# anihcsam/OpenGaussian

Measured on AMD Instinct MI355X. Metric: fwd+bwd Mpix/s at 1080p, 1M Gaussians (RGB+6-D ins_feat); k-means it/s, higher is better.
Workload: dtype f32; 1 GPU; S1M-1080p RGB(SH3)+depth+alpha (all grads) + 6-ch ins_feat (grad to ins_feat) fwd+bwd, ONE fused 9-channel pass; gaussians=1000000, width=1920, height=1080, views_cycled=8, parallelism=single

## Files before the change

include/ogs_raster.h:

```cpp
#ifndef OGS_RASTER_H
#define OGS_RASTER_H

#include <stddef.h>
#include <stdint.h>

#ifdef __cplusplus
extern "C" {
#endif

#define OGS_OK 0
#define OGS_ERR_INVALID_ARG (-1)
#define OGS_ERR_HIP (-2)
#define OGS_ERR_UNSUPPORTED (-3)
#define OGS_ERR_SCRATCH_TOO_SMALL (-4)
#define OGS_ERR_DEVICE (-5)

#define OGS_TILE 16
#define OGS_MAX_CHANNELS 12

typedef struct OgsRasterFwdArgs {
    int32_t P;
    int32_t W, H;
    int32_t C;
    int32_t sh_degree;
    int32_t sh_coeffs;
    float tanfovx, tanfovy;
    float scale_modifier;
    int32_t prefiltered;
    int32_t debug;
    const float* bg;
    const float* means3D;
    const float* colors_precomp;
    const float* shs;
    const float* opacities;
    const float* scales;
    const float* rotations;
    const float* cov3D_precomp;
    const float* viewmatrix;
    const float* projmatrix;
    const float* campos;
    float* out_color;
    float* out_depth;
    float* out_alpha;
    int32_t* radii;
    void* geom_buffer;
    void* geom_tmp;
    void* image_buffer;
    uint32_t* point_list;
    void* binning_tmp;
    void* sorted_rec;
    void* quad_list;
    const int32_t* group_ids;
    int32_t num_groups;
    int32_t full_binning;
} OgsRasterFwdArgs;

typedef struct OgsRasterBwdArgs {
    int32_t P, W, H, C, sh_degree, sh_coeffs;
    float tanfovx, tanfovy, scale_modifier;
    int32_t debug;
    int32_t num_rendered;
    int32_t geom_channels;
    const float* bg;
    const float* means3D;
    const float* colors_precomp;
    const float* shs;
    const float* opacities;
    const float* scales;
    const float* rotations;
    const float* cov3D_precomp;
    const float* viewmatrix;
    const float* projmatrix;
    const float* campos;
    const int32_t* radii;
    const float* out_alpha;
    const float* dL_dcolor;
    const float* dL_ddepth;
    const float* dL_dalpha;
    const void* geom_buffer;
    const void* image_buffer;
    const uint32_t* point_list;
    const void* sorted_rec;
    const void* quad_list;
    void* bwd_tmp;
    float* dL_dmeans2D;
    float* dL_dcolors;
    float* dL_dopacity;
    float* dL_dmeans3D;
    float* dL_dcov3D;
    float* dL_dsh;
    float* dL_dscales;
    float* dL_drotations;
    int32_t num_groups;
    float* dL_dsh_rgb;
} OgsRasterBwdArgs;

int ogs_version(void);
const char* ogs_last_error(void);

int ogs_check_async_status(void);

size_t ogs_raster_geom_bytes(int32_t P, int32_t C);
size_t ogs_raster_geom_tmp_bytes(int32_t P);
size_t ogs_raster_image_bytes(int32_t W, int32_t H);
size_t ogs_raster_image_bytes_grouped(int32_t W, int32_t H, int32_t num_groups);
size_t ogs_raster_binning_tmp_bytes(int64_t num_rendered, int32_t W, int32_t H);
size_t ogs_raster_backward_tmp_bytes(int32_t P);
size_t ogs_raster_sorted_bytes(int64_t num_rendered, int32_t C);
size_t ogs_raster_quad_list_bytes(int64_t num_rendered);

int ogs_raster_forward_geometry(const OgsRasterFwdArgs* args, void* stream, int64_t* num_rendered_host);

int ogs_raster_forward_render(const OgsRasterFwdArgs* args, int64_t num_rendered, void* stream);

int ogs_raster_read_num_rendered_async(const OgsRasterFwdArgs* args, void* stream, uint32_t* host_pinned);
int ogs_raster_forward_render_deferred(const OgsRasterFwdArgs* args, int64_t capacity, void* stream);

size_t ogs_raster_tiny_max_points(void);
int ogs_raster_forward_tiny(const OgsRasterFwdArgs* args, void* stream);

int ogs_raster_forward_reblend(const OgsRasterFwdArgs* args, void* stream);

int ogs_raster_compact_kept(int32_t W, int32_t H, int32_t C, const void* image_buffer, const void* sorted_rec,
                            const void* quad_list, void* new_image_buffer, void* new_sorted_rec, void* new_quad_list,
                            void* stream);

typedef struct OgsGroupStatsArgs {
    const int32_t* labels;
    int32_t num_labels;
    float alpha_threshold;
    float* max_alpha;
    int64_t* count;
    float* feat_sum;
    void* stats_tmp;
} OgsGroupStatsArgs;

size_t ogs_raster_stats_image_bytes(int32_t W, int32_t H, int32_t num_groups);
size_t ogs_raster_stats_tmp_bytes(int32_t num_groups, int32_t num_labels, int32_t C);
int ogs_raster_forward_group_stats(const OgsRasterFwdArgs* args, const OgsGroupStatsArgs* stats, int64_t num_rendered,
                                   void* stream);

int ogs_raster_backward(const OgsRasterBwdArgs* args, void* stream);

int ogs_mark_visible(int32_t P, const float* means3D, const float* viewmatrix, const float* projmatrix,
                     uint8_t* present, void* stream);

int ogs_sh_grad_from_views(int32_t P, int32_t V, int32_t sh_degree, int32_t sh_coeffs, const float* means3D,
                           const float* campos, const float* dL_drgb, float* dL_dsh, void* stream);

int ogs_raster_export_binning(const OgsRasterFwdArgs* args, int64_t num_rendered, uint64_t* keys_out,
                              uint32_t* ranges_out, uint32_t* n_contrib_out, void* stream);

int ogs_prof_enable(int on);
int ogs_prof_filter(const char* prefix);
int ogs_prof_collect(char* buf, size_t n);

int ogs_selftest_wave_fold16(const float* in, float* out, void* stream);
int ogs_selftest_tile_order(const uint32_t* ranges, int64_t vtiles, uint32_t* order, void* stream);
size_t ogs_selftest_radix_tmp_bytes(int64_t n);
int ogs_selftest_radix_sort(uint32_t* keys0, uint32_t* vals0, uint32_t* keys1, uint32_t* vals1, int64_t n, int32_t key_bits,
                            int32_t variant, int32_t items, const uint32_t* n_dev, void* tmp, int32_t* result_buffer,
                            void* stream);

#ifdef __cplusplus
}
#endif
#endif
```

opengaussian_amd/_lib.py:

```python
from __future__ import annotations

import ctypes as C
import os

_HERE = os.path.dirname(os.path.abspath(__file__))
LIB_PATH = os.environ.get("OGS_LIB_PATH") or os.path.join(_HERE, "lib", "libogs_hip.so")

_f32p = C.POINTER(C.c_float)
_vp = C.c_void_p


class OgsRasterFwdArgs(C.Structure):
    _fields_ = [
        ("P", C.c_int32), ("W", C.c_int32), ("H", C.c_int32), ("C", C.c_int32),
        ("sh_degree", C.c_int32), ("sh_coeffs", C.c_int32),
        ("tanfovx", C.c_float), ("tanfovy", C.c_float), ("scale_modifier", C.c_float),
        ("prefiltered", C.c_int32), ("debug", C.c_int32),
        ("bg", _vp), ("means3D", _vp), ("colors_precomp", _vp), ("shs", _vp), ("opacities", _vp),
        ("scales", _vp), ("rotations", _vp), ("cov3D_precomp", _vp),
        ("viewmatrix", _vp), ("projmatrix", _vp), ("campos", _vp),
        ("out_color", _vp), ("out_depth", _vp), ("out_alpha", _vp), ("radii", _vp),
        ("geom_buffer", _vp), ("geom_tmp", _vp), ("image_buffer", _vp), ("point_list", _vp),
        ("binning_tmp", _vp), ("sorted_rec", _vp), ("quad_list", _vp), ("group_ids", _vp), ("num_groups", C.c_int32),
        ("full_binning", C.c_int32),
    ]


class OgsRasterBwdArgs(C.Structure):
    _fields_ = [
        ("P", C.c_int32), ("W", C.c_int32), ("H", C.c_int32), ("C", C.c_int32),
        ("sh_degree", C.c_int32), ("sh_coeffs", C.c_int32),
        ("tanfovx", C.c_float), ("tanfovy", C.c_float), ("scale_modifier", C.c_float),
        ("debug", C.c_int32), ("num_rendered", C.c_int32), ("geom_channels", C.c_int32),
        ("bg", _vp), ("means3D", _vp), ("colors_precomp", _vp), ("shs", _vp), ("opacities", _vp),
        ("scales", _vp), ("rotations", _vp), ("cov3D_precomp", _vp),
        ("viewmatrix", _vp), ("projmatrix", _vp), ("campos", _vp),
        ("radii", _vp), ("out_alpha", _vp), ("dL_dcolor", _vp), ("dL_ddepth", _vp), ("dL_dalpha", _vp),
        ("geom_buffer", _vp), ("image_buffer", _vp), ("point_list", _vp), ("sorted_rec", _vp), ("quad_list", _vp), ("bwd_tmp", _vp),
        ("dL_dmeans2D", _vp), ("dL_dcolors", _vp), ("dL_dopacity", _vp), ("dL_dmeans3D", _vp),
        ("dL_dcov3D", _vp), ("dL_dsh", _vp), ("dL_dscales", _vp), ("dL_drotations", _vp), ("num_groups", C.c_int32), ("dL_dsh_rgb", _vp),
    ]


class OgsAdamTensor(C.Structure):
    _fields_ = [("param", _vp), ("grad", _vp), ("exp_avg", _vp), ("exp_avg_sq", _vp), ("numel", C.c_int64),
                ("lr", C.c_double), ("step", C.c_int64)]


class OgsRowTensor(C.Structure):
    _fields_ = [("src", _vp), ("dst", _vp), ("width", C.c_int32), ("zero_new", C.c_int32)]


class OgsDensifyArgs(C.Structure):
    _fields_ = [("N", C.c_int32), ("grad_accum", _vp), ("denom", _vp), ("scaling", _vp), ("opacity", _vp),
                ("max_grad", C.c_float), ("min_opacity", C.c_float), ("extent", C.c_float), ("percent_dense", C.c_float),
                ("prune_world_size", C.c_int32)]


class OgsGroupStatsArgs(C.Structure):
    _fields_ = [("labels", _vp), ("num_labels", C.c_int32), ("alpha_threshold", C.c_float), ("max_alpha", _vp),
                ("count", _vp), ("feat_sum", _vp), ("stats_tmp", _vp)]


SIGNATURES = {
    "ogs_version": (C.c_int, []),
    "ogs_last_error": (C.c_char_p, []),
    "ogs_raster_geom_bytes": (C.c_size_t, [C.c_int32, C.c_int32]),
    "ogs_raster_geom_tmp_bytes": (C.c_size_t, [C.c_int32]),
    "ogs_raster_image_bytes": (C.c_size_t, [C.c_int32, C.c_int32]),
    "ogs_raster_image_bytes_grouped": (C.c_size_t, [C.c_int32, C.c_int32, C.c_int32]),
    "ogs_raster_binning_tmp_bytes": (C.c_size_t, [C.c_int64, C.c_int32, C.c_int32]),
    "ogs_raster_backward_tmp_bytes": (C.c_size_t, [C.c_int32]),
    "ogs_raster_sorted_bytes": (C.c_size_t, [C.c_int64, C.c_int32]),
    "ogs_raster_quad_list_bytes": (C.c_size_t, [C.c_int64]),
    "ogs_raster_forward_geometry": (C.c_int, [C.POINTER(OgsRasterFwdArgs), _vp, C.POINTER(C.c_int64)]),
    "ogs_raster_forward_render": (C.c_int, [C.POINTER(OgsRasterFwdArgs), C.c_int64, _vp]),
    "ogs_raster_read_num_rendered_async": (C.c_int, [C.POINTER(OgsRasterFwdArgs), _vp, _vp]),
    "ogs_raster_forward_render_deferred": (C.c_int, [C.POINTER(OgsRasterFwdArgs), C.c_int64, _vp]),
    "ogs_raster_stats_image_bytes": (C.c_size_t, [C.c_int32, C.c_int32, C.c_int32]),
    "ogs_raster_stats_tmp_bytes": (C.c_size_t, [C.c_int32, C.c_int32, C.c_int32]),
    "ogs_raster_forward_group_stats": (C.c_int, [C.POINTER(OgsRasterFwdArgs), C.POINTER(OgsGroupStatsArgs), C.c_int64, _vp]),
    "ogs_raster_backward": (C.c_int, [C.POINTER(OgsRasterBwdArgs), _vp]),
    "ogs_raster_tiny_max_points": (C.c_size_t, []),
    "ogs_raster_forward_tiny": (C.c_int, [C.POINTER(OgsRasterFwdArgs), _vp]),
    "ogs_raster_forward_reblend": (C.c_int, [C.POINTER(OgsRasterFwdArgs), _vp]),
    "ogs_raster_compact_kept": (C.c_int, [C.c_int32, C.c_int32, C.c_int32, _vp, _vp, _vp, _vp, _vp, _vp, _vp]),
    "ogs_mark_visible": (C.c_int, [C.c_int32, _vp, _vp, _vp, _vp, _vp]),
    "ogs_sh_grad_from_views": (C.c_int, [C.c_int32, C.c_int32, C.c_int32, C.c_int32, _vp, _vp, _vp, _vp, _vp]),
    "ogs_raster_export_binning": (C.c_int, [C.POINTER(OgsRasterFwdArgs), C.c_int64, _vp, _vp, _vp, _vp]),
    "ogs_selftest_wave_fold16": (C.c_int, [_vp, _vp, _vp]),
    "ogs_selftest_tile_order": (C.c_int, [_vp, C.c_int64, _vp, _vp]),
    "ogs_selftest_radix_tmp_bytes": (C.c_size_t, [C.c_int64]),
    "ogs_selftest_radix_sort": (C.c_int, [_vp, _vp, _vp, _vp, C.c_int64, C.c_int32, C.c_int32, C.c_int32, _vp, _vp, _vp, _vp]),
    "ogs_check_async_status": (C.c_int, []),
    "ogs_prof_enable": (C.c_int, [C.c_int]),
    "ogs_prof_filter": (C.c_int, [C.c_char_p]),
    "ogs_prof_collect": (C.c_int, [C.c_char_p, C.c_size_t]),
    "ogs_kmeans_tmp_bytes": (C.c_size_t, [C.c_int64, C.c_int32, C.c_int32]),
    "ogs_kmeans_lloyd": (C.c_int, [_vp, C.c_int64, C.c_int32, _vp, C.c_int32, C.c_int32, C.c_int32, C.c_int32,
                                   _vp, C.c_int64, _vp, _vp]),
    "ogs_kmeans_assign": (C.c_int, [_vp, C.c_int64, C.c_int32, _vp, C.c_int32, _vp, C.c_int64, _vp]),
    "ogs_mask_feature_sums": (C.c_int, [_vp, _vp, _vp, C.c_int32, C.c_int32, C.c_int64, C.c_int32, _vp, _vp]),
    "ogs_mask_feature_sums_backward": (C.c_int, [_vp, _vp, _vp, _vp, _vp, C.c_int32, C.c_int32, C.c_int64, _vp, _vp, _vp]),
    "ogs_mask_cohesion": (C.c_int, [_vp, _vp, _vp, C.c_int32, C.c_int32, C.c_int64, _vp, _vp]),
    "ogs_mask_cohesion_backward": (C.c_int, [_vp, _vp, _vp, _vp, C.c_int32, C.c_int32, C.c_int64, _vp, _vp, _vp]),
    "ogs_separation_loss": (C.c_int, [_vp, C.c_int32, C.c_int32, C.c_int32, _vp, _vp, _vp, _vp]),
    "ogs_adam_step": (C.c_int, [C.POINTER(OgsAdamTensor), C.c_int32, C.c_double, C.c_double, C.c_double, _vp]),
    "ogs_rows_gather": (C.c_int, [C.POINTER(OgsRowTensor), C.c_int32, _vp, _vp, C.c_int64, _vp]),
    "ogs_densify_tmp_bytes": (C.c_size_t, [C.c_int32]),
    "ogs_densify_plan": (C.c_int, [C.POINTER(OgsDensifyArgs), _vp, C.POINTER(C.c_uint32), _vp]),
    "ogs_densify_map": (C.c_int, [C.c_int32, _vp, _vp, _vp, _vp, _vp]),
    "ogs_densify_split_children": (C.c_int, [C.c_int64, _vp, _vp, _vp, _vp, _vp, _vp, _vp, _vp, _vp, _vp]),
    "ogs_densify_stats": (C.c_int, [C.c_int32, _vp, C.c_int32, _vp, _vp, _vp, _vp, _vp, _vp]),
    "ogs_kmeans_accumulate": (C.c_int, [_vp, C.c_int64, C.c_int32, _vp, C.c_int32, C.c_int32, _vp, _vp, _vp]),
    "ogs_kmeans_update": (C.c_int, [_vp, C.c_int32, C.c_int32, C.c_int32, _vp, _vp, _vp]),
    "ogs_kmeans_gather": (C.c_int, [_vp, _vp, C.c_int64, C.c_int32, C.c_int32, _vp, _vp]),
}

_lib = None


class OgsError(RuntimeError):
    pass


def lib() -> C.CDLL:
    global _lib
    if _lib is None:
        if not os.path.exists(LIB_PATH):
            raise OgsError(f"{LIB_PATH} not found -- build it with `python -m opengaussian_amd.build` "
                           "(the product path has no CPU fallback)")
        l = C.CDLL(LIB_PATH)
        for name, (res, args) in SIGNATURES.items():
            fn = getattr(l, name)
            fn.restype = res
            fn.argtypes = args
        _lib = l
    return _lib


def check(rc: int, what: str):
    if rc != 0:
        raise OgsError(f"{what} failed (code {rc}): {lib().ogs_last_error().decode()}")


def prof_filter(prefix: str):
    check(lib().ogs_prof_filter(prefix.encode()), "ogs_prof_filter")


def prof_enable(mode):
    check(lib().ogs_prof_enable(int(mode)), "ogs_prof_enable")


def prof_collect() -> dict:
    import json
    buf = C.create_string_buffer(1 << 16)
    check(lib().ogs_prof_collect(buf, len(buf)), "ogs_prof_collect")
    return json.loads(buf.value.decode())


def ptr(t):
    return None if t is None else t.data_ptr()
```

opengaussian_amd/csrc/binning.hip:

```cpp
#include <stdlib.h>
#include <string.h>

#include "ogs_common.h"

namespace ogs {

namespace {

constexpr size_t kSweepHeaderWords = 4 * 256 + 4 + 60;
constexpr int kScanItems = 8;
constexpr int kScanTile = kBlock * kScanItems;

__device__ __forceinline__ uint32_t wave_inclusive_scan(uint32_t v) {
#pragma unroll
    for (int d = 1; d < kWave; d <<= 1) {
        uint32_t t = __shfl_up(v, d, kWave);
        if (lane_id() >= d) v += t;
    }
    return v;
}

__device__ __forceinline__ uint32_t block_exclusive_scan(uint32_t v, uint32_t& total, uint32_t* wave_sums ) {
    const int wave = threadIdx.x >> 6;
    const uint32_t inc = wave_inclusive_scan(v);
    if (lane_id() == kWave - 1) wave_sums[wave] = inc;
    __syncthreads();
    uint32_t base = 0, tot = 0;
#pragma unroll
    for (int w = 0; w < kBlock / kWave; ++w) {
        const uint32_t s = wave_sums[w];
        if (w < wave) base += s;
        tot += s;
    }
    total = tot;
    __syncthreads();
    return base + inc - v;
}

__device__ __forceinline__ void load_items(const uint32_t* __restrict__ in, const uint32_t* __restrict__ gather,
                                           int64_t base, int64_t n, uint32_t item[kScanItems]) {
#pragma unroll
    for (int i = 0; i < kScanItems; ++i) {
        const int64_t idx = base + i;
        uint32_t v = 0;
        if (idx < n) v = gather ? in[gather[idx]] : in[idx];
        item[i] = v;
    }
}

__global__ __launch_bounds__(kBlock) void scan_reduce_kernel(const uint32_t* __restrict__ in,
                                                             const uint32_t* __restrict__ gather, int64_t n,
                                                             uint32_t* __restrict__ partials, const uint32_t* __restrict__ n_dev) {
    __shared__ uint32_t wave_sums[4];
    if (n_dev) n = min(n, (int64_t)*n_dev);
    const int64_t base = (int64_t)blockIdx.x * kScanTile + (int64_t)threadIdx.x * kScanItems;
    uint32_t item[kScanItems];
    load_items(in, gather, base, n, item);
    uint32_t s = 0;
#pragma unroll
    for (int i = 0; i < kScanItems; ++i) s += item[i];
    uint32_t total;
    block_exclusive_scan(s, total, wave_sums);
    if (threadIdx.x == 0) partials[blockIdx.x] = total;
}

template <bool SUM_PARTIALS>
__global__ __launch_bounds__(kBlock) void scan_apply_kernel(const uint32_t* __restrict__ in,
                                                            const uint32_t* __restrict__ gather,
                                                            uint32_t* __restrict__ out, int64_t n,
                                                            const uint32_t* __restrict__ partial_offsets,
                                                            uint32_t* __restrict__ total_out, const uint32_t* __restrict__ n_dev) {
    __shared__ uint32_t wave_sums[4];
    if (n_dev) n = min(n, (int64_t)*n_dev);
    const int64_t base = (int64_t)blockIdx.x * kScanTile + (int64_t)threadIdx.x * kScanItems;
    uint32_t item[kScanItems];
    load_items(in, gather, base, n, item);
    uint32_t s = 0;
#pragma unroll
    for (int i = 0; i < kScanItems; ++i) s += item[i];
    uint32_t block_base = 0;
    if (SUM_PARTIALS) {
        uint32_t acc = 0;
        for (uint32_t j = threadIdx.x; j < blockIdx.x; j += kBlock) acc += partial_offsets[j];
        uint32_t tot;
        block_exclusive_scan(acc, tot, wave_sums);
        block_base = tot;
    } else if (partial_offsets) {
        block_base = partial_offsets[blockIdx.x];
    }
    uint32_t total;
    uint32_t run = block_exclusive_scan(s, total, wave_sums) + block_base;
#pragma unroll
    for (int i = 0; i < kScanItems; ++i) {
        const int64_t idx = base + i;
        if (idx < n) out[idx] = run;
        run += item[i];
    }
    if (total_out && threadIdx.x == 0) {
        if (SUM_PARTIALS) { if (blockIdx.x == gridDim.x - 1) *total_out = block_base + total; }
        else if (partial_offsets == nullptr) *total_out = total;
    }
}

__global__ void scan_total_kernel(const uint32_t* __restrict__ in, const uint32_t* __restrict__ gather,
                                  const uint32_t* __restrict__ out, int64_t n, uint32_t* __restrict__ total_out,
                                  const uint32_t* __restrict__ n_dev) {
    if (threadIdx.x == 0 && blockIdx.x == 0) {
        if (n_dev) n = min(n, (int64_t)*n_dev);
        if (n <= 0) { *total_out = 0u; return; }
        const uint32_t last = gather ? in[gather[n - 1]] : in[n - 1];
        *total_out = out[n - 1] + last;
    }
}

inline int scan_blocks(int64_t n) { return (int)((n + kScanTile - 1) / kScanTile); }
constexpr int kFlatScanBlocks = 16384;

template <int ITEMS>
__global__ __launch_bounds__(kBlock) void radix_hist_kernel(const uint32_t* __restrict__ keys, int64_t n_cap,
                                                            const uint32_t* __restrict__ n_dev, int shift,
                                                            int bits, uint32_t* __restrict__ hist, int nblocks, bool drop) {
    __shared__ uint32_t h[256];
    const int64_t n = n_dev ? min((int64_t)*n_dev, n_cap) : n_cap;
    const int ndig = 1 << bits;
    const uint32_t mask = ndig - 1;
    h[threadIdx.x] = 0;
    __syncthreads();
    const int64_t base = (int64_t)blockIdx.x * (kBlock * ITEMS);
#pragma unroll
    for (int i = 0; i < ITEMS; ++i) {
        const int64_t idx = base + i * kBlock + threadIdx.x;
        if (idx < n) {
            const uint32_t k = keys[idx];
            if (!(drop && k == kDropKey)) atomicAdd(&h[(k >> shift) & mask], 1u);
        }
    }
    __syncthreads();
    if ((int)threadIdx.x < ndig) hist[(size_t)threadIdx.x * nblocks + blockIdx.x] = h[threadIdx.x];
}

__global__ __launch_bounds__(kBlock) void radix_rowscan_kernel(uint32_t* __restrict__ hist, int nblocks,
                                                               uint32_t* __restrict__ row_total) {
    __shared__ uint32_t wave_sums[4];
    uint32_t* row = hist + (size_t)blockIdx.x * nblocks;
    uint32_t carry = 0;
    for (int base = 0; base < nblocks; base += kScanTile) {
        uint32_t item[kScanItems];
        const int b0 = base + (int)threadIdx.x * kScanItems;
        uint32_t sum = 0;
#pragma unroll
        for (int i = 0; i < kScanItems; ++i) {
            item[i] = (b0 + i < nblocks) ? row[b0 + i] : 0u;
            sum += item[i];
        }
        uint32_t total;
        uint32_t run = carry + block_exclusive_scan(sum, total, wave_sums);
#pragma unroll
        for (int i = 0; i < kScanItems; ++i) {
            if (b0 + i < nblocks) row[b0 + i] = run;
            run += item[i];
        }
        carry += total;
    }
    if (threadIdx.x == 0) row_total[blockIdx.x] = carry;
}

template <int ITEMS>
__global__ __launch_bounds__(kBlock) void radix_scatter_kernel(const uint32_t* __restrict__ keys_in,
                                                               const uint32_t* __restrict__ vals_in,
                                                               uint32_t* __restrict__ keys_out,
                                                               uint32_t* __restrict__ vals_out, int64_t n_cap,
                                                               const uint32_t* __restrict__ n_dev, int shift,
                                                               int bits, const uint32_t* __restrict__ offsets,
                                                               const uint32_t* __restrict__ row_total,
                                                               int nblocks, bool drop, uint32_t* __restrict__ kept_out) {
    __shared__ uint32_t wave_hist_s[kBlock / kWave][256];
    __shared__ uint32_t scan_sums[4];
    __shared__ uint32_t dig_start[256], glob_base[256];
    __shared__ uint32_t stage_k[kBlock * ITEMS], stage_v[kBlock * ITEMS];
    volatile uint32_t(*wave_hist)[256] = wave_hist_s;
    const int64_t n = n_dev ? min((int64_t)*n_dev, n_cap) : n_cap;
    const int ndig = 1 << bits;
    const uint32_t mask = ndig - 1;
    const int tid = threadIdx.x, lane = tid & 63, wave = tid >> 6;
#pragma unroll
    for (int w = 0; w < kBlock / kWave; ++w) wave_hist_s[w][tid] = 0;
    __syncthreads();

    const int64_t base = (int64_t)blockIdx.x * (kBlock * ITEMS) + (int64_t)wave * (ITEMS * kWave);
    uint32_t key[ITEMS], val[ITEMS], rank[ITEMS];
#pragma unroll
    for (int i = 0; i < ITEMS; ++i) {
        const int64_t idx = base + i * kWave + lane;
        const bool valid = idx < n;
        key[i] = valid ? keys_in[idx] : 0xFFFFFFFFu;
        val[i] = valid ? vals_in[idx] : 0u;
    }
    const uint64_t lt_mask = (1ull << lane) - 1ull;
#pragma unroll
    for (int i = 0; i < ITEMS; ++i) {
        const int64_t idx = base + i * kWave + lane;
        const bool valid = drop ? key[i] != kDropKey : idx < n;
        const uint32_t d = (key[i] >> shift) & mask;
        uint64_t peers = __ballot(valid);
        for (int b = 0; b < bits; ++b) {
            const bool bit = (d >> b) & 1u;
            const uint64_t m = __ballot(bit);
            peers &= bit ? m : ~m;
        }
        const uint32_t r = __popcll(peers & lt_mask);
        const uint32_t cnt = __popcll(peers);
        uint32_t pre = 0;
        if (valid) pre = wave_hist[wave][d];
        __builtin_amdgcn_wave_barrier();
        if (valid && r == 0) wave_hist[wave][d] = pre + cnt;
        __builtin_amdgcn_wave_barrier();
        rank[i] = pre + r;
    }
    __syncthreads();
    uint32_t run_len = 0;
    if (tid < ndig) {
#pragma unroll
        for (int w = 0; w < kBlock / kWave; ++w) {
            const uint32_t t = wave_hist_s[w][tid];
            wave_hist_s[w][tid] = run_len;
            run_len += t;
        }
    }
    uint32_t n_valid;
    const uint32_t local_start = block_exclusive_scan(run_len, n_valid, scan_sums);
    uint32_t dummy_total;
    const uint32_t digit_base = block_exclusive_scan(tid < ndig ? row_total[tid] : 0u, dummy_total, scan_sums);
    if (kept_out != nullptr && blockIdx.x == 0 && tid == 0) *kept_out = dummy_total;
    if (tid < ndig) {
        dig_start[tid] = local_start;
        glob_base[tid] = digit_base + offsets[(size_t)tid * nblocks + blockIdx.x] - local_start;
    }
    __syncthreads();
#pragma unroll
    for (int i = 0; i < ITEMS; ++i) {
        const int64_t idx = base + i * kWave + lane;
        if (drop ? key[i] != kDropKey : idx < n) {
            const uint32_t d = (key[i] >> shift) & mask;
            const uint32_t lp = dig_start[d] + wave_hist_s[wave][d] + rank[i];
            stage_k[lp] = key[i];
            stage_v[lp] = val[i];
        }
    }
    __syncthreads();
    for (uint32_t j = tid; j < n_valid; j += kBlock) {
        const uint32_t k = stage_k[j];
        const uint32_t pos = glob_base[(k >> shift) & mask] + j;
        keys_out[pos] = k;
        vals_out[pos] = stage_v[j];
    }
}

constexpr uint32_t kStatAgg = 1u << 30, kStatInc = 2u << 30, kStatMask = (1u << 30) - 1u;
constexpr int kSpinLimit = 1 << 22;
constexpr int kLookBack = 8;
constexpr int kHistAllBlocks = 256;

struct RadixPlanDev { int npass; int shift[4]; int bits[4]; };

__global__ __launch_bounds__(kBlock) void radix_hist_all_kernel(const uint32_t* __restrict__ keys, int64_t n_cap,
                                                                const uint32_t* __restrict__ n_dev, RadixPlanDev plan,
                                                                uint32_t* __restrict__ ghist , bool drop) {
    __shared__ uint32_t h[4][256];
    const int64_t n = n_dev ? min((int64_t)*n_dev, n_cap) : n_cap;
#pragma unroll
    for (int p = 0; p < 4; ++p) h[p][threadIdx.x] = 0;
    __syncthreads();
    for (int64_t idx = (int64_t)blockIdx.x * kBlock + threadIdx.x; idx < n; idx += (int64_t)gridDim.x * kBlock) {
        const uint32_t k = keys[idx];
        if (drop && k == kDropKey) continue;
#pragma unroll
        for (int p = 0; p < 4; ++p)
            if (p < plan.npass) atomicAdd(&h[p][(k >> plan.shift[p]) & ((1u << plan.bits[p]) - 1u)], 1u);
    }
    __syncthreads();
#pragma unroll
    for (int p = 0; p < 4; ++p)
        if (p < plan.npass && h[p][threadIdx.x] != 0) atomicAdd(&ghist[p * 256 + threadIdx.x], h[p][threadIdx.x]);
}

template <int ITEMS>
__global__ __launch_bounds__(kBlock) void radix_onesweep_kernel(const uint32_t* __restrict__ keys_in,
                                                                const uint32_t* __restrict__ vals_in,
                                                                uint32_t* __restrict__ keys_out,
                                                                uint32_t* __restrict__ vals_out, int64_t n_cap,
                                                                const uint32_t* __restrict__ n_dev, int shift, int bits,
                                                                const uint32_t* __restrict__ ghist ,
                                                                uint32_t* __restrict__ status ,
                                                                uint32_t* __restrict__ ticket ,
                                                                uint32_t* __restrict__ status_word ,
                                                                int spin_limit, bool drop,
                                                                uint32_t* __restrict__ kept_out) {
    __shared__ uint32_t wave_hist_s[kBlock / kWave][256];
    __shared__ uint32_t scan_sums[4];
    __shared__ uint32_t dig_start[256], glob_base[256];
    __shared__ uint32_t stage_k[kBlock * ITEMS], stage_v[kBlock * ITEMS];
    __shared__ uint32_t s_ticket;
    volatile uint32_t(*wave_hist)[256] = wave_hist_s;
    const int64_t n = n_dev ? min((int64_t)*n_dev, n_cap) : n_cap;
    const int ndig = 1 << bits;
    const uint32_t mask = ndig - 1;
    const int tid = threadIdx.x, lane = tid & 63, wave = tid >> 6;
    if (tid == 0) s_ticket = atomicAdd(ticket, 1u);
#pragma unroll
    for (int w = 0; w < kBlock / kWave; ++w) wave_hist_s[w][tid] = 0;
    __syncthreads();
    const uint32_t tile = s_ticket;
    if ((int64_t)tile * (kBlock * ITEMS) >= n) {
        if (kept_out != nullptr && tile == 0 && tid == 0) *kept_out = 0u;
        return;
    }

    const int64_t base = (int64_t)tile * (kBlock * ITEMS) + (int64_t)wave * (ITEMS * kWave);
    uint32_t key[ITEMS], val[ITEMS], rank[ITEMS];
#pragma unroll
    for (int i = 0; i < ITEMS; ++i) {
        const int64_t idx = base + i * kWave + lane;
        const bool valid = idx < n;
        key[i] = valid ? keys_in[idx] : 0xFFFFFFFFu;
        val[i] = valid ? vals_in[idx] : 0u;
    }
    const uint64_t lt_mask = (1ull << lane) - 1ull;
#pragma unroll
    for (int i = 0; i < ITEMS; ++i) {
        const int64_t idx = base + i * kWave + lane;
        const bool valid = drop ? key[i] != kDropKey : idx < n;
        const uint32_t d = (key[i] >> shift) & mask;
        uint64_t peers = __ballot(valid);
        for (int b = 0; b < bits; ++b) {
            const bool bit = (d >> b) & 1u;
            const uint64_t m = __ballot(bit);
            peers &= bit ? m : ~m;
        }
        const uint32_t r = __popcll(peers & lt_mask);
        const uint32_t cnt = __popcll(peers);
        uint32_t pre = 0;
        if (valid) pre = wave_hist[wave][d];
        __builtin_amdgcn_wave_barrier();
        if (valid && r == 0) wave_hist[wave][d] = pre + cnt;
        __builtin_amdgcn_wave_barrier();
        rank[i] = pre + r;
    }
    __syncthreads();
    uint32_t run_len = 0;
    if (tid < ndig) {
#pragma unroll
        for (int w = 0; w < kBlock / kWave; ++w) {
            const uint32_t t = wave_hist_s[w][tid];
            wave_hist_s[w][tid] = run_len;
            run_len += t;
        }
        __hip_atomic_store(&status[(size_t)tile * 256 + tid], (tile == 0 ? kStatInc : kStatAgg) | run_len,
                           __ATOMIC_RELAXED, __HIP_MEMORY_SCOPE_AGENT);
    }
    uint32_t n_valid;
    const uint32_t local_start = block_exclusive_scan(run_len, n_valid, scan_sums);
    uint32_t dummy_total;
    const uint32_t digit_base = block_exclusive_scan(tid < ndig ? ghist[tid] : 0u, dummy_total, scan_sums);
    if (kept_out != nullptr && tile == 0 && tid == 0) *kept_out = dummy_total;
    uint32_t before = 0;
    if (tid < ndig && tile > 0) {
        int64_t pb = (int64_t)tile - 1;
        int spins = 0;
        bool done = false;
        while (!done) {
            uint32_t sw[kLookBack];
#pragma unroll
            for (int k = 0; k < kLookBack; ++k)
                sw[k] = pb - k >= 0 ? __hip_atomic_load(&status[(size_t)(pb - k) * 256 + tid], __ATOMIC_RELAXED, __HIP_MEMORY_SCOPE_AGENT)
                                    : kStatInc;
            int used = 0;
#pragma unroll
            for (int k = 0; k < kLookBack; ++k) {
                if (done || used != k) continue;
                const uint32_t flag = sw[k] & ~kStatMask;
                if (flag == 0u) continue;
                before += sw[k] & kStatMask;
                used = k + 1;
                done = flag == kStatInc;
            }
            pb -= used;
            if (!done && used < kLookBack) {
                if (++spins > spin_limit) {
                    __hip_atomic_fetch_or(status_word, kAsyncRadixSpin, __ATOMIC_RELAXED, __HIP_MEMORY_SCOPE_SYSTEM);
                    break;
                }
                __builtin_amdgcn_s_sleep(1);
            }
        }
        __hip_atomic_store(&status[(size_t)tile * 256 + tid], kStatInc | ((before + run_len) & kStatMask),
                           __ATOMIC_RELAXED, __HIP_MEMORY_SCOPE_AGENT);
    }
    if (tid < ndig) {
        dig_start[tid] = local_start;
        glob_base[tid] = digit_base + before - local_start;
    }
    __syncthreads();
#pragma unroll
    for (int i = 0; i < ITEMS; ++i) {
        const int64_t idx = base + i * kWave + lane;
        if (drop ? key[i] != kDropKey : idx < n) {
            const uint32_t d = (key[i] >> shift) & mask;
            const uint32_t lp = dig_start[d] + wave_hist_s[wave][d] + rank[i];
            stage_k[lp] = key[i];
            stage_v[lp] = val[i];
        }
    }
    __syncthreads();
    for (uint32_t j = tid; j < n_valid; j += kBlock) {
        const uint32_t k = stage_k[j];
        const uint32_t pos = glob_base[(k >> shift) & mask] + j;
        if ((int64_t)pos < n) {
            keys_out[pos] = k;
            vals_out[pos] = stage_v[j];
        }
    }
}

constexpr int kRangeItems = 4;
__global__ __launch_bounds__(kBlock) void tile_ranges_kernel(const uint32_t* __restrict__ tile_keys, int64_t D_cap,
                                                             const uint32_t* __restrict__ n_dev,
                                                             uint2* __restrict__ ranges) {
    const int64_t D = n_dev ? min((int64_t)*n_dev, D_cap) : D_cap;
    const int64_t i0 = ((int64_t)blockIdx.x * kBlock + threadIdx.x) * kRangeItems;
    if (i0 >= D) return;
    uint32_t k[kRangeItems];
    if (i0 + kRangeItems <= D) {
        const uint4 v = *reinterpret_cast<const uint4*>(tile_keys + i0);
        k[0] = v.x; k[1] = v.y; k[2] = v.z; k[3] = v.w;
    } else {
#pragma unroll
        for (int j = 0; j < kRangeItems; ++j) k[j] = i0 + j < D ? tile_keys[i0 + j] : 0u;
    }
    uint32_t prev = i0 > 0 ? tile_keys[i0 - 1] : 0u;
#pragma unroll
    for (int j = 0; j < kRangeItems; ++j) {
        const int64_t i = i0 + j;
        if (i < D) {
            const uint32_t cur = k[j];
            if (i == 0) {
                ranges[cur].x = 0;
            } else if (prev != cur) {
                ranges[prev].y = (uint32_t)i;
                ranges[cur].x = (uint32_t)i;
            }
            if (i == D - 1) ranges[cur].y = (uint32_t)D;
            prev = cur;
        }
    }
}

__global__ __launch_bounds__(kBlock) void export_keys_kernel(const uint2* __restrict__ ranges,
                                                             const uint32_t* __restrict__ point_list,
                                                             const float4* __restrict__ rec, int recv4,
                                                             uint64_t* __restrict__ keys_out) {
    const uint32_t tile = blockIdx.x;
    const uint2 r = ranges[tile];
    for (uint32_t i = r.x + threadIdx.x; i < r.y; i += kBlock) {
        const uint32_t gid = point_list[i] & kGidMask;
        const uint32_t bits = __float_as_uint(rec[(size_t)gid * recv4].z);
        keys_out[i] = ((uint64_t)tile << 32) | bits;
    }
}

}

size_t scan_tmp_bytes(int64_t n) {
    size_t total = 0;
    int64_t m = n;
    while (true) {
        const int nb = scan_blocks(m);
        if (nb <= 1) break;
        total += align_up((size_t)nb * sizeof(uint32_t));
        m = nb;
    }
    return total + kAlign;
}

size_t sort_tmp_bytes(int64_t n) {
    const int64_t hist = (int64_t)256 * sort_blocks_for(n > 0 ? n : 1);
    const size_t legacy = align_up((size_t)hist * sizeof(uint32_t)) + align_up(256 * sizeof(uint32_t)) + scan_tmp_bytes(hist);
    const int64_t tiles4 = ((n > 0 ? n : 1) + kBlock * 4 - 1) / (kBlock * 4);
    const size_t sweep = align_up(kSweepHeaderWords * sizeof(uint32_t)) + 4 * align_up((size_t)256 * tiles4 * sizeof(uint32_t));
    return legacy > sweep ? legacy : sweep;
}

static int sweep_items_for(int64_t n, int forced) {
    if (forced == 4 || forced == 16) return forced;
    return n <= (int64_t)(256 << 10) ? 4 : 16;
}

bool radix_onesweep_enabled(int64_t n) {
    static const int forced = [] {
        const char* e = getenv("OGS_RADIX");
        return !e ? 0 : strcmp(e, "legacy") == 0 ? 1 : strcmp(e, "sweep") == 0 ? 2 : 0;
    }();
    if (forced == 1 || n >= (int64_t)kStatMask) return false;
    return forced == 2 || n <= (int64_t)(256 << 10);
}

namespace {
struct SweepTmp {
    uint32_t* ghist;
    uint32_t* ticket;
    uint32_t* status[4];
    size_t zero_bytes;
    static SweepTmp carve(void* tmp, int64_t n, int npass, int items_forced) {
        SweepTmp t;
        char* p = static_cast<char*>(tmp);
        t.ghist = reinterpret_cast<uint32_t*>(p);
        t.ticket = t.ghist + 4 * 256;
        const int items = sweep_items_for(n, items_forced);
        const int64_t tiles = ((n > 0 ? n : 1) + (int64_t)kBlock * items - 1) / ((int64_t)kBlock * items);
        const size_t table = align_up((size_t)256 * tiles * sizeof(uint32_t));
        char* q = p + align_up(kSweepHeaderWords * sizeof(uint32_t));
        for (int i = 0; i < 4; ++i) t.status[i] = reinterpret_cast<uint32_t*>(q + (size_t)i * table);
        t.zero_bytes = align_up(kSweepHeaderWords * sizeof(uint32_t)) + (size_t)npass * table;
        return t;
    }
};
}

int radix_sort_begin(const uint32_t* keys, int64_t n, const uint32_t* n_dev, int npass, const int* shifts, const int* bits,
                     void* tmp, hipStream_t stream, int debug, bool drop, int items) {
    if (n <= 0) return OGS_OK;
    if (npass < 1 || npass > 4) { set_error("radix_sort_begin: npass=%d out of range", npass); return OGS_ERR_INVALID_ARG; }
    const SweepTmp t = SweepTmp::carve(tmp, n, npass, items);
    OGS_HIP_CHECK(hipMemsetAsync(tmp, 0, t.zero_bytes, stream));
    RadixPlanDev plan{};
    plan.npass = npass;
    for (int i = 0; i < npass; ++i) {
        if (bits[i] < 1 || bits[i] > 8) { set_error("radix_sort_begin: bits=%d out of range", bits[i]); return OGS_ERR_INVALID_ARG; }
        plan.shift[i] = shifts[i];
        plan.bits[i] = bits[i];
    }
    const int64_t want = (n + kBlock * 16 - 1) / (kBlock * 16);
    const int grid = (int)(want < 1 ? 1 : (want > kHistAllBlocks ? kHistAllBlocks : want));
    OGS_LAUNCH(radix_hist_all_kernel, dim3(grid), dim3(kBlock), 0, stream, keys, n, n_dev, plan, t.ghist, drop);
    OGS_LAUNCH_CHECK(debug, stream);
    return OGS_OK;
}

int radix_sort_pass(int pass, int npass, const uint32_t* keys_in, const uint32_t* vals_in, uint32_t* keys_out, uint32_t* vals_out,
                    int64_t n, int shift, int bits, void* tmp, hipStream_t stream, int debug, const uint32_t* n_dev, bool drop,
                    uint32_t* kept_out, int items_forced, int spin_limit) {
    if (n <= 0) return OGS_OK;
    const SweepTmp t = SweepTmp::carve(tmp, n, npass, items_forced);
    const int items = sweep_items_for(n, items_forced);
    const int nb = (int)((n + (int64_t)kBlock * items - 1) / ((int64_t)kBlock * items));
    uint32_t* status_word = async_status_word();
    if (!status_word) return OGS_ERR_HIP;
    if (spin_limit < 0) spin_limit = kSpinLimit;
    if (items == 4) {
        OGS_LAUNCH(radix_onesweep_kernel<4>, dim3(nb), dim3(kBlock), 0, stream, keys_in, vals_in, keys_out, vals_out, n, n_dev,
                   shift, bits, (const uint32_t*)(t.ghist + pass * 256), t.status[pass], t.ticket + pass, status_word, spin_limit,
                   drop, kept_out);
    } else {
        OGS_LAUNCH(radix_onesweep_kernel<16>, dim3(nb), dim3(kBlock), 0, stream, keys_in, vals_in, keys_out, vals_out, n, n_dev,
                   shift, bits, (const uint32_t*)(t.ghist + pass * 256), t.status[pass], t.ticket + pass, status_word, spin_limit,
                   drop, kept_out);
    }
    OGS_LAUNCH_CHECK(debug, stream);
    return OGS_OK;
}

int exclusive_scan_u32(const uint32_t* in, const uint32_t* gather, uint32_t* out, int64_t n, uint32_t* total,
                       void* tmp, hipStream_t stream, int debug, const uint32_t* n_dev) {
    if (n <= 0) {
        if (total) OGS_HIP_CHECK(hipMemsetAsync(total, 0, sizeof(uint32_t), stream));
        return OGS_OK;
    }
    const int nb = scan_blocks(n);
    if (nb == 1) {
        OGS_LAUNCH(scan_apply_kernel<false>, dim3(1), dim3(kBlock), 0, stream, in, gather, out, n,
                           (const uint32_t*)nullptr, total, n_dev);
        OGS_LAUNCH_CHECK(debug, stream);
        return OGS_OK;
    }
    uint32_t* partials = static_cast<uint32_t*>(tmp);
    void* next_tmp = static_cast<char*>(tmp) + align_up((size_t)nb * sizeof(uint32_t));
    OGS_LAUNCH(scan_reduce_kernel, dim3(nb), dim3(kBlock), 0, stream, in, gather, n, partials, n_dev);
    OGS_LAUNCH_CHECK(debug, stream);
    if (nb <= kFlatScanBlocks) {
        OGS_LAUNCH(scan_apply_kernel<true>, dim3(nb), dim3(kBlock), 0, stream, in, gather, out, n,
                           (const uint32_t*)partials, total, n_dev);
        OGS_LAUNCH_CHECK(debug, stream);
        return OGS_OK;
    }
    int rc = exclusive_scan_u32(partials, nullptr, partials, nb, nullptr, next_tmp, stream, debug, nullptr);
    if (rc != OGS_OK) return rc;
    OGS_LAUNCH(scan_apply_kernel<false>, dim3(nb), dim3(kBlock), 0, stream, in, gather, out, n,
                       (const uint32_t*)partials, (uint32_t*)nullptr, n_dev);
    OGS_LAUNCH_CHECK(debug, stream);
    if (total) {
        if (in == out) { set_error("exclusive_scan_u32: total with in-place scan unsupported"); return OGS_ERR_INVALID_ARG; }
        OGS_LAUNCH(scan_total_kernel, dim3(1), dim3(64), 0, stream, in, gather, (const uint32_t*)out, n, total, n_dev);
        OGS_LAUNCH_CHECK(debug, stream);
    }
    return OGS_OK;
}

int radix_pass(const uint32_t* keys_in, const uint32_t* vals_in, uint32_t* keys_out, uint32_t* vals_out, int64_t n,
               int shift, int bits, void* tmp, hipStream_t stream, int debug, const uint32_t* n_dev, bool drop,
               uint32_t* kept_out) {
    if (n <= 0) return OGS_OK;
    if (bits < 1 || bits > 8) { set_error("radix_pass: bits=%d out of range", bits); return OGS_ERR_INVALID_ARG; }
    const int items = sort_items_for(n);
    const int nb = sort_blocks_for(n);
    const int ndig = 1 << bits;
    uint32_t* hist = static_cast<uint32_t*>(tmp);
    uint32_t* row_total = reinterpret_cast<uint32_t*>(static_cast<char*>(tmp) + align_up((size_t)256 * nb * sizeof(uint32_t)));
    if (items == 4) {
        OGS_LAUNCH(radix_hist_kernel<4>, dim3(nb), dim3(kBlock), 0, stream, keys_in, n, n_dev, shift, bits, hist, nb, drop);
    } else {
        OGS_LAUNCH(radix_hist_kernel<8>, dim3(nb), dim3(kBlock), 0, stream, keys_in, n, n_dev, shift, bits, hist, nb, drop);
    }
    OGS_LAUNCH_CHECK(debug, stream);
    OGS_LAUNCH(radix_rowscan_kernel, dim3(ndig), dim3(kBlock), 0, stream, hist, nb, row_total);
    OGS_LAUNCH_CHECK(debug, stream);
    if (items == 4) {
        OGS_LAUNCH(radix_scatter_kernel<4>, dim3(nb), dim3(kBlock), 0, stream, keys_in, vals_in, keys_out, vals_out, n, n_dev,
                   shift, bits, (const uint32_t*)hist, (const uint32_t*)row_total, nb, drop, kept_out);
    } else {
        OGS_LAUNCH(radix_scatter_kernel<8>, dim3(nb), dim3(kBlock), 0, stream, keys_in, vals_in, keys_out, vals_out, n, n_dev,
                   shift, bits, (const uint32_t*)hist, (const uint32_t*)row_total, nb, drop, kept_out);
    }
    OGS_LAUNCH_CHECK(debug, stream);
    return OGS_OK;
}

int launch_tile_ranges(const uint32_t* tile_keys_sorted, int64_t D, uint2* ranges, int64_t tiles, hipStream_t s,
                       int debug, const uint32_t* n_dev, bool already_zeroed) {
    if (!already_zeroed) OGS_HIP_CHECK(hipMemsetAsync(ranges, 0, (size_t)tiles * sizeof(uint2), s));
    if (D <= 0) return OGS_OK;
    const int grid = (int)((D + (int64_t)kBlock * kRangeItems - 1) / ((int64_t)kBlock * kRangeItems));
    OGS_LAUNCH(tile_ranges_kernel, dim3(grid), dim3(kBlock), 0, s, tile_keys_sorted, D, n_dev, ranges);
    OGS_LAUNCH_CHECK(debug, s);
    return OGS_OK;
}

int launch_export_keys(const uint2* ranges, int tiles, const uint32_t* point_list, const float4* rec, int recv4,
                       uint64_t* keys_out, hipStream_t s) {
    OGS_LAUNCH(export_keys_kernel, dim3(tiles), dim3(kBlock), 0, s, ranges, point_list, rec, recv4, keys_out);
    OGS_LAUNCH_CHECK(0, s);
    return OGS_OK;
}

}
```

opengaussian_amd/csrc/blend_fwd.hip:

```cpp
#include "ogs_common.h"

namespace ogs {

namespace {

constexpr float kAlphaMin = 1.0f / 255.0f;
typedef float v2f __attribute__((ext_vector_type(2)));

__device__ __forceinline__ uint64_t shfl_up_u64(uint64_t v, int d) {
    const uint32_t lo = __shfl_up((uint32_t)v, d, kWave), hi = __shfl_up((uint32_t)(v >> 32), d, kWave);
    return ((uint64_t)hi << 32) | lo;
}


template <int C>
struct RowRec {
    static constexpr int NV4 = stream_vec4(C);
    float4 v[NV4];
    __device__ __forceinline__ void load_lds(const float4* __restrict__ p) {
#pragma unroll
        for (int k = 0; k < NV4; ++k) v[k] = p[k];
    }
    __device__ __forceinline__ float at(int i) const {
        const float4 q = v[i >> 2];
        return (i & 3) == 0 ? q.x : (i & 3) == 1 ? q.y : (i & 3) == 2 ? q.z : q.w;
    }
    __device__ __forceinline__ float feat(int c) const { return at(8 + c); }
};

constexpr int kRowSlots = 65;
constexpr int kRowListLen = 72;
template <int C>
struct RowsLds {
    float4 s_rec[kBlock / kWave][kRowSlots * stream_vec4(C)];
    uint32_t s_list[kBlock / kWave][4][kRowListLen];
};

template <int C, int RF = -1>
__device__ __forceinline__ void blend_rows_tile(
    const uint2 range, int n, int n_kept, const float* __restrict__ stream,
    const uint32_t* __restrict__ quad_list, int W, int H, int gx, int img, int timg, const float* __restrict__ bg, float* __restrict__ out_color,
    float* __restrict__ out_depth, float* __restrict__ out_alpha, uint32_t* __restrict__ n_contrib,
    float* __restrict__ final_T, int pf_lines, RowsLds<C>& lds, const float* __restrict__ feats = nullptr) {
    constexpr int NV4 = stream_vec4(C);
    constexpr int RS = NV4 * 4;
    constexpr int kListLen = kRowListLen;
    auto& s_rec = lds.s_rec;
    auto& s_list = lds.s_list;
    const int tx = timg % gx, ty = timg / gx;
    const int tid = threadIdx.x, lane = tid & 63, wave = __builtin_amdgcn_readfirstlane(tid >> 6);
    const int row = lane >> 4, l16 = lane & 15;
    const int qx0 = tx * kTile + (wave & 1) * 8, qy0 = ty * kTile + (wave >> 1) * 8;
    const int px = qx0 + 4 * (row & 1) + (l16 & 3);
    const int py = qy0 + 4 * (row >> 1) + (l16 >> 2);
    const bool inside = px < W && py < H;
    const float fy = (float)py;

    const int n_tile = (int)(range.y - range.x);
    const float* __restrict__ tb = stream + (size_t)range.x * RS;
    const uint32_t* __restrict__ qi = quad_list + ((size_t)range.x * 5 + (size_t)wave * n_tile);
    const uint32_t lim = n_kept > 0 ? (uint32_t)n_kept - 1u : 0u;
    RecordPrefetch pf;
    pf.issue(tb, n_kept, RS, tid, pf_lines);

    float4* __restrict__ recs = s_rec[wave];
    uint32_t* __restrict__ mylist = s_list[wave][row];
    if (lane == 0) {
#pragma unroll
        for (int k = 0; k < NV4; ++k) recs[64 * NV4 + k] = float4{0.f, 0.f, 0.f, 0.f};
        recs[64 * NV4 + 1] = float4{0.f, -1.f, 0.f, 0.f};
    }
    float fxe = inside ? (float)px : kFar;
    float T = 1.0f;
    constexpr int NPF = (C + 2) / 2;
    v2f accp[NPF];
#pragma unroll
    for (int k = 0; k < NPF; ++k) accp[k] = (v2f){0.f, 0.f};
    float wacc = 0.f;
    uint32_t last = 0;
    bool all_done = false;

    constexpr uint32_t kNoEntry = 0xFFFFFFFFu;
    uint32_t last_e = kNoEntry;
    auto consume = [&](const RowRec<C>& rec, uint32_t entry) {
        const v2f d = (v2f){rec.at(0), rec.at(1)} - (v2f){fxe, fy};
        const v2f m = (v2f){rec.at(2), rec.at(3)} * d;
        const float u = fmaf(rec.at(4), d.y, m.x);
        const float power = fmaf(m.y, d.y, u * d.x);
        const float h = rec.at(5);
        const bool cand = fabsf(power + h) <= h;
        if (__ballot(cand) != 0ull) {
            const float araw = fminf(0.99f, rec.at(6) * __expf(power));
            const bool act = cand && araw >= kAlphaMin;
            const float alpha = act ? araw : 0.f;
            const float test_T = T * (1.0f - alpha);
            const bool stop = test_T < 0.0001f;
            const float w = stop ? 0.f : alpha * T;
            const v2f w2 = {w, w};
#pragma unroll
            for (int k = 0; k < NPF; ++k)
                accp[k] = __builtin_elementwise_fma((v2f){rec.feat(2 * k), rec.feat(2 * k + 1)}, w2, accp[k]);
            wacc += w;
            T = stop ? T : test_T;
            last_e = (act && !stop) ? entry : last_e;
            fxe = stop ? kFar : fxe;
            if (__ballot(stop) != 0ull) all_done = __ballot(fxe < kFarTest) == 0ull;
        }
    };

    const float bx0 = (float)(qx0 + 4 * 0), by0 = (float)qy0;
    for (int c0 = 0; c0 < n && !all_done; c0 += kWave) {
        const int cnt = min(kWave, n - c0);
        const bool have = lane < cnt;
        const uint32_t ridx = have ? min(qi[c0 + lane], lim) : 0u;
        const float4* __restrict__ rp = reinterpret_cast<const float4*>(tb + (size_t)ridx * RS);
        float4 r[NV4];
#pragma unroll
        for (int k = 0; k < NV4; ++k) r[k] = rp[k];
        if constexpr (RF >= 0) {
            constexpr int E = C - RF;
            const float* __restrict__ fp = feats + (size_t)__float_as_uint(r[1].w) * E;
            float fv[E];
#pragma unroll
            for (int k = 0; k < E; ++k) fv[k] = fp[k];
            float* rf = reinterpret_cast<float*>(r);
#pragma unroll
            for (int k = 0; k < E; ++k) rf[8 + RF + k] = fv[k];
        }
#pragma unroll
        for (int k = 0; k < NV4; ++k) recs[lane * NV4 + k] = r[k];
        bool reach[4];
        {
            const float gxp = r[0].x, gyp = r[0].y;
            const float A = -2.f * r[0].z, B = -r[1].x, Cc = -2.f * r[0].w, thr = -2.f * r[1].y;
            const float nbA = -B / A, nbC = -B / Cc;
#pragma unroll
            for (int b = 0; b < 4; ++b) {
                const float ox = bx0 + 4.f * (float)(b & 1), oy = by0 + 4.f * (float)(b >> 1);
                const float m = max_power_in_box(A, B, Cc, nbA, nbC, gxp - ox - 3.f, gxp - ox, gyp - oy - 3.f, gyp - oy);
                reach[b] = have && m >= thr;
            }
        }
        constexpr uint32_t kDummy = (64u << 16) | (64u * NV4 * 16u);
#pragma unroll
        for (int b = 0; b < 4; ++b) s_list[wave][b][lane] = kDummy;
        if (lane < kListLen - kWave) {
#pragma unroll
            for (int b = 0; b < 4; ++b) s_list[wave][b][kWave + lane] = kDummy;
        }
        int maxlen = 0;
#pragma unroll
        for (int b = 0; b < 4; ++b) {
            const uint64_t mask = __ballot(reach[b]);
            const int pos = (int)__builtin_amdgcn_mbcnt_hi((uint32_t)(mask >> 32), __builtin_amdgcn_mbcnt_lo((uint32_t)mask, 0u));
            if (reach[b]) s_list[wave][b][pos] = ((uint32_t)lane << 16) | ((uint32_t)lane * NV4 * 16u);
            maxlen = max(maxlen, (int)__popcll(mask));
        }
        __builtin_amdgcn_fence(__ATOMIC_RELEASE, "wavefront");
        __builtin_amdgcn_wave_barrier();
        RowRec<C> ra, rb;
        auto rec_of = [&](uint32_t e) {
            return reinterpret_cast<const float4*>(reinterpret_cast<const char*>(recs) + (e & 0xFFFFu));
        };
        uint32_t e0 = mylist[0], e1 = mylist[1];
        ra.load_lds(rec_of(e0));
        for (int t = 0; t < maxlen && !all_done; t += 2) {
            const uint32_t e2 = mylist[t + 2], e3 = mylist[t + 3];
            rb.load_lds(rec_of(e1));
            consume(ra, e0);
            ra.load_lds(rec_of(e2));
            if (t + 1 < maxlen) consume(rb, e1);
            e0 = e2; e1 = e3;
        }
        if (last_e != kNoEntry) last = (uint32_t)c0 + (last_e >> 16) + 1u;
        last_e = kNoEntry;
        __builtin_amdgcn_wave_barrier();
    }

    if (inside) {
        const size_t plane = (size_t)W * H;
        const size_t pix = (size_t)img * plane + (size_t)py * W + px;
        float* oc = out_color + (size_t)img * (C - 1) * plane;
#pragma unroll
        for (int c = 0; c < C; ++c) oc[c * plane + pix] = ((c & 1) ? accp[c / 2].y : accp[c / 2].x) + T * bg[c];
        out_depth[pix] = (C & 1) ? accp[C / 2].y : accp[C / 2].x;
        out_alpha[pix] = wacc;
        n_contrib[pix] = last;
        final_T[pix] = T;
    }
    pf.retire(n_contrib, W);
}

template <int C, int RF = -1>
__global__ __launch_bounds__(kBlock) void blend_forward_rows_kernel(
    const uint2* __restrict__ ranges, const uint32_t* __restrict__ qcount, const float* __restrict__ stream,
    const uint32_t* __restrict__ quad_list, int W, int H, int gx, int tiles, const float* __restrict__ bg, float* __restrict__ out_color,
    float* __restrict__ out_depth, float* __restrict__ out_alpha, uint32_t* __restrict__ n_contrib,
    float* __restrict__ final_T, int pf_lines, const uint32_t* __restrict__ tile_order, const float* __restrict__ feats) {
    __shared__ RowsLds<C> lds;
    const int tile = tile_order ? (int)tile_order[blockIdx.x] : (int)blockIdx.x;
    const int img = tile / tiles, timg = tile - img * tiles;
    const int wave = __builtin_amdgcn_readfirstlane((int)threadIdx.x >> 6);
    blend_rows_tile<C, RF>(ranges[tile], (int)qcount[tile * 5 + wave], (int)qcount[tile * 5 + 4], stream, quad_list, W, H, gx, img, timg,
                           bg, out_color, out_depth, out_alpha, n_contrib, final_T, pf_lines, lds, feats);
}

template <int C>
struct ChunkLds {
    static constexpr int SV = stream_vec4(C);
    uint64_t wave_tot[kBlock / kWave];
    uint32_t done[kBlock / kWave];
    float4 s_rec[(kBlock + 1) * SV];
    uint32_t s_list[kBlock / kWave][4][kRowListLen];
    uint8_t s_qnew[4][kBlock];
};

struct GroupStatsOut {
    const int32_t* labels;
    int32_t L;
    float thr;
    uint32_t* max_alpha;
    unsigned long long* count;
    unsigned long long* fsum;
};

constexpr float kFixedScale = 4294967296.0f;

__device__ __forceinline__ unsigned long long shfl_xor_u64(unsigned long long v, int m) {
    const uint32_t lo = __shfl_xor((uint32_t)v, m, kWave), hi = __shfl_xor((uint32_t)(v >> 32), m, kWave);
    return ((unsigned long long)hi << 32) | lo;
}

template <int C>
__device__ __forceinline__ void group_stats_epilogue(const GroupStatsOut& st, float* __restrict__ s_buf, int img, int W, int pix,
                                                     float alpha, const float (&colour)[C]) {
    float* s_val = s_buf;
    float* s_alpha = s_buf + C * kBlock;
    int* s_key = reinterpret_cast<int*>(s_buf + (C + 1) * kBlock);
    const int tid = threadIdx.x, lane = tid & 63;
    int key = -1;
    if (pix >= 0 && alpha > st.thr) {
        const int l = st.labels[pix];
        key = (l >= 0 && l < st.L) ? l : st.L;
    }
    s_key[tid] = key;
    s_alpha[tid] = pix >= 0 ? alpha : 0.f;
#pragma unroll
    for (int c = 0; c < C; ++c) s_val[c * kBlock + tid] = colour[c];
    lds_barrier();
    if (tid >= kWave) return;
    int k[kBlock / kWave];
    float m = 0.f;
#pragma unroll
    for (int j = 0; j < kBlock / kWave; ++j) {
        k[j] = s_key[lane + kWave * j];
        m = fmaxf(m, s_alpha[lane + kWave * j]);
    }
#pragma unroll
    for (int off = kWave / 2; off > 0; off >>= 1) m = fmaxf(m, __shfl_xor(m, off, kWave));
    if (lane == 0 && m > 0.f) atomicMax(st.max_alpha + img, __float_as_uint(m));
    const size_t row0 = (size_t)img * (size_t)(st.L + 1);
    for (;;) {
        int cand = -1;
#pragma unroll
        for (int j = kBlock / kWave - 1; j >= 0; --j) cand = k[j] >= 0 ? k[j] : cand;
        const uint64_t pending = __ballot(cand >= 0);
        if (pending == 0ull) break;
        const int K = __shfl(cand, __ffsll((unsigned long long)pending) - 1, kWave);
        unsigned long long cnt = 0, sum[C];
#pragma unroll
        for (int c = 0; c < C; ++c) sum[c] = 0ull;
#pragma unroll
        for (int j = 0; j < kBlock / kWave; ++j) {
            if (k[j] == K) {
                ++cnt;
#pragma unroll
                for (int c = 0; c < C; ++c) sum[c] += (unsigned long long)__float2ll_rn(s_val[c * kBlock + lane + kWave * j] * kFixedScale);
                k[j] = -1;
            }
        }
#pragma unroll
        for (int off = kWave / 2; off > 0; off >>= 1) {
            cnt += (unsigned long long)__shfl_xor((uint32_t)cnt, off, kWave);
#pragma unroll
            for (int c = 0; c < C; ++c) sum[c] += shfl_xor_u64(sum[c], off);
        }
        if (lane == 0) {
            const size_t r = row0 + (size_t)K;
            atomicAdd(st.count + r, cnt);
#pragma unroll
            for (int c = 0; c < C; ++c) atomicAdd(st.fsum + r * C + c, sum[c]);
        }
    }
}

__global__ __launch_bounds__(256) void group_stats_finish_kernel(const long long* __restrict__ fsum, float* __restrict__ out, size_t n) {
    const size_t i = (size_t)blockIdx.x * 256 + threadIdx.x;
    if (i < n) out[i] = (float)((double)fsum[i] * (1.0 / 4294967296.0));
}

template <int C, bool STATS = false>
__global__ __launch_bounds__(kBlock) __attribute__((amdgpu_waves_per_eu(6, 8)))
void pack_blend_chunked_kernel(
    const uint2* __restrict__ ranges, const uint32_t* __restrict__ point_list, const float4* __restrict__ rec,
    float4* __restrict__ stream, uint32_t* __restrict__ quad_list, uint32_t* __restrict__ qcount, int W, int H, int gx, int tiles,
    const float* __restrict__ bg, float* __restrict__ out_color, float* __restrict__ out_depth, float* __restrict__ out_alpha,
    uint32_t* __restrict__ n_contrib, float* __restrict__ final_T, const uint32_t* __restrict__ tile_order,
    GroupStatsOut st = GroupStatsOut{}) {
    constexpr int NV = rec_vec4(C);
    constexpr int SV = stream_vec4(C);
    constexpr int kListLen = kRowListLen;
    __shared__ ChunkLds<C> lds;
    const int tile = tile_order ? (int)tile_order[blockIdx.x] : (int)blockIdx.x;
    const int img = tile / tiles, timg = tile - img * tiles;
    const uint2 range = ranges[tile];
    const int n = (int)(range.y - range.x);
    const int tx = timg % gx, ty = timg / gx;
    const int tid = threadIdx.x, lane = tid & 63, wave = __builtin_amdgcn_readfirstlane(tid >> 6);
    const float X0 = (float)(tx * kTile), Y0 = (float)(ty * kTile);
    const int row = lane >> 4, l16 = lane & 15;
    const int qx0 = tx * kTile + (wave & 1) * 8, qy0 = ty * kTile + (wave >> 1) * 8;
    const int px = qx0 + 4 * (row & 1) + (l16 & 3);
    const int py = qy0 + 4 * (row >> 1) + (l16 >> 2);
    const bool inside = px < W && py < H;
    const float fy = (float)py;
    float fxe = inside ? (float)px : kFar;
    float T = 1.0f;
    constexpr int NPF = (C + 2) / 2;
    v2f accp[NPF];
#pragma unroll
    for (int k = 0; k < NPF; ++k) accp[k] = (v2f){0.f, 0.f};
    float wacc = 0.f;
    uint32_t last = 0;
    uint64_t alive = __ballot(inside);

    const float4* __restrict__ recs = lds.s_rec;
    uint32_t* __restrict__ mylist = lds.s_list[wave][row];
    if (tid == 0) {
#pragma unroll
        for (int k = 0; k < SV; ++k) lds.s_rec[kBlock * SV + k] = float4{0.f, 0.f, 0.f, 0.f};
        lds.s_rec[kBlock * SV + 1] = float4{0.f, -1.f, 0.f, 0.f};
    }

    constexpr uint32_t kNoEntry = 0xFFFFFFFFu;
    uint32_t last_e = kNoEntry;
    auto consume = [&](const RowRec<C>& r, uint32_t entry) {
        const v2f d = (v2f){r.at(0), r.at(1)} - (v2f){fxe, fy};
        const v2f m = (v2f){r.at(2), r.at(3)} * d;
        const float u = fmaf(r.at(4), d.y, m.x);
        const float power = fmaf(m.y, d.y, u * d.x);
        const float h = r.at(5);
        const bool cand = fabsf(power + h) <= h;
        if (__ballot(cand) != 0ull) {
            const float araw = fminf(0.99f, r.at(6) * __expf(power));
            const bool act = cand && araw >= kAlphaMin;
            const float alpha = act ? araw : 0.f;
            const float test_T = T * (1.0f - alpha);
            const bool stop = test_T < 0.0001f;
            float w = alpha * T;
            bool contributes = act;
            if (__ballot(stop) != 0ull) {
                w = stop ? 0.f : w;
                T = stop ? T : test_T;
                fxe = stop ? kFar : fxe;
                alive = __ballot(fxe < kFarTest);
                contributes = act && !stop;
            } else {
                T = test_T;
            }
            const v2f w2 = {w, w};
#pragma unroll
            for (int k = 0; k < NPF; ++k)
                accp[k] = __builtin_elementwise_fma((v2f){r.feat(2 * k), r.feat(2 * k + 1)}, w2, accp[k]);
            wacc += w;
            last_e = contributes ? entry : last_e;
        }
    };

    uint32_t running[5];
#pragma unroll
    for (int q = 0; q < 5; ++q) running[q] = 0u;
    const float bx0 = (float)qx0, by0 = (float)qy0;

    for (int base = 0; base < n; base += kBlock) {
        const int i = base + tid;
        uint32_t mask = 0;
        float4 a = make_float4(0, 0, 0, 0), b = a;
        float h = 0.f;
        uint32_t gid_of_thread = 0;
        const uint32_t sv = i < n ? point_list[range.x + i] : 0u;
        if (sv >> kReachBit) {
            const uint32_t gid = sv & kGidMask;
            gid_of_thread = gid;
            const float4* src = rec + (size_t)gid * NV;
            a = src[0]; b = src[1];
            h = 0.5f * (__logf(255.0f * b.w) + kThrMargin);
            const float thr = -2.0f * h;
            const float nbA = -b.y / b.x, nbC = -b.y / b.z;
#pragma unroll
            for (int q = 0; q < 4; ++q) {
                const float qx = X0 + (float)((q & 1) * 8), qy = Y0 + (float)((q >> 1) * 8);
                const float m = max_power_in_box(b.x, b.y, b.z, nbA, nbC, a.x - qx - 7.f, a.x - qx, a.y - qy - 7.f, a.y - qy);
                if (m >= thr) mask |= 1u << q;
            }
        }
        const uint64_t mine = (uint64_t)(mask & 1u) | ((uint64_t)((mask >> 1) & 1u) << 12) |
                              ((uint64_t)((mask >> 2) & 1u) << 24) | ((uint64_t)((mask >> 3) & 1u) << 36) |
                              ((uint64_t)(mask != 0u ? 1u : 0u) << 48);
        uint64_t inc = mine;
#pragma unroll
        for (int d = 1; d < kWave; d <<= 1) {
            const uint64_t t = shfl_up_u64(inc, d);
            if (lane >= d) inc += t;
        }
        if (lane == kWave - 1) lds.wave_tot[wave] = inc;
        lds_barrier();
        uint64_t before = 0, total = 0;
#pragma unroll
        for (int w = 0; w < kBlock / kWave; ++w) {
            const uint64_t t = lds.wave_tot[w];
            if (w < wave) before += t;
            total += t;
        }
        const uint64_t pos = before + inc - mine;
        if (mask) {
            const uint32_t c_loc = (uint32_t)(pos >> 48) & 0xFFFu;
            const uint32_t c_idx = running[4] + c_loc;
            float4* dst = lds.s_rec + c_loc * SV;
            dst[0] = make_float4(a.x, a.y, -0.5f * b.x, -0.5f * b.z);
            dst[1] = make_float4(-b.y, h, b.w, __uint_as_float(gid_of_thread));
            const float4* src = rec + (size_t)gid_of_thread * NV;
            float f[(SV - 2) * 4];
#pragma unroll
            for (int k = 0; k < (SV - 2) * 4; ++k) f[k] = 0.f;
#pragma unroll
            for (int v = 0; v < NV - 2; ++v) {
                const float4 t = src[2 + v];
                f[4 * v] = t.x; f[4 * v + 1] = t.y; f[4 * v + 2] = t.z; f[4 * v + 3] = t.w;
            }
            f[C] = a.z;
#pragma unroll
            for (int v = 0; v < SV - 2; ++v) dst[2 + v] = make_float4(f[4 * v], f[4 * v + 1], f[4 * v + 2], f[4 * v + 3]);
#pragma unroll
            for (int q = 0; q < 4; ++q) {
                if (mask & (1u << q)) {
                    const uint32_t pq = (uint32_t)(pos >> (12 * q)) & 0xFFFu;
                    if constexpr (!STATS) quad_list[(size_t)range.x * 5 + (size_t)q * n + running[q] + pq] = c_idx;
                    lds.s_qnew[q][pq] = (uint8_t)c_loc;
                }
            }
            if constexpr (!STATS) quad_list[(size_t)range.x * 5 + (size_t)4 * n + c_idx] = (uint32_t)i;
        }
        lds_barrier();
        if constexpr (!STATS) {
            const int kept4 = (int)((uint32_t)(total >> 48) & 0xFFFu) * SV;
            float4* __restrict__ out = stream + ((size_t)range.x + (size_t)running[4]) * SV;
            for (int e = tid; e < kept4; e += kBlock) out[e] = lds.s_rec[e];
        }
        const int cnt_q = (int)((uint32_t)(total >> (12 * wave)) & 0xFFFu);
        const uint32_t j0 = wave == 0 ? running[0] : wave == 1 ? running[1] : wave == 2 ? running[2] : running[3];
        for (int c0 = 0; c0 < cnt_q && alive != 0ull; c0 += kWave) {
            const int cnt = min(kWave, cnt_q - c0);
            const bool have = lane < cnt;
            const uint32_t cl = have ? (uint32_t)lds.s_qnew[wave][c0 + lane] : (uint32_t)kBlock;
            const float4 r0 = recs[cl * SV], r1 = recs[cl * SV + 1];
            bool reach[4];
            {
                const float gxp = r0.x, gyp = r0.y;
                const float A = -2.f * r0.z, B = -r1.x, Cc = -2.f * r0.w, thr = -2.f * r1.y;
                const float nbA = -B / A, nbC = -B / Cc;
#pragma unroll
                for (int bb = 0; bb < 4; ++bb) {
                    const float ox = bx0 + 4.f * (float)(bb & 1), oy = by0 + 4.f * (float)(bb >> 1);
                    const float m = max_power_in_box(A, B, Cc, nbA, nbC, gxp - ox - 3.f, gxp - ox, gyp - oy - 3.f, gyp - oy);
                    reach[bb] = have && m >= thr;
                }
            }
            constexpr uint32_t kDummy = (64u << 16) | ((uint32_t)kBlock * SV * 16u);
#pragma unroll
            for (int bb = 0; bb < 4; ++bb) lds.s_list[wave][bb][lane] = kDummy;
            if (lane < kListLen - kWave) {
#pragma unroll
                for (int bb = 0; bb < 4; ++bb) lds.s_list[wave][bb][kWave + lane] = kDummy;
            }
            int maxlen = 0;
#pragma unroll
            for (int bb = 0; bb < 4; ++bb) {
                const uint64_t m64 = __ballot(reach[bb]);
                const int p = (int)__builtin_amdgcn_mbcnt_hi((uint32_t)(m64 >> 32), __builtin_amdgcn_mbcnt_lo((uint32_t)m64, 0u));
                if (reach[bb]) lds.s_list[wave][bb][p] = ((uint32_t)lane << 16) | (cl * SV * 16u);
                maxlen = max(maxlen, (int)__popcll(m64));
            }
            __builtin_amdgcn_fence(__ATOMIC_RELEASE, "wavefront");
            __builtin_amdgcn_wave_barrier();
            RowRec<C> ra, rb;
            auto rec_of = [&](uint32_t e) {
                return reinterpret_cast<const float4*>(reinterpret_cast<const char*>(recs) + (e & 0xFFFFu));
            };
            uint32_t e0 = mylist[0], e1 = mylist[1];
            ra.load_lds(rec_of(e0));
            const uint32_t jbase = j0 + (uint32_t)c0 + 1u;
            for (int t = 0; t < maxlen && alive != 0ull; t += 2) {
                const uint32_t e2 = mylist[t + 2], e3 = mylist[t + 3];
                rb.load_lds(rec_of(e1));
                consume(ra, e0);
                ra.load_lds(rec_of(e2));
                if (t + 1 < maxlen) consume(rb, e1);
                e0 = e2; e1 = e3;
            }
            if (last_e != kNoEntry) last = jbase + (last_e >> 16);
            last_e = kNoEntry;
            __builtin_amdgcn_wave_barrier();
        }
#pragma unroll
        for (int q = 0; q < 5; ++q) running[q] += (uint32_t)(total >> (12 * q)) & 0xFFFu;
        if (lane == 0) lds.done[wave] = alive == 0ull ? 1u : 0u;
        lds_barrier();
        if ((lds.done[0] & lds.done[1] & lds.done[2] & lds.done[3]) != 0u) break;
    }
    if constexpr (STATS) {
        float colour[C];
#pragma unroll
        for (int c = 0; c < C; ++c) colour[c] = ((c & 1) ? accp[c / 2].y : accp[c / 2].x) + T * bg[c];
        group_stats_epilogue<C>(st, reinterpret_cast<float*>(lds.s_rec), img, W, inside ? py * W + px : -1, wacc, colour);
    } else {
        if (tid == 0) {
#pragma unroll
            for (int q = 0; q < 5; ++q) qcount[tile * 5 + q] = running[q];
        }
        if (inside) {
            const size_t plane = (size_t)W * H;
            const size_t pix = (size_t)img * plane + (size_t)py * W + px;
            float* oc = out_color + (size_t)img * (C - 1) * plane;
#pragma unroll
            for (int c = 0; c < C; ++c) oc[c * plane + pix] = ((c & 1) ? accp[c / 2].y : accp[c / 2].x) + T * bg[c];
            out_depth[pix] = (C & 1) ? accp[C / 2].y : accp[C / 2].x;
            out_alpha[pix] = wacc;
            n_contrib[pix] = last;
            final_T[pix] = T;
        }
    }
}

template <int C>
__global__ __launch_bounds__(kBlock) void export_n_contrib_kernel(const uint2* __restrict__ ranges,
                                                                  const uint32_t* __restrict__ point_list,
                                                                  const uint32_t* __restrict__ quad_list, int W, int H,
                                                                  int gx, int tiles, const uint32_t* __restrict__ n_contrib,
                                                                  uint32_t* __restrict__ out) {
    const int tile = blockIdx.x;
    const int img = tile / tiles, timg = tile - img * tiles;
    const int tx = timg % gx, ty = timg / gx;
    const int tid = threadIdx.x, lane = tid & 63, wave = tid >> 6;
    const int px = tx * kTile + (wave & 1) * 8 + (lane & 7);
    const int py = ty * kTile + (wave >> 1) * 8 + (lane >> 3);
    if (px >= W || py >= H) return;
    const uint2 range = ranges[tile];
    const int n_tile = (int)(range.y - range.x);
    n_contrib += (size_t)img * W * H;
    out += (size_t)img * W * H;
    const uint32_t last = n_contrib[(size_t)py * W + px];
    uint32_t res = 0;
    if (last > 0) {
        const uint32_t c_idx = quad_list[(size_t)range.x * 5 + (size_t)wave * n_tile + (last - 1)];
        res = quad_list[(size_t)range.x * 5 + (size_t)4 * n_tile + c_idx] + 1u;
    }
    out[(size_t)py * W + px] = res;
}

template <int C>
__global__ __launch_bounds__(kBlock) void tiny_blend_kernel(int P, const uint32_t* __restrict__ order,
                                                            const float4* __restrict__ rec, int W, int H, int gx,
                                                            const float* __restrict__ bg, float* __restrict__ out_color,
                                                            float* __restrict__ out_depth, float* __restrict__ out_alpha) {
    constexpr int NV = rec_vec4(C);
    constexpr int RS = 8 + (C + 1 + 3) / 4 * 4;
    static_assert(kTinyMaxP == kBlock, "one staging round");
    __shared__ float s_rec[kTinyMaxP * RS];
    __shared__ uint32_t s_wave_cnt[kBlock / kWave];
    const int tile = blockIdx.x;
    const int tx = tile % gx, ty = tile / gx;
    const int tid = threadIdx.x, lane = tid & 63, wave = tid >> 6;
    const int gy = (H + kTile - 1) / kTile;

    bool keep = false;
    float4 a = make_float4(0, 0, 0, 0), b = a;
    uint32_t gid = 0;
    if (tid < P) {
        gid = order[tid];
        const float4* src = rec + (size_t)gid * NV;
        a = src[0]; b = src[1];
        const int radius = __float_as_int(a.w);
        if (radius > 0) {
            const float rf = (float)radius;
            auto tr = [](float v) -> int {
                if (!(fabsf(v) < 3.0e38f)) v = 0.f;
                v = fminf(fmaxf(v, -2.0e9f), 2.0e9f);
                return (int)v;
            };
            const int rminx = min(gx, max(0, tr((a.x - rf) / (float)kTile)));
            const int rminy = min(gy, max(0, tr((a.y - rf) / (float)kTile)));
            const int rmaxx = min(gx, max(0, tr((a.x + rf + (float)kTile - 1.0f) / (float)kTile)));
            const int rmaxy = min(gy, max(0, tr((a.y + rf + (float)kTile - 1.0f) / (float)kTile)));
            keep = tx >= rminx && tx < rmaxx && ty >= rminy && ty < rmaxy;
        }
    }
    const uint64_t bal = __ballot(keep);
    if (lane == 0) s_wave_cnt[wave] = (uint32_t)__popcll(bal);
    __syncthreads();
    uint32_t before = 0, n = 0;
#pragma unroll
    for (int w = 0; w < kBlock / kWave; ++w) {
        const uint32_t c = s_wave_cnt[w];
        if (w < wave) before += c;
        n += c;
    }
    if (keep) {
        const uint32_t pos = before + (uint32_t)__popcll(bal & ((1ull << lane) - 1ull));
        float* dst = s_rec + pos * RS;
        dst[0] = a.x; dst[1] = a.y; dst[2] = -0.5f * b.x; dst[3] = -b.y; dst[4] = -0.5f * b.z;
        dst[5] = 0.5f * (__logf(255.0f * b.w) + kThrMargin);
        dst[6] = b.w; dst[7] = __uint_as_float(gid);
        const float4* src = rec + (size_t)gid * NV;
        float f[(NV - 2) * 4 + 4];
#pragma unroll
        for (int v = 0; v < NV - 2; ++v) {
            const float4 t = src[2 + v];
            f[4 * v] = t.x; f[4 * v + 1] = t.y; f[4 * v + 2] = t.z; f[4 * v + 3] = t.w;
        }
#pragma unroll
        for (int c = 0; c < C; ++c) dst[8 + c] = f[c];
        dst[8 + C] = a.z;
    }
    __syncthreads();

    const int px = tx * kTile + (wave & 1) * 8 + (lane & 7);
    const int py = ty * kTile + (wave >> 1) * 8 + (lane >> 3);
    const bool inside = px < W && py < H;
    const float fx = (float)px, fy = (float)py;
    float T = 1.0f, wacc = 0.f;
    float acc[C + 1];
#pragma unroll
    for (int c = 0; c <= C; ++c) acc[c] = 0.f;
    bool done = !inside;
    for (uint32_t j = 0; j < n; ++j) {
        if (__ballot(!done) == 0ull) break;
        const float* r = s_rec + j * RS;
        const float dx = r[0] - fx, dy = r[1] - fy;
        const float power = blend_power(r[2], r[3], r[4], dx, dy);
        const bool cand = !done && fabsf(power + r[5]) <= r[5];
        if (cand) {
            float alpha = fminf(0.99f, r[6] * __expf(power));
            alpha = alpha >= kAlphaMin ? alpha : 0.f;
            const float test_T = T * (1.0f - alpha);
            const bool stop = test_T < 0.0001f;
            const float w = stop ? 0.f : alpha * T;
#pragma unroll
            for (int c = 0; c <= C; ++c) acc[c] = fmaf(r[8 + c], w, acc[c]);
            wacc += w;
            T = stop ? T : test_T;
            done = stop;
        }
    }
    if (inside) {
        const size_t plane = (size_t)W * H;
        const size_t pix = (size_t)py * W + px;
#pragma unroll
        for (int c = 0; c < C; ++c) out_color[c * plane + pix] = acc[c] + T * bg[c];
        out_depth[pix] = acc[C];
        out_alpha[pix] = wacc;
    }
}

template <int C>
int tiny_c(const OgsRasterFwdArgs& a, const GeomState& gs, const uint32_t* order, hipStream_t s) {
    const int gx = (a.W + kTile - 1) / kTile, gy = (a.H + kTile - 1) / kTile;
    OGS_LAUNCH(tiny_blend_kernel<C>, dim3((unsigned)(gx * gy)), dim3(kBlock), 0, s, a.P, order, (const float4*)gs.rec, a.W, a.H,
               gx, a.bg, a.out_color, a.out_depth, a.out_alpha);
    OGS_LAUNCH_CHECK(a.debug, s);
    return OGS_OK;
}


constexpr int kOrderThreads = 1024;
constexpr int64_t kOrderMaxTiles = 1 << 16;
__device__ __forceinline__ uint32_t work_class(uint32_t n) {
    if (n < 8u) return 255u - n;
    const uint32_t e = 31u - (uint32_t)__builtin_clz(n);
    const uint32_t v = e * 8u + ((n >> (e - 3u)) & 7u);
    return 255u - min(v, 255u);
}
__device__ __forceinline__ uint32_t class_counter_add(uint32_t* bins, uint32_t cls, bool valid, int lane) {
    uint32_t pos = 0u;
    uint64_t todo = __ballot(valid);
    while (todo != 0ull) {
        const int leader = __ffsll((unsigned long long)todo) - 1;
        const uint32_t c0 = (uint32_t)__shfl((int)cls, leader, kWave);
        const uint64_t same = __ballot(valid && cls == c0) & todo;
        uint32_t base = 0u;
        if (lane == leader) base = atomicAdd(&bins[c0], (uint32_t)__popcll(same));
        base = (uint32_t)__shfl((int)base, leader, kWave);
        if ((same >> lane) & 1ull) pos = base + (uint32_t)__popcll(same & ((1ull << lane) - 1ull));
        todo &= ~same;
    }
    return pos;
}
__global__ __launch_bounds__(kOrderThreads) void tile_order_kernel(const uint2* __restrict__ ranges, uint32_t vtiles,
                                                                   uint32_t* __restrict__ order) {
    __shared__ uint32_t bins[256];
    __shared__ uint32_t wave_max[kOrderThreads / kWave], wave_sum[kOrderThreads / kWave];
    const uint32_t tid = threadIdx.x;
    uint32_t my_max = 0u, my_sum = 0u;
    for (uint32_t t0 = 0; t0 < vtiles; t0 += 8u * kOrderThreads) {
        uint2 r[8];
#pragma unroll
        for (int k = 0; k < 8; ++k) {
            const uint32_t t = t0 + (uint32_t)k * kOrderThreads + tid;
            r[k] = t < vtiles ? ranges[t] : make_uint2(0u, 0u);
        }
#pragma unroll
        for (int k = 0; k < 8; ++k) { my_max = max(my_max, r[k].y - r[k].x); my_sum += r[k].y - r[k].x; }
    }
#pragma unroll
    for (int d = 32; d >= 1; d >>= 1) {
        my_max = max(my_max, (uint32_t)__shfl_xor((int)my_max, d, kWave));
        my_sum += (uint32_t)__shfl_xor((int)my_sum, d, kWave);
    }
    if ((tid & 63u) == 0u) { wave_max[tid >> 6] = my_max; wave_sum[tid >> 6] = my_sum; }
    if (tid < 256u) bins[tid] = 0u;
    __syncthreads();
    uint32_t longest = 0u;
    unsigned long long total = 0ull;
#pragma unroll
    for (int w = 0; w < kOrderThreads / kWave; ++w) { longest = max(longest, wave_max[w]); total += wave_sum[w]; }
    if ((unsigned long long)longest * vtiles <= 2ull * total) {
        for (uint32_t t = tid; t < vtiles; t += kOrderThreads) order[t] = t;
        return;
    }
    for (uint32_t t0 = 0; t0 < vtiles; t0 += kOrderThreads) {
        const uint32_t t = t0 + tid;
        const bool valid = t < vtiles;
        const uint2 r = valid ? ranges[t] : make_uint2(0u, 0u);
        (void)class_counter_add(bins, work_class(r.y - r.x), valid, (int)(tid & 63u));
    }
    __syncthreads();
    if (tid < 64u) {
        uint32_t c[4], sum = 0u;
#pragma unroll
        for (int k = 0; k < 4; ++k) { c[k] = bins[tid * 4u + k]; sum += c[k]; }
        uint32_t incl = sum;
#pragma unroll
        for (int d = 1; d < 64; d <<= 1) {
            const uint32_t o = __shfl_up(incl, d, kWave);
            if ((int)tid >= d) incl += o;
        }
        uint32_t base = incl - sum;
#pragma unroll
        for (int k = 0; k < 4; ++k) { bins[tid * 4u + k] = base; base += c[k]; }
    }
    __syncthreads();
    for (uint32_t t0 = 0; t0 < vtiles; t0 += kOrderThreads) {
        const uint32_t t = t0 + tid;
        const bool valid = t < vtiles;
        const uint2 r = valid ? ranges[t] : make_uint2(0u, 0u);
        const uint32_t pos = class_counter_add(bins, work_class(r.y - r.x), valid, (int)(tid & 63u));
        if (valid) order[pos] = t;
    }
}

template <int C>
int launch_c(const OgsRasterFwdArgs& a, const GeomState& gs, const ImageState& is, int64_t D, hipStream_t s) {
    const int gx = (a.W + kTile - 1) / kTile, gy = (a.H + kTile - 1) / kTile;
    const int tiles = gx * gy;
    const unsigned vtiles = (unsigned)tiles * (unsigned)num_groups_of(a.num_groups);
    if (D > 0) {
        const uint32_t* order = launch_tile_order(is, vtiles, a.P, s, a.debug);
        static constexpr const char* const kChunked[4] = {"pack_blend_chunked_kernel<3>", "pack_blend_chunked_kernel<6>",
                                                          "pack_blend_chunked_kernel<9>", "pack_blend_chunked_kernel<12>"};
        OGS_LAUNCH_NAMED(chan_name<C>(kChunked), pack_blend_chunked_kernel<C>, dim3(vtiles), dim3(kBlock), 0, s,
                         (const uint2*)is.ranges, (const uint32_t*)a.point_list, (const float4*)gs.rec, stream_base<C>(a.sorted_rec),
                         quad_base(a.quad_list), is.qcount, a.W, a.H, gx, tiles, a.bg, a.out_color, a.out_depth, a.out_alpha,
                         is.n_contrib, is.final_T, order);
        OGS_LAUNCH_CHECK(a.debug, s);
        return OGS_OK;
    }
    OGS_HIP_CHECK(hipMemsetAsync(is.qcount, 0, (size_t)vtiles * 5 * sizeof(uint32_t), s));
    static constexpr const char* const kRows[4] = {"blend_forward_rows_kernel<3>", "blend_forward_rows_kernel<6>",
                                                   "blend_forward_rows_kernel<9>", "blend_forward_rows_kernel<12>"};
    OGS_LAUNCH_NAMED(chan_name<C>(kRows), blend_forward_rows_kernel<C>, dim3(vtiles), dim3(kBlock), 0, s,
                     (const uint2*)is.ranges, (const uint32_t*)is.qcount, (const float*)stream_base<C>(a.sorted_rec),
                     (const uint32_t*)quad_base(a.quad_list), a.W, a.H, gx, tiles, a.bg, a.out_color, a.out_depth,
                     a.out_alpha, is.n_contrib, is.final_T, blend_prefetch_lines(), (const uint32_t*)nullptr, (const float*)nullptr);
    OGS_LAUNCH_CHECK(a.debug, s);
    return OGS_OK;
}

template <int C>
int stats_c(const OgsRasterFwdArgs& a, const OgsGroupStatsArgs& sa, const GeomState& gs, const ImageState& is, hipStream_t s) {
    const int gx = (a.W + kTile - 1) / kTile, gy = (a.H + kTile - 1) / kTile;
    const int tiles = gx * gy;
    const int G = num_groups_of(a.num_groups);
    const unsigned vtiles = (unsigned)tiles * (unsigned)G;
    const size_t rows = (size_t)G * (size_t)(sa.num_labels + 1);
    long long* fixed = static_cast<long long*>(sa.stats_tmp);
    OGS_HIP_CHECK(hipMemsetAsync(sa.max_alpha, 0, (size_t)G * sizeof(float), s));
    OGS_HIP_CHECK(hipMemsetAsync(sa.count, 0, rows * sizeof(int64_t), s));
    OGS_HIP_CHECK(hipMemsetAsync(fixed, 0, rows * C * sizeof(long long), s));
    const uint32_t* order = launch_tile_order(is, vtiles, a.P, s, a.debug);
    GroupStatsOut st;
    st.labels = sa.labels;
    st.L = sa.num_labels;
    st.thr = sa.alpha_threshold;
    st.max_alpha = reinterpret_cast<uint32_t*>(sa.max_alpha);
    st.count = reinterpret_cast<unsigned long long*>(sa.count);
    st.fsum = reinterpret_cast<unsigned long long*>(fixed);
    static constexpr const char* const kStats[4] = {"pack_blend_chunked_kernel<3, stats>", "pack_blend_chunked_kernel<6, stats>",
                                                    "pack_blend_chunked_kernel<9, stats>", "pack_blend_chunked_kernel<12, stats>"};
    OGS_LAUNCH_NAMED(chan_name<C>(kStats), (pack_blend_chunked_kernel<C, true>), dim3(vtiles), dim3(kBlock), 0, s,
                     (const uint2*)is.ranges, (const uint32_t*)a.point_list, (const float4*)gs.rec, (float4*)nullptr,
                     (uint32_t*)nullptr, (uint32_t*)nullptr, a.W, a.H, gx, tiles, a.bg, (float*)nullptr, (float*)nullptr,
                     (float*)nullptr, (uint32_t*)nullptr, (float*)nullptr, order, st);
    OGS_LAUNCH_CHECK(a.debug, s);
    const size_t n = rows * C;
    OGS_LAUNCH(group_stats_finish_kernel, dim3((unsigned)((n + 255) / 256)), dim3(256), 0, s, (const long long*)fixed,
               sa.feat_sum, n);
    OGS_LAUNCH_CHECK(a.debug, s);
    return OGS_OK;
}

template <int C>
int reblend_c(const OgsRasterFwdArgs& a, const ImageState& is, hipStream_t s) {
    const int gx = (a.W + kTile - 1) / kTile, gy = (a.H + kTile - 1) / kTile;
    const int tiles = gx * gy;
    const unsigned vtiles = (unsigned)tiles;
    const uint32_t* order = tile_order_of(is, vtiles, a.P);
    static constexpr const char* const kRows[4] = {"blend_forward_rows_kernel<3, refresh>", "blend_forward_rows_kernel<6, refresh>",
                                                   "blend_forward_rows_kernel<9, refresh>", "blend_forward_rows_kernel<12, refresh>"};
    const float* stream = reinterpret_cast<const float*>(stream_base<C>(a.sorted_rec));
#define OGS_REBLEND(RFV)                                                                                                    \
    OGS_LAUNCH_NAMED(chan_name<C>(kRows), (blend_forward_rows_kernel<C, RFV>), dim3(vtiles), dim3(kBlock), 0, s,           \
                     (const uint2*)is.ranges, (const uint32_t*)is.qcount, stream, (const uint32_t*)quad_base(a.quad_list), a.W,  \
                     a.H, gx, tiles, a.bg, a.out_color, a.out_depth, a.out_alpha, is.n_contrib, is.final_T,                  \
                     blend_prefetch_lines(), order, a.colors_precomp)
    if (a.sh_coeffs != 0) {
        if constexpr (C > 3) {
            OGS_REBLEND(3);
        } else {
            set_error("forward_reblend: a 3-channel SH pass has no channel to replace");
            return OGS_ERR_INVALID_ARG;
        }
    } else {
        OGS_REBLEND(0);
    }
#undef OGS_REBLEND
    OGS_LAUNCH_CHECK(a.debug, s);
    return OGS_OK;
}

template <int C>
__global__ __launch_bounds__(kBlock) void compact_kept_kernel(const uint2* __restrict__ old_ranges, const uint2* __restrict__ new_ranges,
                                                              const uint32_t* __restrict__ qcount, const float4* __restrict__ old_rec,
                                                              const uint32_t* __restrict__ old_quad, float4* __restrict__ new_rec,
                                                              uint32_t* __restrict__ new_quad) {
    constexpr int SV = stream_vec4(C);
    const int tile = blockIdx.x;
    const uint2 ro = old_ranges[tile], rn = new_ranges[tile];
    const uint32_t n_old = ro.y - ro.x, k = qcount[tile * 5 + 4];
    const float4* __restrict__ src = old_rec + (size_t)ro.x * SV;
    float4* __restrict__ dst = new_rec + (size_t)rn.x * SV;
    for (uint32_t e = threadIdx.x; e < k * SV; e += kBlock) dst[e] = src[e];
#pragma unroll
    for (int q = 0; q < 4; ++q) {
        const uint32_t nq = qcount[tile * 5 + q];
        const uint32_t* __restrict__ qs = old_quad + ((size_t)ro.x * 5 + (size_t)q * n_old);
        uint32_t* __restrict__ qd = new_quad + ((size_t)rn.x * 5 + (size_t)q * k);
        for (uint32_t e = threadIdx.x; e < nq; e += kBlock) qd[e] = qs[e];
    }
}

template <int C>
int compact_c(int W, int H, const ImageState& is_old, const ImageState& is_new, const void* old_rec, const void* old_quad,
              void* new_rec, void* new_quad, hipStream_t s) {
    const int gx = (W + kTile - 1) / kTile, gy = (H + kTile - 1) / kTile;
    OGS_LAUNCH(compact_kept_kernel<C>, dim3((unsigned)(gx * gy)), dim3(kBlock), 0, s, (const uint2*)is_old.ranges,
               (const uint2*)is_new.ranges, (const uint32_t*)is_old.qcount, (const float4*)stream_base<C>(const_cast<void*>(old_rec)),
               (const uint32_t*)quad_base(const_cast<void*>(old_quad)), stream_base<C>(new_rec), quad_base(new_quad));
    OGS_LAUNCH_CHECK(0, s);
    return OGS_OK;
}

template <int C>
int export_c(const OgsRasterFwdArgs& a, const ImageState& is, uint32_t* out, hipStream_t s) {
    const int gx = (a.W + kTile - 1) / kTile, gy = (a.H + kTile - 1) / kTile;
    OGS_LAUNCH(export_n_contrib_kernel<C>, dim3((unsigned)(gx * gy) * (unsigned)num_groups_of(a.num_groups)), dim3(kBlock), 0,
               s, (const uint2*)is.ranges, (const uint32_t*)a.point_list, (const uint32_t*)quad_base(a.quad_list), a.W,
               a.H, gx, gx * gy, (const uint32_t*)is.n_contrib, out);
    OGS_LAUNCH_CHECK(0, s);
    return OGS_OK;
}

}

static bool tile_order_enabled() {
    static const bool v = [] { const char* e = getenv("OGS_TILE_ORDER"); return !(e && atoi(e) == 0); }();
    return v;
}
const uint32_t* tile_order_of(const ImageState& is, int64_t vtiles, int P) {
    return (tile_order_enabled() && vtiles > 1 && vtiles <= kOrderMaxTiles && (int64_t)P >= 4 * vtiles) ? is.tile_order : nullptr;
}
const uint32_t* launch_tile_order(const ImageState& is, int64_t vtiles, int P, hipStream_t s, int debug) {
    const uint32_t* order = tile_order_of(is, vtiles, P);
    if (!order) return nullptr;
    OGS_LAUNCH(tile_order_kernel, dim3(1), dim3(kOrderThreads), 0, s, (const uint2*)is.ranges, (uint32_t)vtiles, is.tile_order);
    if (debug) (void)hipStreamSynchronize(s);
    return order;
}

int launch_tile_order_test(const uint32_t* ranges, int64_t vtiles, uint32_t* order, hipStream_t s) {
    if (vtiles > kOrderMaxTiles) { set_error("selftest: more than %lld tiles", (long long)kOrderMaxTiles); return OGS_ERR_UNSUPPORTED; }
    OGS_LAUNCH(tile_order_kernel, dim3(1), dim3(kOrderThreads), 0, s, (const uint2*)ranges, (uint32_t)vtiles, order);
    OGS_LAUNCH_CHECK(1, s);
    return OGS_OK;
}

int launch_blend_forward(const OgsRasterFwdArgs& a, const GeomState& gs, const ImageState& is, int64_t D,
                         hipStream_t s) {
    switch (a.C) {
        case 3: return launch_c<3>(a, gs, is, D, s);
        case 6: return launch_c<6>(a, gs, is, D, s);
        case 9: return launch_c<9>(a, gs, is, D, s);
        case 12: return launch_c<12>(a, gs, is, D, s);
        default: set_error("unsupported channel count C=%d", a.C); return OGS_ERR_UNSUPPORTED;
    }
}

int launch_group_stats(const OgsRasterFwdArgs& a, const OgsGroupStatsArgs& st, const GeomState& gs, const ImageState& is,
                       hipStream_t s) {
    switch (a.C) {
        case 3: return stats_c<3>(a, st, gs, is, s);
        case 6: return stats_c<6>(a, st, gs, is, s);
        case 9: return stats_c<9>(a, st, gs, is, s);
        case 12: return stats_c<12>(a, st, gs, is, s);
        default: set_error("unsupported channel count C=%d", a.C); return OGS_ERR_UNSUPPORTED;
    }
}

int launch_compact_kept(int W, int H, int C, const ImageState& is_old, const ImageState& is_new, const void* old_rec,
                        const void* old_quad, void* new_rec, void* new_quad, hipStream_t s) {
    switch (C) {
        case 3: return compact_c<3>(W, H, is_old, is_new, old_rec, old_quad, new_rec, new_quad, s);
        case 6: return compact_c<6>(W, H, is_old, is_new, old_rec, old_quad, new_rec, new_quad, s);
        case 9: return compact_c<9>(W, H, is_old, is_new, old_rec, old_quad, new_rec, new_quad, s);
        case 12: return compact_c<12>(W, H, is_old, is_new, old_rec, old_quad, new_rec, new_quad, s);
        default: set_error("unsupported channel count C=%d", C); return OGS_ERR_UNSUPPORTED;
    }
}

int launch_reblend(const OgsRasterFwdArgs& a, const ImageState& is, hipStream_t s) {
    switch (a.C) {
        case 3: return reblend_c<3>(a, is, s);
        case 6: return reblend_c<6>(a, is, s);
        case 9: return reblend_c<9>(a, is, s);
        case 12: return reblend_c<12>(a, is, s);
        default: set_error("unsupported channel count C=%d", a.C); return OGS_ERR_UNSUPPORTED;
    }
}

int launch_tiny_blend(const OgsRasterFwdArgs& a, const GeomState& gs, const uint32_t* order, hipStream_t s) {
    switch (a.C) {
        case 3: return tiny_c<3>(a, gs, order, s);
        case 6: return tiny_c<6>(a, gs, order, s);
        case 9: return tiny_c<9>(a, gs, order, s);
        case 12: return tiny_c<12>(a, gs, order, s);
        default: set_error("unsupported channel count C=%d", a.C); return OGS_ERR_UNSUPPORTED;
    }
}

int launch_export_n_contrib(const OgsRasterFwdArgs& a, const ImageState& is, uint32_t* out, hipStream_t s) {
    switch (a.C) {
        case 3: return export_c<3>(a, is, out, s);
        case 6: return export_c<6>(a, is, out, s);
        case 9: return export_c<9>(a, is, out, s);
        case 12: return export_c<12>(a, is, out, s);
        default: set_error("unsupported channel count C=%d", a.C); return OGS_ERR_UNSUPPORTED;
    }
}

}
```

opengaussian_amd/csrc/capi.hip:

```cpp
#include <stdarg.h>
#include <stdlib.h>
#include <string.h>

#include <map>
#include <mutex>
#include <string>
#include <vector>

#include "ogs_common.h"

namespace ogs {

static thread_local char g_err[512] = "";

void set_error(const char* fmt, ...) {
    va_list ap;
    va_start(ap, fmt);
    vsnprintf(g_err, sizeof(g_err), fmt, ap);
    va_end(ap);
}

namespace {
struct ProfRec { const char* name; hipEvent_t start, stop; };
int g_prof_mode = 0;
char g_prof_prefix[64] = "blend_";
std::vector<ProfRec> g_prof;
std::vector<hipEvent_t> g_event_pool;
std::mutex g_prof_mu;
hipEvent_t take_event() {
    if (!g_event_pool.empty()) { hipEvent_t e = g_event_pool.back(); g_event_pool.pop_back(); return e; }
    hipEvent_t e = nullptr;
    (void)hipEventCreate(&e);
    return e;
}
}

ProfScope::ProfScope(const char* n, hipStream_t s) : name(n), stream(s), slot(-1) {
    if (g_prof_mode == 0) return;
    if (g_prof_mode == 2 && strncmp(n, g_prof_prefix, strlen(g_prof_prefix)) != 0) return;
    std::lock_guard<std::mutex> lk(g_prof_mu);
    ProfRec r{n, take_event(), take_event()};
    (void)hipEventRecord(r.start, s);
    g_prof.push_back(r);
    slot = (int)g_prof.size() - 1;
}
ProfScope::~ProfScope() {
    if (slot < 0) return;
    std::lock_guard<std::mutex> lk(g_prof_mu);
    (void)hipEventRecord(g_prof[slot].stop, stream);
}

namespace {
uint32_t* g_async_status = nullptr;
std::mutex g_async_mu;
}
uint32_t* async_status_word() {
    std::lock_guard<std::mutex> lk(g_async_mu);
    if (!g_async_status) {
        void* p = nullptr;
        const hipError_t e = hipHostMalloc(&p, 64, hipHostMallocMapped | hipHostMallocPortable);
        if (e != hipSuccess || !p) {
            set_error("hipHostMalloc of the async status word failed: %s", hipGetErrorString(e));
            return nullptr;
        }
        memset(p, 0, 64);
        g_async_status = static_cast<uint32_t*>(p);
    }
    return g_async_status;
}
int take_async_status() {
    std::lock_guard<std::mutex> lk(g_async_mu);
    if (!g_async_status) return 0;
    return (int)__atomic_exchange_n(g_async_status, 0u, __ATOMIC_ACQ_REL);
}
int check_async_status(const char* where) {
    const int st = take_async_status();
    if (st == 0) return OGS_OK;
    set_error("%s: a kernel of an earlier launch reported status 0x%x%s -- the results of the passes since the last check "
              "are not valid", where, st,
              (st & (int)kAsyncRadixSpin) ? " (one-launch radix pass: a look-back wait exceeded its bound)" : "");
    return OGS_ERR_DEVICE;
}

}
int ogs::blend_prefetch_lines() {
    static const int v = [] {
        const char* e = getenv("OGS_BLEND_PREFETCH");
        const int n = e ? atoi(e) : kPrefetchMax;
        const int lines = (n & 0xFF) > kPrefetchMax ? kPrefetchMax : (n & 0xFF);
#ifdef OGS_EXPERIMENTS
        return n < 0 ? 0 : (lines | (n & 0x300));
#else
        return n < 0 ? 0 : lines;
#endif
    }();
    return v;
}
namespace ogs {

static int bit_length(uint32_t v) {
    int n = 0;
    while (v) { ++n; v >>= 1; }
    return n;
}

static int validate_fwd(const OgsRasterFwdArgs* a, bool images = true) {
    if (!a) { set_error("args == NULL"); return OGS_ERR_INVALID_ARG; }
    if (a->P < 0 || a->W <= 0 || a->H <= 0) { set_error("bad sizes P=%d W=%d H=%d", a->P, a->W, a->H); return OGS_ERR_INVALID_ARG; }
    if (a->C != 3 && a->C != 6 && a->C != 9 && a->C != 12) { set_error("C=%d unsupported (3, 6, 9, 12)", a->C); return OGS_ERR_UNSUPPORTED; }
    if (a->shs == nullptr && a->colors_precomp == nullptr) {
        set_error("provide shs or colors_precomp"); return OGS_ERR_INVALID_ARG;
    }
    if (a->shs != nullptr && (a->colors_precomp != nullptr) != (a->C > 3)) {
        set_error("with shs: C == 3 and no colors_precomp, or C > 3 with colors_precomp holding the C-3 extra channels");
        return OGS_ERR_INVALID_ARG;
    }
    const bool sr = a->scales != nullptr && a->rotations != nullptr;
    if (sr == (a->cov3D_precomp != nullptr) || (a->scales != nullptr) != (a->rotations != nullptr)) {
        set_error("provide exactly one of (scales, rotations) / cov3D_precomp"); return OGS_ERR_INVALID_ARG;
    }
    if (a->shs) {
        if (a->sh_degree < 0 || a->sh_degree > 3 || a->sh_coeffs < (a->sh_degree + 1) * (a->sh_degree + 1)) {
            set_error("sh_degree=%d needs >= %d coefficients, got %d", a->sh_degree, (a->sh_degree + 1) * (a->sh_degree + 1), a->sh_coeffs);
            return OGS_ERR_INVALID_ARG;
        }
    }
    if (!a->bg || !a->viewmatrix || !a->projmatrix || !a->campos || (images && (!a->out_color || !a->out_depth || !a->out_alpha))) {
        set_error("NULL required pointer"); return OGS_ERR_INVALID_ARG;
    }
    if (a->P > 0 && (!a->means3D || !a->opacities || !a->radii || !a->geom_buffer || !a->geom_tmp)) {
        set_error("NULL required per-Gaussian pointer"); return OGS_ERR_INVALID_ARG;
    }
    if (a->num_groups < 0 || (a->num_groups > 1 && a->P > 0 && !a->group_ids)) {
        set_error("num_groups=%d needs group_ids", a->num_groups); return OGS_ERR_INVALID_ARG;
    }
    return OGS_OK;
}

}

using namespace ogs;

extern "C" {

int ogs_version(void) { return 400; }

int ogs_check_async_status(void) { return check_async_status("ogs_check_async_status"); }

int ogs_prof_enable(int on) {
    std::lock_guard<std::mutex> lk(g_prof_mu);
    for (auto& r : g_prof) { g_event_pool.push_back(r.start); g_event_pool.push_back(r.stop); }
    g_prof.clear();
    g_prof_mode = on;
    return OGS_OK;
}

int ogs_prof_filter(const char* prefix) {
    std::lock_guard<std::mutex> lk(g_prof_mu);
    if (!prefix || strlen(prefix) >= sizeof(g_prof_prefix)) { set_error("prof_filter: prefix NULL or longer than %zu", sizeof(g_prof_prefix) - 1); return OGS_ERR_INVALID_ARG; }
    strcpy(g_prof_prefix, prefix);
    return OGS_OK;
}

int ogs_prof_collect(char* buf, size_t n) {
    std::lock_guard<std::mutex> lk(g_prof_mu);
    std::map<std::string, std::pair<long, double>> agg;
    for (auto& r : g_prof) {
        OGS_HIP_CHECK(hipEventSynchronize(r.stop));
        float ms = 0.f;
        OGS_HIP_CHECK(hipEventElapsedTime(&ms, r.start, r.stop));
        auto& a = agg[r.name];
        a.first += 1;
        a.second += ms;
    }
    std::string out = "{";
    bool first = true;
    for (auto& kv : agg) {
        char line[384];
        std::string nm = kv.first;
        for (auto& ch : nm) if (ch == '"') ch = '\'';
        snprintf(line, sizeof(line), "%s\"%s\": {\"calls\": %ld, \"total_ms\": %.6f}", first ? "" : ", ", nm.c_str(),
                 kv.second.first, kv.second.second);
        out += line;
        first = false;
    }
    out += "}";
    if (!buf || out.size() + 1 > n) { set_error("prof_collect: buffer too small (%zu needed)", out.size() + 1); return OGS_ERR_SCRATCH_TOO_SMALL; }
    memcpy(buf, out.c_str(), out.size() + 1);
    return OGS_OK;
}
const char* ogs_last_error(void) { return g_err; }

size_t ogs_raster_geom_bytes(int32_t P, int32_t C) { return GeomState::bytes(P > 0 ? P : 1, C); }
size_t ogs_raster_geom_tmp_bytes(int32_t P) { return GeomTmp::bytes(P > 0 ? P : 1); }
size_t ogs_raster_image_bytes(int32_t W, int32_t H) { return ImageState::bytes(W, H); }
size_t ogs_raster_image_bytes_grouped(int32_t W, int32_t H, int32_t G) { return ImageState::bytes(W, H, num_groups_of(G)); }
size_t ogs_raster_binning_tmp_bytes(int64_t D, int32_t, int32_t) { return BinTmp::bytes(D > 0 ? D : 1); }
size_t ogs_raster_sorted_bytes(int64_t D, int32_t C) {
    return align_up((size_t)(D > 0 ? D : 1) * stream_vec4(C) * sizeof(float4));
}
size_t ogs_raster_quad_list_bytes(int64_t D) {
    return align_up((size_t)(5 * (D > 0 ? D : 1) + 2 * kQuadPad) * sizeof(uint32_t));
}
size_t ogs_raster_backward_tmp_bytes(int32_t P) { return align_up((size_t)(P > 0 ? P : 1) * 16 * sizeof(double)); }

int ogs_raster_forward_geometry(const OgsRasterFwdArgs* a, void* stream_, int64_t* num_rendered_host) {
    int rc = validate_fwd(a, false);
    if (rc != OGS_OK) return rc;
    hipStream_t s = static_cast<hipStream_t>(stream_);
    if (num_rendered_host) *num_rendered_host = 0;
    if (a->P == 0) return OGS_OK;
    rc = check_async_status("forward (entry)");
    if (rc != OGS_OK) return rc;
    const GeomState gs = GeomState::carve(a->geom_buffer, a->P, a->C);
    const GeomTmp gt = GeomTmp::carve(a->geom_tmp, a->P);
    if (a->P <= kSmallMaxP) {
        rc = launch_small_geometry(*a, gs, gt, s);
        if (rc != OGS_OK) return rc;
    } else {
        rc = launch_preprocess(*a, gs, gt, s);
        if (rc != OGS_OK) return rc;
        const bool sweep = radix_onesweep_enabled(a->P);
        if (sweep) {
            const int shifts[4] = {0, 8, 16, 24}, nbits[4] = {8, 8, 8, 8};
            rc = radix_sort_begin(gt.keys[0], a->P, nullptr, 4, shifts, nbits, gt.sort_tmp, s, a->debug, true);
            if (rc != OGS_OK) return rc;
        }
        for (int pass = 0; pass < 4; ++pass) {
            const int in = pass & 1, out = in ^ 1;
            const bool drop = pass == 0;
            const uint32_t* n_pass = drop ? nullptr : gt.visible();
            rc = sweep ? radix_sort_pass(pass, 4, gt.keys[in], gt.order[in], gt.keys[out], gt.order[out], a->P, 8 * pass, 8, gt.sort_tmp, s, a->debug, n_pass, drop, drop ? gt.visible() : nullptr)
                       : radix_pass(gt.keys[in], gt.order[in], gt.keys[out], gt.order[out], a->P, 8 * pass, 8, gt.sort_tmp, s, a->debug, n_pass, drop, drop ? gt.visible() : nullptr);
            if (rc != OGS_OK) return rc;
        }
        rc = exclusive_scan_u32(gt.tiles_touched, gt.order[0], gt.offsets, a->P, gt.num_rendered, gt.sort_tmp, s, a->debug, gt.visible());
        if (rc != OGS_OK) return rc;
    }
    if (num_rendered_host) {
        uint32_t d = 0;
        OGS_HIP_CHECK(hipMemcpyAsync(&d, gt.num_rendered, sizeof(uint32_t), hipMemcpyDeviceToHost, s));
        OGS_HIP_CHECK(hipStreamSynchronize(s));
        *num_rendered_host = (int64_t)d;
        rc = check_async_status("forward geometry phase");
        if (rc != OGS_OK) return rc;
    }
    return OGS_OK;
}

int ogs_raster_read_num_rendered_async(const OgsRasterFwdArgs* a, void* stream_, uint32_t* host_pinned) {
    if (!a || !host_pinned) { set_error("read_num_rendered_async: NULL pointer"); return OGS_ERR_INVALID_ARG; }
    if (a->P == 0) { *host_pinned = 0; return OGS_OK; }
    const GeomTmp gt = GeomTmp::carve(a->geom_tmp, a->P);
    OGS_HIP_CHECK(hipMemcpyAsync(host_pinned, gt.num_rendered, sizeof(uint32_t), hipMemcpyDeviceToHost,
                                 static_cast<hipStream_t>(stream_)));
    return OGS_OK;
}

static int render_impl(const OgsRasterFwdArgs* a, int64_t D, bool deferred, hipStream_t s,
                       const OgsGroupStatsArgs* stats = nullptr) {
    int rc = validate_fwd(a, stats == nullptr);
    if (rc != OGS_OK) return rc;
    if (!a->image_buffer) { set_error("image_buffer == NULL"); return OGS_ERR_INVALID_ARG; }
    const int G = num_groups_of(a->num_groups);
    const ImageState is = stats ? ImageState::carve_stats(a->image_buffer, a->W, a->H, G)
                                : ImageState::carve(a->image_buffer, a->W, a->H, G);
    const int gx = (a->W + kTile - 1) / kTile, gy = (a->H + kTile - 1) / kTile;
    const int64_t tiles = (int64_t)gx * gy * G;
    if (tiles >= (1ll << 31)) { set_error("%d groups x %d tiles exceed 2^31 virtual tiles", G, gx * gy); return OGS_ERR_UNSUPPORTED; }
    const GeomState gs = GeomState::carve(a->geom_buffer, a->P > 0 ? a->P : 1, a->C);
    if (D > 0) {
        if (!a->point_list || !a->binning_tmp) { set_error("point_list / binning_tmp == NULL with num_rendered=%lld", (long long)D); return OGS_ERR_INVALID_ARG; }
        if (D >= (1ll << 31)) { set_error("num_rendered=%lld exceeds 2^31", (long long)D); return OGS_ERR_UNSUPPORTED; }
        const GeomTmp gt = GeomTmp::carve(a->geom_tmp, a->P);
        const BinTmp bt = BinTmp::carve(a->binning_tmp, D);
        const int bits = bit_length((uint32_t)(tiles - 1));
        const int passes = bits == 0 ? 1 : (bits + 7) / 8;
        const int per = bits == 0 ? 1 : (bits + passes - 1) / passes;
        uint32_t* vbuf[2];
        vbuf[passes & 1] = a->point_list;
        vbuf[(passes & 1) ^ 1] = bt.vals;
        const uint32_t* n_dev = deferred ? gt.num_rendered : nullptr;
        const bool cull = a->full_binning == 0;
        const bool zero_in_dup = tiles <= (int64_t)a->P;
        rc = launch_duplicate(*a, gs, gt, bt.tile_keys[0], vbuf[0], (uint32_t)D, cull, s, zero_in_dup ? is.ranges : nullptr,
                              zero_in_dup ? (int)tiles : 0);
        if (rc != OGS_OK) return rc;
        const bool sweep = radix_onesweep_enabled(D);
        int shifts[4], nbits[4];
        for (int p = 0; p < passes; ++p) {
            shifts[p] = p * per;
            nbits[p] = (p == passes - 1) ? (bits == 0 ? 1 : bits - shifts[p]) : per;
        }
        if (passes == 2 && (bits & 1)) {
            nbits[0] = bits / 2; shifts[1] = nbits[0]; nbits[1] = bits - nbits[0];
        }
        if (sweep) {
            rc = radix_sort_begin(bt.tile_keys[0], D, n_dev, passes, shifts, nbits, bt.sort_tmp, s, a->debug, cull);
            if (rc != OGS_OK) return rc;
        }
        for (int p = 0; p < passes; ++p) {
            const int in = p & 1, out = in ^ 1;
            const bool drop = cull && p == 0;
            const uint32_t* n_pass = (cull && p > 0) ? bt.kept : n_dev;
            rc = sweep ? radix_sort_pass(p, passes, bt.tile_keys[in], vbuf[in], bt.tile_keys[out], vbuf[out], D, shifts[p], nbits[p], bt.sort_tmp, s, a->debug, n_pass, drop, drop ? bt.kept : nullptr)
                       : radix_pass(bt.tile_keys[in], vbuf[in], bt.tile_keys[out], vbuf[out], D, shifts[p], nbits[p], bt.sort_tmp, s, a->debug, n_pass, drop, drop ? bt.kept : nullptr);
            if (rc != OGS_OK) return rc;
        }
        rc = launch_tile_ranges(bt.tile_keys[passes & 1], D, is.ranges, tiles, s, a->debug, cull ? bt.kept : n_dev, zero_in_dup);
        if (rc != OGS_OK) return rc;
    } else {
        OGS_HIP_CHECK(hipMemsetAsync(is.ranges, 0, (size_t)tiles * sizeof(uint2), s));
    }
    if (stats) return launch_group_stats(*a, *stats, gs, is, s);
    if (!a->sorted_rec || !a->quad_list) { set_error("sorted_rec / quad_list == NULL"); return OGS_ERR_INVALID_ARG; }
    return launch_blend_forward(*a, gs, is, D, s);
}

int ogs_raster_forward_render(const OgsRasterFwdArgs* a, int64_t D, void* stream_) {
    return render_impl(a, D, false, static_cast<hipStream_t>(stream_));
}

size_t ogs_raster_stats_image_bytes(int32_t W, int32_t H, int32_t G) {
    return ImageState::stats_bytes(W > 0 ? W : 1, H > 0 ? H : 1, num_groups_of(G));
}
size_t ogs_raster_stats_tmp_bytes(int32_t G, int32_t L, int32_t C) {
    return align_up((size_t)num_groups_of(G) * (size_t)((L > 0 ? L : 0) + 1) * (size_t)(C > 0 ? C : 1) * sizeof(int64_t));
}

int ogs_raster_forward_group_stats(const OgsRasterFwdArgs* a, const OgsGroupStatsArgs* st, int64_t D, void* stream_) {
    if (!a || !st) { set_error("forward_group_stats: NULL argument"); return OGS_ERR_INVALID_ARG; }
    if (st->num_labels < 0) { set_error("forward_group_stats: num_labels=%d < 0", st->num_labels); return OGS_ERR_INVALID_ARG; }
    if (!st->labels || !st->max_alpha || !st->count || !st->feat_sum || !st->stats_tmp) {
        set_error("forward_group_stats: NULL labels / output / stats_tmp pointer"); return OGS_ERR_INVALID_ARG;
    }
    if (D < 0) { set_error("forward_group_stats: num_rendered=%lld < 0", (long long)D); return OGS_ERR_INVALID_ARG; }
    if (a->P == 0) D = 0;
    return render_impl(a, D, false, static_cast<hipStream_t>(stream_), st);
}

int ogs_raster_forward_render_deferred(const OgsRasterFwdArgs* a, int64_t capacity, void* stream_) {
    if (capacity <= 0) { set_error("forward_render_deferred: capacity must be > 0"); return OGS_ERR_INVALID_ARG; }
    return render_impl(a, capacity, true, static_cast<hipStream_t>(stream_));
}

int ogs_raster_forward_reblend(const OgsRasterFwdArgs* a, void* stream_) {
    if (!a) { set_error("args == NULL"); return OGS_ERR_INVALID_ARG; }
    if (a->P <= 0 || a->W <= 0 || a->H <= 0) { set_error("forward_reblend: bad sizes P=%d W=%d H=%d", a->P, a->W, a->H); return OGS_ERR_INVALID_ARG; }
    if (a->C != 3 && a->C != 6 && a->C != 9 && a->C != 12) { set_error("C=%d unsupported (3, 6, 9, 12)", a->C); return OGS_ERR_UNSUPPORTED; }
    if (a->num_groups > 1) { set_error("forward_reblend: grouped passes are not kept"); return OGS_ERR_UNSUPPORTED; }
    if (!a->colors_precomp || !a->bg || !a->out_color || !a->out_depth || !a->out_alpha || !a->image_buffer || !a->sorted_rec ||
        !a->quad_list) {
        set_error("forward_reblend: NULL required pointer (colors_precomp, bg, out_*, image_buffer, sorted_rec, quad_list)");
        return OGS_ERR_INVALID_ARG;
    }
    const int rc = check_async_status("forward_reblend (entry)");
    if (rc != OGS_OK) return rc;
    const ImageState is = ImageState::carve(a->image_buffer, a->W, a->H, 1);
    return launch_reblend(*a, is, static_cast<hipStream_t>(stream_));
}

int ogs_raster_compact_kept(int32_t W, int32_t H, int32_t C, const void* image_buffer, const void* sorted_rec, const void* quad_list,
                            void* new_image_buffer, void* new_sorted_rec, void* new_quad_list, void* stream_) {
    if (W <= 0 || H <= 0) { set_error("compact_kept: bad sizes W=%d H=%d", W, H); return OGS_ERR_INVALID_ARG; }
    if (!image_buffer || !sorted_rec || !quad_list || !new_image_buffer || !new_sorted_rec || !new_quad_list) {
        set_error("compact_kept: NULL pointer"); return OGS_ERR_INVALID_ARG;
    }
    const ImageState is_old = ImageState::carve(const_cast<void*>(image_buffer), W, H, 1);
    const ImageState is_new = ImageState::carve(new_image_buffer, W, H, 1);
    return launch_compact_kept(W, H, C, is_old, is_new, sorted_rec, quad_list, new_sorted_rec, new_quad_list,
                               static_cast<hipStream_t>(stream_));
}

size_t ogs_raster_tiny_max_points(void) { return (size_t)kTinyMaxP; }

int ogs_raster_forward_tiny(const OgsRasterFwdArgs* a, void* stream_) {
    int rc = validate_fwd(a);
    if (rc != OGS_OK) return rc;
    if (a->P <= 0 || a->P > kTinyMaxP) { set_error("forward_tiny: P=%d outside [1, %d]", a->P, kTinyMaxP); return OGS_ERR_INVALID_ARG; }
    if (a->num_groups > 1) { set_error("forward_tiny: grouped passes use the streaming path"); return OGS_ERR_UNSUPPORTED; }
    hipStream_t s = static_cast<hipStream_t>(stream_);
    const GeomState gs = GeomState::carve(a->geom_buffer, a->P, a->C);
    uint32_t* order = static_cast<uint32_t*>(a->geom_tmp);
    rc = launch_tiny_geometry(*a, gs, order, s);
    if (rc != OGS_OK) return rc;
    return launch_tiny_blend(*a, gs, order, s);
}

int ogs_raster_backward(const OgsRasterBwdArgs* a, void* stream_) {
    if (!a) { set_error("args == NULL"); return OGS_ERR_INVALID_ARG; }
    if (a->C != 3 && a->C != 6 && a->C != 9) { set_error("backward: C=%d unsupported (3, 6, 9)", a->C); return OGS_ERR_UNSUPPORTED; }
    if (a->P == 0) return OGS_OK;
    const bool feat_only = backward_is_features_only(*a);
    if (!a->dL_dcolor || !a->image_buffer || !a->bwd_tmp || !a->radii) {
        set_error("backward: NULL required pointer"); return OGS_ERR_INVALID_ARG;
    }
    if (!feat_only && (!a->geom_buffer || !a->bg || !a->means3D || !a->viewmatrix || !a->projmatrix || !a->campos)) {
        set_error("backward: NULL required pointer"); return OGS_ERR_INVALID_ARG;
    }
    if (!feat_only && a->num_rendered > 0 && !a->point_list) { set_error("backward: point_list == NULL"); return OGS_ERR_INVALID_ARG; }
    if ((int64_t)a->P * grad_stride(a->C) >= (1ll << 32)) {
        set_error("backward: P=%d exceeds the %lld Gaussians the 32-bit gradient-record offsets address", a->P,
                  (long long)((1ll << 32) / grad_stride(a->C)) - 1);
        return OGS_ERR_UNSUPPORTED;
    }
    {
        const int st = check_async_status("backward (entry)");
        if (st != OGS_OK) return st;
    }
    hipStream_t s = static_cast<hipStream_t>(stream_);
    const GeomState gs = GeomState::carve(const_cast<void*>(a->geom_buffer), a->P, a->C);
    if (a->num_groups < 0) { set_error("backward: num_groups=%d", a->num_groups); return OGS_ERR_INVALID_ARG; }
    const ImageState is = ImageState::carve(const_cast<void*>(a->image_buffer), a->W, a->H, num_groups_of(a->num_groups));
    void* grad_rec = a->bwd_tmp;
    const int rec_doubles = feat_only ? feat_grad_stride(a->C, a->shs ? 3 : 0) : grad_stride(a->C);
    OGS_HIP_CHECK(hipMemsetAsync(grad_rec, 0, (size_t)a->P * rec_doubles * sizeof(double), s));
    if (a->num_rendered > 0 && (!a->sorted_rec || !a->quad_list)) { set_error("backward: sorted_rec / quad_list == NULL"); return OGS_ERR_INVALID_ARG; }
    int rc = launch_blend_backward(*a, is, grad_rec, s);
    if (rc != OGS_OK) return rc;
    return launch_preprocess_backward(*a, gs, grad_rec, s);
}

int ogs_mark_visible(int32_t P, const float* means3D, const float* viewmatrix, const float*, uint8_t* present,
                     void* stream_) {
    if (P == 0) return OGS_OK;
    if (!means3D || !viewmatrix || !present) { set_error("mark_visible: NULL pointer"); return OGS_ERR_INVALID_ARG; }
    return launch_mark_visible(P, means3D, viewmatrix, present, static_cast<hipStream_t>(stream_));
}

int ogs_sh_grad_from_views(int32_t P, int32_t V, int32_t sh_degree, int32_t sh_coeffs, const float* means3D,
                           const float* campos, const float* dL_drgb, float* dL_dsh, void* stream_) {
    if (P == 0) return OGS_OK;
    if (P < 0 || V < 1 || sh_degree < 0 || sh_degree > 3 || sh_coeffs < (sh_degree + 1) * (sh_degree + 1)) {
        set_error("sh_grad_from_views: bad sizes P=%d V=%d degree=%d coeffs=%d", P, V, sh_degree, sh_coeffs);
        return OGS_ERR_INVALID_ARG;
    }
    if (!means3D || !campos || !dL_drgb || !dL_dsh) { set_error("sh_grad_from_views: NULL pointer"); return OGS_ERR_INVALID_ARG; }
    return launch_sh_grad_from_views(P, V, sh_degree, sh_coeffs, means3D, campos, dL_drgb, dL_dsh,
                                     static_cast<hipStream_t>(stream_));
}

int ogs_selftest_wave_fold16(const float* in, float* out, void* stream_) {
    if (!in || !out) { set_error("selftest: NULL pointer"); return OGS_ERR_INVALID_ARG; }
    return launch_wave_fold16_test(in, out, static_cast<hipStream_t>(stream_));
}

int ogs_selftest_tile_order(const uint32_t* ranges, int64_t vtiles, uint32_t* order, void* stream_) {
    if (!ranges || !order || vtiles <= 0) { set_error("selftest: NULL pointer / no tiles"); return OGS_ERR_INVALID_ARG; }
    return launch_tile_order_test(ranges, vtiles, order, static_cast<hipStream_t>(stream_));
}

size_t ogs_selftest_radix_tmp_bytes(int64_t n) { return sort_tmp_bytes(n > 0 ? n : 1); }

int ogs_selftest_radix_sort(uint32_t* keys0, uint32_t* vals0, uint32_t* keys1, uint32_t* vals1, int64_t n, int32_t key_bits,
                            int32_t variant, int32_t items, const uint32_t* n_dev, void* tmp, int32_t* result_buffer,
                            void* stream_) {
    if (!result_buffer) { set_error("selftest_radix_sort: NULL result_buffer"); return OGS_ERR_INVALID_ARG; }
    *result_buffer = 0;
    if (n <= 0) return OGS_OK;
    if (items != 0 && items != 4 && items != 16) { set_error("selftest_radix_sort: items=%d (0, 4 or 16)", items); return OGS_ERR_INVALID_ARG; }
    if (!keys0 || !vals0 || !keys1 || !vals1 || !tmp || key_bits < 1 || key_bits > 32) {
        set_error("selftest_radix_sort: bad arguments"); return OGS_ERR_INVALID_ARG;
    }
    hipStream_t s = static_cast<hipStream_t>(stream_);
    uint32_t* k[2] = {keys0, keys1};
    uint32_t* v[2] = {vals0, vals1};
    const int passes = (key_bits + 7) / 8, per = (key_bits + passes - 1) / passes;
    int shifts[4], nbits[4];
    for (int p = 0; p < passes; ++p) { shifts[p] = p * per; nbits[p] = p == passes - 1 ? key_bits - shifts[p] : per; }
    const bool sweep = (variant & 1) != 0, drop = (variant & 2) != 0;
    const int spin_limit = (variant & 4) ? 0 : -1;
    (void)take_async_status();
    uint32_t* kept = nullptr;
    if (drop) {
        OGS_HIP_CHECK(hipMalloc(&kept, sizeof(uint32_t)));
        OGS_HIP_CHECK(hipMemsetAsync(kept, 0xA5, sizeof(uint32_t), s));
    }
    int rc = OGS_OK;
    if (sweep) rc = radix_sort_begin(k[0], n, n_dev, passes, shifts, nbits, tmp, s, 0, drop, items);
    for (int p = 0; p < passes && rc == OGS_OK; ++p) {
        const int in = p & 1, out = in ^ 1;
        const bool d0 = drop && p == 0;
        const uint32_t* n_pass = (drop && p > 0) ? kept : n_dev;
        rc = sweep ? radix_sort_pass(p, passes, k[in], v[in], k[out], v[out], n, shifts[p], nbits[p], tmp, s, 0, n_pass, d0, d0 ? kept : nullptr, items, spin_limit)
                   : radix_pass(k[in], v[in], k[out], v[out], n, shifts[p], nbits[p], tmp, s, 0, n_pass, d0, d0 ? kept : nullptr);
    }
    uint32_t kept_host = 0;
    if (drop) {
        if (rc == OGS_OK && hipMemcpyAsync(&kept_host, kept, sizeof(uint32_t), hipMemcpyDeviceToHost, s) != hipSuccess) rc = OGS_ERR_HIP;
        (void)hipStreamSynchronize(s);
        (void)hipFree(kept);
    } else {
        (void)hipStreamSynchronize(s);
    }
    if (rc != OGS_OK) return rc;
    *result_buffer = (passes & 1) | (drop ? (int32_t)(kept_host << 1) : 0);
    return check_async_status("selftest_radix_sort");
}

int ogs_raster_export_binning(const OgsRasterFwdArgs* a, int64_t D, uint64_t* keys_out, uint32_t* ranges_out,
                              uint32_t* n_contrib_out, void* stream_) {
    if (!a) { set_error("args == NULL"); return OGS_ERR_INVALID_ARG; }
    hipStream_t s = static_cast<hipStream_t>(stream_);
    const int G = num_groups_of(a->num_groups);
    const ImageState is = ImageState::carve(a->image_buffer, a->W, a->H, G);
    const int gx = (a->W + kTile - 1) / kTile, gy = (a->H + kTile - 1) / kTile;
    if (keys_out && D > 0) {
        const GeomState gs = GeomState::carve(a->geom_buffer, a->P, a->C);
        int rc = launch_export_keys(is.ranges, gx * gy * G, a->point_list, gs.rec, rec_vec4(a->C), keys_out, s);
        if (rc != OGS_OK) return rc;
    }
    if (ranges_out)
        OGS_HIP_CHECK(hipMemcpyAsync(ranges_out, is.ranges, (size_t)gx * gy * G * sizeof(uint2), hipMemcpyDeviceToDevice, s));
    if (n_contrib_out) {
        if (D > 0) {
            int rc = launch_export_n_contrib(*a, is, n_contrib_out, s);
            if (rc != OGS_OK) return rc;
        } else {
            OGS_HIP_CHECK(hipMemsetAsync(n_contrib_out, 0, (size_t)G * a->W * a->H * sizeof(uint32_t), s));
        }
    }
    return OGS_OK;
}

}
```

opengaussian_amd/csrc/ogs_common.h:

```cpp
#pragma once

#include <hip/hip_runtime.h>
#include <stdint.h>
#include <stddef.h>
#include <stdio.h>

#include "../../include/ogs_raster.h"

namespace ogs {

constexpr int kTile = OGS_TILE;
constexpr int kBlock = 256;
constexpr int kWave = 64;
constexpr int kTinyMaxP = 256;
constexpr int kSmallMaxP = 1024;

void set_error(const char* fmt, ...);

#define OGS_HIP_CHECK(expr)                                                              \
    do {                                                                                 \
        hipError_t _e = (expr);                                                          \
        if (_e != hipSuccess) {                                                          \
            ogs::set_error("%s failed: %s (%s:%d)", #expr, hipGetErrorString(_e), __FILE__, __LINE__); \
            return OGS_ERR_HIP;                                                          \
        }                                                                                \
    } while (0)

#define OGS_LAUNCH_CHECK(debug, stream)                                                  \
    do {                                                                                 \
        OGS_HIP_CHECK(hipGetLastError());                                                \
        if (debug) OGS_HIP_CHECK(hipStreamSynchronize(stream));                          \
    } while (0)

constexpr uint32_t kAsyncRadixSpin = 1u;
uint32_t* async_status_word();
int take_async_status();
int check_async_status(const char* where);

struct ProfScope {
    const char* name;
    hipStream_t stream;
    int slot;
    ProfScope(const char* name, hipStream_t s);
    ~ProfScope();
};
#define OGS_LAUNCH(kernel, grid, block, lds, stream, ...)                      \
    do {                                                                       \
        ogs::ProfScope _ps(#kernel, stream);                                   \
        hipLaunchKernelGGL(kernel, grid, block, lds, stream, __VA_ARGS__);     \
    } while (0)

#define OGS_LAUNCH_NAMED(name, kernel, grid, block, lds, stream, ...)          \
    do {                                                                       \
        ogs::ProfScope _ps(name, stream);                                      \
        hipLaunchKernelGGL(kernel, grid, block, lds, stream, __VA_ARGS__);     \
    } while (0)
template <int C>
constexpr const char* chan_name(const char* const (&names)[4]) {
    return C == 3 ? names[0] : C == 6 ? names[1] : C == 9 ? names[2] : names[3];
}

constexpr size_t kAlign = 256;
inline size_t align_up(size_t v, size_t a = kAlign) { return (v + a - 1) / a * a; }

struct Carver {
    char* base;
    size_t off = 0;
    explicit Carver(void* p) : base(static_cast<char*>(p)) {}
    template <typename T>
    T* take(size_t n) {
        T* r = reinterpret_cast<T*>(base ? base + off : nullptr);
        off = align_up(off + n * sizeof(T));
        return r;
    }
};

__host__ __device__ constexpr int rec_vec4(int C) { return 2 + (C + 3) / 4; }

__host__ __device__ constexpr int stream_vec4(int C) { return (8 + C + 1 + 3) / 4; }

constexpr int kQuadPad = 16;
template <int C>
inline float4* stream_base(void* buf) { return static_cast<float4*>(buf); }
inline uint32_t* quad_base(void* buf) { return static_cast<uint32_t*>(buf) + kQuadPad; }
constexpr float kFar = 3.0e18f;
constexpr float kFarTest = 1.0e18f;

typedef float f8 __attribute__((ext_vector_type(8)));
template <int C>
struct StreamRec {
    static constexpr int NF4 = stream_vec4(C) - 2;
    f8 g;
    float4 f[NF4];
    __device__ __forceinline__ void load(const float* __restrict__ p) {
        g = *reinterpret_cast<const f8*>(p);
#pragma unroll
        for (int k = 0; k < NF4; ++k) f[k] = *reinterpret_cast<const float4*>(p + 8 + 4 * k);
    }
    __device__ __forceinline__ float feat(int c) const {
        const float4 v = f[c >> 2];
        return (c & 3) == 0 ? v.x : (c & 3) == 1 ? v.y : (c & 3) == 2 ? v.z : v.w;
    }
};

constexpr int kSlotDepth = 9, kSlotMoments = 10;
__host__ __device__ constexpr int grad_stride(int C) { return (C + 7 <= 16) ? 16 : 32; }
__host__ __device__ constexpr int feat_grad_stride(int C, int F0) { return (C - F0 <= 8) ? 8 : grad_stride(C); }

struct GeomState {
    float4* rec;
    uint32_t* clamped;
    static GeomState carve(void* p, int P, int C) {
        Carver c(p);
        GeomState g;
        g.rec = c.take<float4>((size_t)P * rec_vec4(C));
        g.clamped = c.take<uint32_t>(P);
        return g;
    }
    static size_t bytes(int P, int C) {
        Carver c(nullptr);
        c.take<float4>((size_t)P * rec_vec4(C));
        c.take<uint32_t>(P);
        return c.off;
    }
};

struct ImageState {
    uint2* ranges;
    uint32_t* n_contrib;
    uint32_t* qcount;
    float* final_T;
    uint32_t* tile_order;
    static ImageState carve(void* p, int W, int H, int G = 1) {
        Carver c(p);
        ImageState s;
        const size_t tiles = (size_t)G * ((W + kTile - 1) / kTile) * ((H + kTile - 1) / kTile);
        s.ranges = c.take<uint2>(tiles);
        s.n_contrib = c.take<uint32_t>((size_t)G * W * H);
        s.qcount = c.take<uint32_t>(tiles * 5);
        s.final_T = c.take<float>((size_t)G * W * H);
        s.tile_order = c.take<uint32_t>(tiles);
        return s;
    }
    static size_t bytes(int W, int H, int G = 1) {
        Carver c(nullptr);
        const size_t tiles = (size_t)G * ((W + kTile - 1) / kTile) * ((H + kTile - 1) / kTile);
        c.take<uint2>(tiles);
        c.take<uint32_t>((size_t)G * W * H);
        c.take<uint32_t>(tiles * 5);
        c.take<float>((size_t)G * W * H);
        c.take<uint32_t>(tiles);
        return c.off;
    }
    static ImageState carve_stats(void* p, int W, int H, int G) {
        Carver c(p);
        ImageState s{};
        const size_t tiles = (size_t)G * ((W + kTile - 1) / kTile) * ((H + kTile - 1) / kTile);
        s.ranges = c.take<uint2>(tiles);
        s.tile_order = c.take<uint32_t>(tiles);
        return s;
    }
    static size_t stats_bytes(int W, int H, int G) {
        Carver c(nullptr);
        const size_t tiles = (size_t)G * ((W + kTile - 1) / kTile) * ((H + kTile - 1) / kTile);
        c.take<uint2>(tiles);
        c.take<uint32_t>(tiles);
        return c.off;
    }
};
const uint32_t* launch_tile_order(const ImageState& is, int64_t vtiles, int P, hipStream_t s, int debug);
const uint32_t* tile_order_of(const ImageState& is, int64_t vtiles, int P);
int launch_export_n_contrib(const OgsRasterFwdArgs& a, const ImageState& is, uint32_t* out, hipStream_t s);

constexpr int kSortItemsLarge = 8;
inline int sort_items_for(int64_t n) { return n <= (int64_t)(3 << 20) ? 4 : kSortItemsLarge; }
inline int sort_blocks_for(int64_t n) {
    const int64_t tile = (int64_t)kBlock * sort_items_for(n);
    return (int)((n + tile - 1) / tile);
}
size_t scan_tmp_bytes(int64_t n);
size_t sort_tmp_bytes(int64_t n);

int exclusive_scan_u32(const uint32_t* in, const uint32_t* gather, uint32_t* out, int64_t n,
                       uint32_t* total, void* tmp, hipStream_t stream, int debug, const uint32_t* n_dev = nullptr);
constexpr uint32_t kDropKey = 0xFFFFFFFFu;
bool radix_onesweep_enabled(int64_t n);
int radix_sort_begin(const uint32_t* keys, int64_t n, const uint32_t* n_dev, int npass, const int* shifts, const int* bits,
                     void* tmp, hipStream_t stream, int debug, bool drop = false, int items = 0);
int radix_sort_pass(int pass, int npass, const uint32_t* keys_in, const uint32_t* vals_in, uint32_t* keys_out,
                    uint32_t* vals_out, int64_t n, int shift, int bits, void* tmp, hipStream_t stream, int debug,
                    const uint32_t* n_dev = nullptr, bool drop = false, uint32_t* kept_out = nullptr, int items = 0,
                    int spin_limit = -1);
int radix_pass(const uint32_t* keys_in, const uint32_t* vals_in, uint32_t* keys_out, uint32_t* vals_out,
               int64_t n, int shift, int bits, void* tmp, hipStream_t stream, int debug,
               const uint32_t* n_dev = nullptr, bool drop = false, uint32_t* kept_out = nullptr);

struct GeomTmp {
    uint32_t* tiles_touched;
    uint32_t* keys[2];
    uint32_t* order[2];
    uint32_t* offsets;
    uint32_t* num_rendered;
    void* sort_tmp;
    uint32_t* visible() const { return num_rendered + 1; }
    static GeomTmp carve(void* p, int P) {
        Carver c(p);
        GeomTmp g;
        g.tiles_touched = c.take<uint32_t>(P);
        g.keys[0] = c.take<uint32_t>(P);
        g.keys[1] = c.take<uint32_t>(P);
        g.order[0] = c.take<uint32_t>(P);
        g.order[1] = c.take<uint32_t>(P);
        g.offsets = c.take<uint32_t>(P);
        g.num_rendered = c.take<uint32_t>(64);
        g.sort_tmp = c.take<char>(sort_tmp_bytes(P));
        return g;
    }
    static size_t bytes(int P) {
        Carver c(nullptr);
        for (int i = 0; i < 6; ++i) c.take<uint32_t>(P);
        c.take<uint32_t>(64);
        c.take<char>(sort_tmp_bytes(P));
        return c.off;
    }
};

struct BinTmp {
    uint32_t* tile_keys[2];
    uint32_t* vals;
    uint32_t* kept;
    void* sort_tmp;
    static BinTmp carve(void* p, int64_t D) {
        Carver c(p);
        BinTmp b;
        b.tile_keys[0] = c.take<uint32_t>(D);
        b.tile_keys[1] = c.take<uint32_t>(D);
        b.vals = c.take<uint32_t>(D);
        b.kept = c.take<uint32_t>(1);
        b.sort_tmp = c.take<char>(sort_tmp_bytes(D));
        return b;
    }
    static size_t bytes(int64_t D) {
        Carver c(nullptr);
        for (int i = 0; i < 3; ++i) c.take<uint32_t>(D);
        c.take<uint32_t>(1);
        c.take<char>(sort_tmp_bytes(D));
        return c.off;
    }
};

int launch_preprocess(const OgsRasterFwdArgs& a, const GeomState& gs, const GeomTmp& gt, hipStream_t s);
int launch_tiny_geometry(const OgsRasterFwdArgs& a, const GeomState& gs, uint32_t* order, hipStream_t s);
int launch_small_geometry(const OgsRasterFwdArgs& a, const GeomState& gs, const GeomTmp& gt, hipStream_t s);
int launch_tiny_blend(const OgsRasterFwdArgs& a, const GeomState& gs, const uint32_t* order, hipStream_t s);
int launch_reblend(const OgsRasterFwdArgs& a, const ImageState& is, hipStream_t s);
int launch_compact_kept(int W, int H, int C, const ImageState& is_old, const ImageState& is_new, const void* old_rec,
                        const void* old_quad, void* new_rec, void* new_quad, hipStream_t s);
int launch_duplicate(const OgsRasterFwdArgs& a, const GeomState& gs, const GeomTmp& gt, uint32_t* tile_keys,
                     uint32_t* vals, uint32_t capacity, bool drop_unreachable, hipStream_t s, uint2* zero_ranges = nullptr,
                     int n_zero = 0);
int launch_tile_ranges(const uint32_t* tile_keys_sorted, int64_t D, uint2* ranges, int64_t tiles, hipStream_t s,
                       int debug, const uint32_t* n_dev = nullptr, bool already_zeroed = false);
inline int num_groups_of(int g) { return g > 1 ? g : 1; }
int launch_group_stats(const OgsRasterFwdArgs& a, const OgsGroupStatsArgs& st, const GeomState& gs, const ImageState& is,
                       hipStream_t s);
int launch_blend_forward(const OgsRasterFwdArgs& a, const GeomState& gs, const ImageState& is, int64_t D,
                         hipStream_t s);
int launch_blend_backward(const OgsRasterBwdArgs& a, const ImageState& is, void* grad_rec, hipStream_t s);
int launch_preprocess_backward(const OgsRasterBwdArgs& a, const GeomState& gs, const void* grad_rec, hipStream_t s);
inline bool backward_is_features_only(const OgsRasterBwdArgs& a) {
    return a.dL_dcolors != nullptr && a.colors_precomp != nullptr && !a.dL_dmeans2D && !a.dL_dopacity &&
           !a.dL_dmeans3D && !a.dL_dcov3D && !a.dL_dsh && !a.dL_dscales && !a.dL_drotations && !a.dL_dsh_rgb;
}
int launch_sh_grad_from_views(int P, int V, int sh_degree, int sh_coeffs, const float* means3D, const float* campos,
                              const float* dL_drgb, float* dL_dsh, hipStream_t s);
int launch_wave_fold16_test(const float* in, float* out, hipStream_t s);
int launch_tile_order_test(const uint32_t* ranges, int64_t vtiles, uint32_t* order, hipStream_t s);
int launch_mark_visible(int P, const float* means3D, const float* viewmatrix, uint8_t* present, hipStream_t s);
int launch_export_keys(const uint2* ranges, int tiles, const uint32_t* point_list, const float4* rec, int recv4,
                       uint64_t* keys_out, hipStream_t s);

__device__ __forceinline__ float blend_power(float a2, float b2, float c2, float dx, float dy) {
    const float u = fmaf(b2, dy, a2 * dx);
    return fmaf(c2 * dy, dy, u * dx);
}

constexpr int kPrefetchMax = 4;
struct RecordPrefetch {
    uint32_t v[kPrefetchMax];
    __device__ __forceinline__ void issue(const float* __restrict__ tile_records, int n_tile, int rec_floats, int tid,
                                          int lines) {
        const uint32_t total = (uint32_t)n_tile * (uint32_t)rec_floats;
#pragma unroll
        for (int k = 0; k < kPrefetchMax; ++k) {
            v[k] = 0u;
            const uint32_t off = ((uint32_t)(k * kBlock + tid)) * 32u;
            if (k < lines && off < total) v[k] = __float_as_uint(tile_records[off]);
        }
    }
    __device__ __forceinline__ void retire(uint32_t* __restrict__ sink, int never) const {
        const uint32_t x = v[0] ^ v[1] ^ v[2] ^ v[3];
        if (never < 0 && x == 0x7FC12345u) sink[0] = x;
    }
};
int blend_prefetch_lines();

constexpr float kThrMargin = 0.01f;
constexpr int kReachBit = 31;
constexpr uint32_t kGidMask = (1u << kReachBit) - 1u;
__device__ __forceinline__ float max_power_in_box(float A, float B, float Cc, float nbA, float nbC, float xlo, float xhi,
                                                  float ylo, float yhi) {
    if (xlo <= 0.f && xhi >= 0.f && ylo <= 0.f && yhi >= 0.f) return 0.f;
    auto q = [&](float dx, float dy) { return -0.5f * (A * dx * dx + Cc * dy * dy) - B * dx * dy; };
    float m = q(xlo, fminf(fmaxf(nbC * xlo, ylo), yhi));
    m = fmaxf(m, q(xhi, fminf(fmaxf(nbC * xhi, ylo), yhi)));
    m = fmaxf(m, q(fminf(fmaxf(nbA * ylo, xlo), xhi), ylo));
    m = fmaxf(m, q(fminf(fmaxf(nbA * yhi, xlo), xhi), yhi));
    const float X = fmaxf(fabsf(xlo), fabsf(xhi)), Y = fmaxf(fabsf(ylo), fabsf(yhi));
    return m + 8e-7f * (0.5f * (A * X * X + Cc * Y * Y) + fabsf(B) * X * Y);
}
__device__ __forceinline__ float max_power_in_box(float A, float B, float Cc, float xlo, float xhi, float ylo,
                                                  float yhi) {
    return max_power_in_box(A, B, Cc, -B / A, -B / Cc, xlo, xhi, ylo, yhi);
}

__device__ __forceinline__ void wait_scalar_loads() {
    __builtin_amdgcn_sched_barrier(0);
    __builtin_amdgcn_s_waitcnt(0xC07F);
    __builtin_amdgcn_sched_barrier(0);
}
__device__ __forceinline__ int lane_id() { return threadIdx.x & (kWave - 1); }
__device__ __forceinline__ void lds_barrier() { asm volatile("s_waitcnt lgkmcnt(0)\n\ts_barrier" ::: "memory"); }

}
```

opengaussian_amd/csrc/preprocess_fwd.hip:

```cpp
#include "ogs_common.h"

namespace ogs {

namespace {

__constant__ const float kC0 = 0.28209479177387814f;
__constant__ const float kC1 = 0.4886025119029199f;
__constant__ const float kC2[5] = {1.0925484305920792f, -1.0925484305920792f, 0.31539156525252005f,
                                   -1.0925484305920792f, 0.5462742152960396f};
__constant__ const float kC3[7] = {-0.5900435899266435f, 2.890611442640554f, -0.4570457994644658f,
                                   0.3731763325901154f, -0.4570457994644658f, 1.445305721320277f,
                                   -0.5900435899266435f};

struct Cam {
    float V[16];
    float M[16];
    float campos[3];
};

__device__ __forceinline__ void cov3d_from_scale_rot(const float* __restrict__ scales,
                                                     const float* __restrict__ rots, int idx, float mod,
                                                     float cov[6]) {
    const float sx = mod * scales[3 * idx + 0], sy = mod * scales[3 * idx + 1], sz = mod * scales[3 * idx + 2];
    const float4 q = reinterpret_cast<const float4*>(rots)[idx];
    const float r = q.x, x = q.y, y = q.z, z = q.w;
    const float R00 = 1.f - 2.f * (y * y + z * z), R01 = 2.f * (x * y - r * z), R02 = 2.f * (x * z + r * y);
    const float R10 = 2.f * (x * y + r * z), R11 = 1.f - 2.f * (x * x + z * z), R12 = 2.f * (y * z - r * x);
    const float R20 = 2.f * (x * z - r * y), R21 = 2.f * (y * z + r * x), R22 = 1.f - 2.f * (x * x + y * y);
    const float M00 = R00 * sx, M01 = R01 * sy, M02 = R02 * sz;
    const float M10 = R10 * sx, M11 = R11 * sy, M12 = R12 * sz;
    const float M20 = R20 * sx, M21 = R21 * sy, M22 = R22 * sz;
    cov[0] = M00 * M00 + M01 * M01 + M02 * M02;
    cov[1] = M00 * M10 + M01 * M11 + M02 * M12;
    cov[2] = M00 * M20 + M01 * M21 + M02 * M22;
    cov[3] = M10 * M10 + M11 * M11 + M12 * M12;
    cov[4] = M10 * M20 + M11 * M21 + M12 * M22;
    cov[5] = M20 * M20 + M21 * M21 + M22 * M22;
}

__device__ __forceinline__ void sh_to_rgb(int idx, int deg, int M, const float* __restrict__ shs, float px,
                                          float py, float pz, const float* campos, float rgb[3],
                                          uint32_t& clamped) {
    const float* sh = shs + (size_t)idx * M * 3;
    float dx = px - campos[0], dy = py - campos[1], dz = pz - campos[2];
    const float ln = sqrtf(dx * dx + dy * dy + dz * dz);
    const float x = dx / ln, y = dy / ln, z = dz / ln;
    float res[3];
#pragma unroll
    for (int c = 0; c < 3; ++c) res[c] = kC0 * sh[c];
    if (deg > 0) {
#pragma unroll
        for (int c = 0; c < 3; ++c)
            res[c] = res[c] - kC1 * y * sh[3 + c] + kC1 * z * sh[6 + c] - kC1 * x * sh[9 + c];
        if (deg > 1) {
            const float xx = x * x, yy = y * y, zz = z * z, xy = x * y, yz = y * z, xz = x * z;
#pragma unroll
            for (int c = 0; c < 3; ++c)
                res[c] = res[c] + kC2[0] * xy * sh[12 + c] + kC2[1] * yz * sh[15 + c] +
                         kC2[2] * (2.f * zz - xx - yy) * sh[18 + c] + kC2[3] * xz * sh[21 + c] +
                         kC2[4] * (xx - yy) * sh[24 + c];
            if (deg > 2) {
#pragma unroll
                for (int c = 0; c < 3; ++c)
                    res[c] = res[c] + kC3[0] * y * (3.f * xx - yy) * sh[27 + c] + kC3[1] * xy * z * sh[30 + c] +
                             kC3[2] * y * (4.f * zz - xx - yy) * sh[33 + c] +
                             kC3[3] * z * (2.f * zz - 3.f * xx - 3.f * yy) * sh[36 + c] +
                             kC3[4] * x * (4.f * zz - xx - yy) * sh[39 + c] + kC3[5] * z * (xx - yy) * sh[42 + c] +
                             kC3[6] * x * (xx - 3.f * yy) * sh[45 + c];
            }
        }
    }
    clamped = 0;
#pragma unroll
    for (int c = 0; c < 3; ++c) {
        res[c] = res[c] + 0.5f;
        if (res[c] < 0.f) clamped |= 1u << c;
        rgb[c] = fmaxf(res[c], 0.f);
    }
}

template <int C>
__device__ __forceinline__ uint32_t preprocess_one(
    int idx, int W, int H, int sh_degree, int sh_coeffs, float tanfovx, float tanfovy, float focal_x, float focal_y,
    float scale_modifier, const float* __restrict__ means3D, const float* __restrict__ colors_precomp,
    const float* __restrict__ shs, const float* __restrict__ opacities, const float* __restrict__ scales,
    const float* __restrict__ rotations, const float* __restrict__ cov3D_precomp, const float* __restrict__ viewmatrix,
    const float* __restrict__ projmatrix, const float* __restrict__ campos, float4* __restrict__ rec_row,
    uint32_t* __restrict__ clamped_out, int32_t* __restrict__ radii, uint32_t* __restrict__ tiles_touched,
    const int32_t* __restrict__ group_ids, int num_groups) {
    constexpr int NV = rec_vec4(C);
    float V[16], M[16];
#pragma unroll
    for (int i = 0; i < 16; ++i) { V[i] = viewmatrix[i]; M[i] = projmatrix[i]; }

    const float x = means3D[3 * idx + 0], y = means3D[3 * idx + 1], z = means3D[3 * idx + 2];
    const float opacity = opacities[idx];

    float feat[(C + 3) / 4 * 4];
#pragma unroll
    for (int c = 0; c < (C + 3) / 4 * 4; ++c) feat[c] = 0.f;
    uint32_t clamped = 0;

    int radius = 0;
    uint32_t touched = 0;
    float pxl = 0.f, pyl = 0.f, depth = 0.f, cA = 0.f, cB = 0.f, cC = 0.f;

    const float pvx = V[0] * x + V[4] * y + V[8] * z + V[12];
    const float pvy = V[1] * x + V[5] * y + V[9] * z + V[13];
    const float pvz = V[2] * x + V[6] * y + V[10] * z + V[14];
    bool ok = pvz > 0.2f;
    if (group_ids != nullptr) ok = ok && (uint32_t)group_ids[idx] < (uint32_t)num_groups;
    if (ok) {
        const float hx = M[0] * x + M[4] * y + M[8] * z + M[12];
        const float hy = M[1] * x + M[5] * y + M[9] * z + M[13];
        const float hw = M[3] * x + M[7] * y + M[11] * z + M[15];
        const float p_w = 1.0f / (hw + 0.0000001f);
        const float projx = hx * p_w, projy = hy * p_w;
        float cov[6];
        if (cov3D_precomp != nullptr) {
#pragma unroll
            for (int i = 0; i < 6; ++i) cov[i] = cov3D_precomp[6 * idx + i];
        } else {
            cov3d_from_scale_rot(scales, rotations, idx, scale_modifier, cov);
        }
        const float limx = 1.3f * tanfovx, limy = 1.3f * tanfovy;
        const float txtz = pvx / pvz, tytz = pvy / pvz;
        const float tx = fminf(limx, fmaxf(-limx, txtz)) * pvz;
        const float ty = fminf(limy, fmaxf(-limy, tytz)) * pvz;
        const float tz = pvz;
        const float J00 = focal_x / tz;
        const float J02 = -(focal_x * tx) / (tz * tz);
        const float J11 = focal_y / tz;
        const float J12 = -(focal_y * ty) / (tz * tz);
        const float T00 = J00 * V[0] + J02 * V[2];
        const float T01 = J00 * V[4] + J02 * V[6];
        const float T02 = J00 * V[8] + J02 * V[10];
        const float T10 = J11 * V[1] + J12 * V[2];
        const float T11 = J11 * V[5] + J12 * V[6];
        const float T12 = J11 * V[9] + J12 * V[10];
        const float a0 = T00 * cov[0] + T01 * cov[1] + T02 * cov[2];
        const float a1 = T00 * cov[1] + T01 * cov[3] + T02 * cov[4];
        const float a2 = T00 * cov[2] + T01 * cov[4] + T02 * cov[5];
        const float b0 = T10 * cov[0] + T11 * cov[1] + T12 * cov[2];
        const float b1 = T10 * cov[1] + T11 * cov[3] + T12 * cov[4];
        const float b2 = T10 * cov[2] + T11 * cov[4] + T12 * cov[5];
        const float ca = a0 * T00 + a1 * T01 + a2 * T02 + 0.3f;
        const float cb = a0 * T10 + a1 * T11 + a2 * T12;
        const float cc = b0 * T10 + b1 * T11 + b2 * T12 + 0.3f;
        const float det = ca * cc - cb * cb;
        ok = det != 0.f;
        if (ok) {
            const float det_inv = 1.f / det;
            cA = cc * det_inv;
            cB = -cb * det_inv;
            cC = ca * det_inv;
            const float mid = 0.5f * (ca + cc);
            const float sq = sqrtf(fmaxf(0.1f, mid * mid - det));
            const float lam = fmaxf(mid + sq, mid - sq);
            float rad_f = ceilf(3.f * sqrtf(lam));
            if (!(fabsf(rad_f) < 3.0e38f)) rad_f = 0.f;
            const int my_radius = (int)rad_f;
            pxl = ((projx + 1.0f) * (float)W - 1.0f) * 0.5f;
            pyl = ((projy + 1.0f) * (float)H - 1.0f) * 0.5f;
            const int gx = (W + kTile - 1) / kTile, gy = (H + kTile - 1) / kTile;
            const float rf = (float)my_radius;
            auto tr = [](float v) -> int {
                if (!(fabsf(v) < 3.0e38f)) v = 0.f;
                v = fminf(fmaxf(v, -2.0e9f), 2.0e9f);
                return (int)v;
            };
            const int rminx = min(gx, max(0, tr((pxl - rf) / (float)kTile)));
            const int rminy = min(gy, max(0, tr((pyl - rf) / (float)kTile)));
            const int rmaxx = min(gx, max(0, tr((pxl + rf + (float)kTile - 1.0f) / (float)kTile)));
            const int rmaxy = min(gy, max(0, tr((pyl + rf + (float)kTile - 1.0f) / (float)kTile)));
            const int area = (rmaxx - rminx) * (rmaxy - rminy);
            ok = area != 0 && my_radius > 0;
            if (ok) {
                radius = my_radius;
                touched = (uint32_t)area;
                depth = pvz;
            }
        }
    }

    const int coff = shs != nullptr ? 3 : 0;
    if (colors_precomp != nullptr) {
#pragma unroll
        for (int c = 0; c < C; ++c)
            if (c >= coff) feat[c] = colors_precomp[(size_t)idx * (C - coff) + (c - coff)];
    }
    if (shs != nullptr && ok) {
        float rgb[3];
        float cp[3] = {campos[0], campos[1], campos[2]};
        sh_to_rgb(idx, sh_degree, sh_coeffs, shs, x, y, z, cp, rgb, clamped);
        feat[0] = rgb[0]; feat[1] = rgb[1]; feat[2] = rgb[2];
    }

    if (!ok) { pxl = 0.f; pyl = 0.f; cA = cB = cC = 0.f; depth = 0.f; }

    float4* r = rec_row;
    r[0] = make_float4(pxl, pyl, depth, __int_as_float(radius));
    r[1] = make_float4(cA, cB, cC, opacity);
#pragma unroll
    for (int v = 0; v < NV - 2; ++v) r[2 + v] = make_float4(feat[4 * v], feat[4 * v + 1], feat[4 * v + 2], feat[4 * v + 3]);
    clamped_out[idx] = clamped;
    radii[idx] = radius;
    if (tiles_touched) tiles_touched[idx] = touched;
    return ok ? __float_as_uint(depth) : 0xFFFFFFFFu;
}

template <int C>
__global__ __launch_bounds__(kBlock) void preprocess_kernel(
    int P, int W, int H, int sh_degree, int sh_coeffs, float tanfovx, float tanfovy, float focal_x, float focal_y,
    float scale_modifier, const float* __restrict__ means3D, const float* __restrict__ colors_precomp,
    const float* __restrict__ shs, const float* __restrict__ opacities, const float* __restrict__ scales,
    const float* __restrict__ rotations, const float* __restrict__ cov3D_precomp, const float* __restrict__ viewmatrix,
    const float* __restrict__ projmatrix, const float* __restrict__ campos, float4* __restrict__ rec,
    uint32_t* __restrict__ clamped_out, int32_t* __restrict__ radii, uint32_t* __restrict__ tiles_touched,
    uint32_t* __restrict__ depth_keys, uint32_t* __restrict__ order, const int32_t* __restrict__ group_ids,
    int num_groups) {
    constexpr int NV = rec_vec4(C);
    __shared__ float4 s_rec[kBlock * NV];
    const int tid = threadIdx.x;
    const int idx = blockIdx.x * kBlock + tid;
    if (idx < P) {
        depth_keys[idx] = preprocess_one<C>(idx, W, H, sh_degree, sh_coeffs, tanfovx, tanfovy, focal_x, focal_y, scale_modifier,
                                            means3D, colors_precomp, shs, opacities, scales, rotations, cov3D_precomp, viewmatrix,
                                            projmatrix, campos, s_rec + tid * NV, clamped_out, radii, tiles_touched, group_ids,
                                            num_groups);
        order[idx] = (uint32_t)idx;
    }
    __syncthreads();
    const size_t row0 = (size_t)blockIdx.x * kBlock;
    const int n4 = min(kBlock, P - (int)row0) * NV;
    float4* __restrict__ out = rec + row0 * NV;
    for (int e = tid; e < n4; e += kBlock) out[e] = s_rec[e];
}

template <int C>
__global__ __launch_bounds__(kTinyMaxP) void tiny_geometry_kernel(
    int P, int W, int H, int sh_degree, int sh_coeffs, float tanfovx, float tanfovy, float focal_x, float focal_y,
    float scale_modifier, const float* __restrict__ means3D, const float* __restrict__ colors_precomp,
    const float* __restrict__ shs, const float* __restrict__ opacities, const float* __restrict__ scales,
    const float* __restrict__ rotations, const float* __restrict__ cov3D_precomp, const float* __restrict__ viewmatrix,
    const float* __restrict__ projmatrix, const float* __restrict__ campos, float4* __restrict__ rec,
    uint32_t* __restrict__ clamped_out, int32_t* __restrict__ radii, uint32_t* __restrict__ order) {
    __shared__ uint32_t s_key[kTinyMaxP];
    const int idx = threadIdx.x;
    uint32_t key = 0xFFFFFFFFu;
    if (idx < P)
        key = preprocess_one<C>(idx, W, H, sh_degree, sh_coeffs, tanfovx, tanfovy, focal_x, focal_y, scale_modifier, means3D,
                                colors_precomp, shs, opacities, scales, rotations, cov3D_precomp, viewmatrix, projmatrix,
                                campos, rec + (size_t)idx * rec_vec4(C), clamped_out, radii, nullptr, nullptr, 0);
    s_key[idx] = key;
    __syncthreads();
    if (idx < P) {
        int rank = 0;
        for (int j = 0; j < P; ++j) {
            const uint32_t kj = s_key[j];
            rank += (kj < key || (kj == key && j < idx)) ? 1 : 0;
        }
        order[rank] = (uint32_t)idx;
    }
}

template <int C>
__global__ __launch_bounds__(kSmallMaxP) void small_geometry_kernel(
    int P, int W, int H, int sh_degree, int sh_coeffs, float tanfovx, float tanfovy, float focal_x, float focal_y,
    float scale_modifier, const float* __restrict__ means3D, const float* __restrict__ colors_precomp,
    const float* __restrict__ shs, const float* __restrict__ opacities, const float* __restrict__ scales,
    const float* __restrict__ rotations, const float* __restrict__ cov3D_precomp, const float* __restrict__ viewmatrix,
    const float* __restrict__ projmatrix, const float* __restrict__ campos, float4* __restrict__ rec,
    uint32_t* __restrict__ clamped_out, int32_t* __restrict__ radii, uint32_t* __restrict__ order,
    uint32_t* __restrict__ offsets, uint32_t* __restrict__ num_rendered, const int32_t* __restrict__ group_ids,
    int num_groups) {
    __shared__ uint32_t s_key[kSmallMaxP];
    __shared__ uint32_t s_touched[kSmallMaxP];
    __shared__ uint32_t s_sorted[kSmallMaxP];
    __shared__ uint32_t s_wave[kSmallMaxP / kWave];
    const int idx = threadIdx.x, lane = idx & 63, wave = idx >> 6;
    uint32_t key = 0xFFFFFFFFu;
    s_touched[idx] = 0u;
    if (idx < P)
        key = preprocess_one<C>(idx, W, H, sh_degree, sh_coeffs, tanfovx, tanfovy, focal_x, focal_y, scale_modifier, means3D,
                                colors_precomp, shs, opacities, scales, rotations, cov3D_precomp, viewmatrix, projmatrix,
                                campos, rec + (size_t)idx * rec_vec4(C), clamped_out, radii, s_touched, group_ids, num_groups);
    s_key[idx] = key;
    __syncthreads();
    int rank = idx;
    if (idx < P) {
        rank = 0;
        for (int j = 0; j < P; ++j) {
            const uint32_t kj = s_key[j];
            rank += (kj < key || (kj == key && j < idx)) ? 1 : 0;
        }
        order[rank] = (uint32_t)idx;
    }
    s_sorted[rank] = s_touched[idx];
    __syncthreads();
    const uint32_t v = s_sorted[idx];
    uint32_t incl = v;
#pragma unroll
    for (int d = 1; d < kWave; d <<= 1) {
        const uint32_t o = __shfl_up(incl, d, kWave);
        if (lane >= d) incl += o;
    }
    if (lane == kWave - 1) s_wave[wave] = incl;
    __syncthreads();
    uint32_t before = 0u, total = 0u;
#pragma unroll
    for (int w = 0; w < kSmallMaxP / kWave; ++w) {
        const uint32_t t = s_wave[w];
        if (w < wave) before += t;
        total += t;
    }
    if (idx < P) offsets[idx] = before + incl - v;
    if (idx == 0) { num_rendered[0] = total; num_rendered[1] = (uint32_t)P; }
}

template <int NV>
__global__ __launch_bounds__(kBlock) void duplicate_kernel(int P_cap, const uint32_t* __restrict__ n_visible, int W, int H,
                                                           const float4* __restrict__ rec,
                                                           const uint32_t* __restrict__ order,
                                                           const uint32_t* __restrict__ offsets,
                                                           uint32_t* __restrict__ tile_keys,
                                                           uint32_t* __restrict__ vals, uint32_t capacity,
                                                           const int32_t* __restrict__ group_ids, bool drop_unreachable,
                                                           uint2* __restrict__ zero_ranges, int n_zero) {
    __shared__ uint32_t s_off[kBlock];
    __shared__ uint32_t s_gid[kBlock];
    __shared__ uint32_t s_rect[kBlock];
    __shared__ uint32_t s_first, s_total;
    __shared__ uint32_t s_key0[kBlock];
    __shared__ float4 s_ctr[kBlock];
    __shared__ float4 s_con[kBlock];
    const int tid = threadIdx.x;
    const int r = blockIdx.x * kBlock + tid;
    if (zero_ranges != nullptr && r < n_zero) zero_ranges[r] = make_uint2(0u, 0u);
    const int P = min(P_cap, (int)*n_visible);
    if ((int)blockIdx.x * kBlock >= P) return;
    const int gx = (W + kTile - 1) / kTile, gy = (H + kTile - 1) / kTile;
    uint32_t off = 0, cnt = 0, gid = 0, rect = 1u << 24, key0 = 0;
    float4 ctr = make_float4(0.f, 0.f, 0.f, 0.f);
    float4 con = make_float4(1.f, 1.f, 0.f, 0.f);
    if (r < P) {
        gid = order[r];
        off = offsets[r];
        if (group_ids != nullptr) key0 = (uint32_t)max(group_ids[gid], 0) * (uint32_t)(gx * gy);
        const float4 a = rec[(size_t)gid * NV];
        const int radius = __float_as_int(a.w);
        if (radius > 0) {
            const float4 b = rec[(size_t)gid * NV + 1];
            ctr = make_float4(a.x, a.y, -(__logf(255.0f * b.w) + kThrMargin), b.y);
            con = make_float4(b.x, b.z, -b.y / b.x, -b.y / b.z);
            const float rf = (float)radius;
            auto tr = [](float v) -> int {
                if (!(fabsf(v) < 3.0e38f)) v = 0.f;
                v = fminf(fmaxf(v, -2.0e9f), 2.0e9f);
                return (int)v;
            };
            const int rminx = min(gx, max(0, tr((a.x - rf) / (float)kTile)));
            const int rminy = min(gy, max(0, tr((a.y - rf) / (float)kTile)));
            const int rmaxx = min(gx, max(0, tr((a.x + rf + (float)kTile - 1.0f) / (float)kTile)));
            const int rmaxy = min(gy, max(0, tr((a.y + rf + (float)kTile - 1.0f) / (float)kTile)));
            const int w = rmaxx - rminx, h = rmaxy - rminy;
            if (w > 0 && h > 0) {
                cnt = (uint32_t)(w * h);
                rect = (uint32_t)rminx | ((uint32_t)rminy << 12) | ((uint32_t)min(w, 255) << 24);
                if (w > 255) {
                    uint32_t o = off;
                    for (int ty = rminy; ty < rmaxy; ++ty)
                        for (int tx = rminx; tx < rmaxx; ++tx) {
                            if (o < capacity) { tile_keys[o] = key0 + (uint32_t)(ty * gx + tx); vals[o] = gid | (1u << kReachBit); }
                            ++o;
                        }
                    rect |= 0u;
                    gid |= 0x80000000u;
                }
            }
        }
    }
    if (tid == 0) s_first = off;
    __syncthreads();
    const uint32_t first = s_first;
    s_off[tid] = (r < P) ? off - first : 0xFFFFFFFFu;
    s_gid[tid] = gid;
    s_rect[tid] = rect;
    s_key0[tid] = key0;
    s_ctr[tid] = ctr;
    s_con[tid] = con;
    const int last = min(P - 1 - blockIdx.x * kBlock, kBlock - 1);
    if (tid == last) s_total = off - first + cnt;
    __syncthreads();
    const uint32_t total = s_total;
    for (uint32_t j = tid; j < total; j += kBlock) {
        int lo = 0, hi = kBlock;
#pragma unroll
        for (int step = kBlock / 2; step >= 1; step >>= 1) {
            const int mid = lo + step;
            if (mid < hi && s_off[mid] <= j) lo = mid;
        }
        const uint32_t g = s_gid[lo];
        if (g & 0x80000000u) continue;
        const uint32_t rc = s_rect[lo];
        const uint32_t local = j - s_off[lo];
        const uint32_t w = rc >> 24;
        const uint32_t row = local / w, col = local - row * w;
        const uint32_t o = first + j;
        if (o < capacity) {
            const uint32_t tx = (rc & 0xFFFu) + col, ty = (rc >> 12 & 0xFFFu) + row;
            const uint32_t key = s_key0[lo] + ty * (uint32_t)gx + tx;
            const float4 c = s_ctr[lo];
            const float4 k = s_con[lo];
            const float X0 = (float)(tx * kTile), Y0 = (float)(ty * kTile);
            const float m = max_power_in_box(k.x, c.w, k.y, k.z, k.w, c.x - X0 - 15.f, c.x - X0, c.y - Y0 - 15.f, c.y - Y0);
            const bool reach = m >= c.z;
            tile_keys[o] = (drop_unreachable && !reach) ? kDropKey : key;
            vals[o] = g | ((reach ? 1u : 0u) << kReachBit);
        }
    }
}

__global__ __launch_bounds__(kBlock) void mark_visible_kernel(int P, const float* __restrict__ means3D,
                                                              const float* __restrict__ V,
                                                              uint8_t* __restrict__ present) {
    const int idx = blockIdx.x * kBlock + threadIdx.x;
    if (idx >= P) return;
    const float x = means3D[3 * idx], y = means3D[3 * idx + 1], z = means3D[3 * idx + 2];
    const float pvz = V[2] * x + V[6] * y + V[10] * z + V[14];
    present[idx] = pvz > 0.2f ? 1 : 0;
}

template <int C>
int launch_preprocess_c(const OgsRasterFwdArgs& a, const GeomState& gs, const GeomTmp& gt, hipStream_t s) {
    const float focal_x = (float)a.W / (2.0f * a.tanfovx);
    const float focal_y = (float)a.H / (2.0f * a.tanfovy);
    const int grid = (a.P + kBlock - 1) / kBlock;
    static constexpr const char* const kNames[4] = {"preprocess_kernel<3>", "preprocess_kernel<6>", "preprocess_kernel<9>", "preprocess_kernel<12>"};
    OGS_LAUNCH_NAMED(chan_name<C>(kNames), preprocess_kernel<C>, dim3(grid), dim3(kBlock), 0, s, a.P, a.W, a.H, a.sh_degree, a.sh_coeffs,
                       a.tanfovx, a.tanfovy, focal_x, focal_y, a.scale_modifier, a.means3D, a.colors_precomp, a.shs,
                       a.opacities, a.scales, a.rotations, a.cov3D_precomp, a.viewmatrix, a.projmatrix, a.campos,
                       gs.rec, gs.clamped, a.radii, gt.tiles_touched, gt.keys[0], gt.order[0],
                       a.num_groups > 1 ? a.group_ids : (const int32_t*)nullptr, a.num_groups);
    OGS_LAUNCH_CHECK(a.debug, s);
    return OGS_OK;
}

template <int C>
int launch_tiny_geometry_c(const OgsRasterFwdArgs& a, const GeomState& gs, uint32_t* order, hipStream_t s) {
    const float focal_x = (float)a.W / (2.0f * a.tanfovx);
    const float focal_y = (float)a.H / (2.0f * a.tanfovy);
    OGS_LAUNCH(tiny_geometry_kernel<C>, dim3(1), dim3(kTinyMaxP), 0, s, a.P, a.W, a.H, a.sh_degree, a.sh_coeffs, a.tanfovx,
               a.tanfovy, focal_x, focal_y, a.scale_modifier, a.means3D, a.colors_precomp, a.shs, a.opacities, a.scales,
               a.rotations, a.cov3D_precomp, a.viewmatrix, a.projmatrix, a.campos, gs.rec, gs.clamped, a.radii, order);
    OGS_LAUNCH_CHECK(a.debug, s);
    return OGS_OK;
}

template <int C>
int launch_small_geometry_c(const OgsRasterFwdArgs& a, const GeomState& gs, const GeomTmp& gt, hipStream_t s) {
    const float focal_x = (float)a.W / (2.0f * a.tanfovx);
    const float focal_y = (float)a.H / (2.0f * a.tanfovy);
    OGS_LAUNCH(small_geometry_kernel<C>, dim3(1), dim3(kSmallMaxP), 0, s, a.P, a.W, a.H, a.sh_degree, a.sh_coeffs, a.tanfovx,
               a.tanfovy, focal_x, focal_y, a.scale_modifier, a.means3D, a.colors_precomp, a.shs, a.opacities, a.scales,
               a.rotations, a.cov3D_precomp, a.viewmatrix, a.projmatrix, a.campos, gs.rec, gs.clamped, a.radii, gt.order[0],
               gt.offsets, gt.num_rendered, a.num_groups > 1 ? a.group_ids : (const int32_t*)nullptr, a.num_groups);
    OGS_LAUNCH_CHECK(a.debug, s);
    return OGS_OK;
}

}

int launch_small_geometry(const OgsRasterFwdArgs& a, const GeomState& gs, const GeomTmp& gt, hipStream_t s) {
    switch (a.C) {
        case 3: return launch_small_geometry_c<3>(a, gs, gt, s);
        case 6: return launch_small_geometry_c<6>(a, gs, gt, s);
        case 9: return launch_small_geometry_c<9>(a, gs, gt, s);
        case 12: return launch_small_geometry_c<12>(a, gs, gt, s);
        default: set_error("unsupported channel count C=%d (3, 6, 9 or 12)", a.C); return OGS_ERR_UNSUPPORTED;
    }
}

int launch_tiny_geometry(const OgsRasterFwdArgs& a, const GeomState& gs, uint32_t* order, hipStream_t s) {
    switch (a.C) {
        case 3: return launch_tiny_geometry_c<3>(a, gs, order, s);
        case 6: return launch_tiny_geometry_c<6>(a, gs, order, s);
        case 9: return launch_tiny_geometry_c<9>(a, gs, order, s);
        case 12: return launch_tiny_geometry_c<12>(a, gs, order, s);
        default: set_error("unsupported channel count C=%d (3, 6, 9 or 12)", a.C); return OGS_ERR_UNSUPPORTED;
    }
}

int launch_preprocess(const OgsRasterFwdArgs& a, const GeomState& gs, const GeomTmp& gt, hipStream_t s) {
    switch (a.C) {
        case 3: return launch_preprocess_c<3>(a, gs, gt, s);
        case 6: return launch_preprocess_c<6>(a, gs, gt, s);
        case 9: return launch_preprocess_c<9>(a, gs, gt, s);
        case 12: return launch_preprocess_c<12>(a, gs, gt, s);
        default: set_error("unsupported channel count C=%d (3, 6, 9 or 12)", a.C); return OGS_ERR_UNSUPPORTED;
    }
}

int launch_duplicate(const OgsRasterFwdArgs& a, const GeomState& gs, const GeomTmp& gt, uint32_t* tile_keys,
                     uint32_t* vals, uint32_t capacity, bool drop_unreachable, hipStream_t s, uint2* zero_ranges, int n_zero) {
    if (n_zero > a.P) { set_error("duplicate: %d ranges to clear with %d threads", n_zero, a.P); return OGS_ERR_INVALID_ARG; }
    const int grid = (a.P + kBlock - 1) / kBlock;
    const int32_t* grp = a.num_groups > 1 ? a.group_ids : nullptr;
    if ((a.W + kTile - 1) / kTile > 4095 || (a.H + kTile - 1) / kTile > 4095) {
        set_error("image %dx%d exceeds 4095 tiles per side", a.W, a.H);
        return OGS_ERR_UNSUPPORTED;
    }
    switch (rec_vec4(a.C)) {
        case 3: OGS_LAUNCH(duplicate_kernel<3>, dim3(grid), dim3(kBlock), 0, s, a.P, (const uint32_t*)gt.visible(), a.W, a.H, gs.rec, gt.order[0], gt.offsets, tile_keys, vals, capacity, grp, drop_unreachable, zero_ranges, n_zero); break;
        case 4: OGS_LAUNCH(duplicate_kernel<4>, dim3(grid), dim3(kBlock), 0, s, a.P, (const uint32_t*)gt.visible(), a.W, a.H, gs.rec, gt.order[0], gt.offsets, tile_keys, vals, capacity, grp, drop_unreachable, zero_ranges, n_zero); break;
        case 5: OGS_LAUNCH(duplicate_kernel<5>, dim3(grid), dim3(kBlock), 0, s, a.P, (const uint32_t*)gt.visible(), a.W, a.H, gs.rec, gt.order[0], gt.offsets, tile_keys, vals, capacity, grp, drop_unreachable, zero_ranges, n_zero); break;
        default: set_error("unsupported record size"); return OGS_ERR_UNSUPPORTED;
    }
    OGS_LAUNCH_CHECK(a.debug, s);
    return OGS_OK;
}

int launch_mark_visible(int P, const float* means3D, const float* viewmatrix, uint8_t* present, hipStream_t s) {
    const int grid = (P + kBlock - 1) / kBlock;
    OGS_LAUNCH(mark_visible_kernel, dim3(grid), dim3(kBlock), 0, s, P, means3D, viewmatrix, present);
    OGS_LAUNCH_CHECK(0, s);
    return OGS_OK;
}

}
```

Baseline: 1394 Mpix/s.

## Replace global depth sort with per-tile depth sort after tile binning

For single-group scenes above the small-P threshold, the preprocess no longer produces a global depth order. Duplicated entries are emitted in index order and binned by tile only, and a new kernel then radix-sorts each tile's list by depth in LDS: a wave-level sort for short lists, a block-level sort for medium ones, and a chunked multi-pass block sort through scratch for long ones. The aim is to drop the global depth sort over all Gaussians in favour of many small local sorts. The cost is an extra kernel whose speed depends on the distribution of tile list lengths, plus atomic-heavy ranking in LDS.

```diff
diff --git a/include/ogs_raster.h b/include/ogs_raster.h
--- a/include/ogs_raster.h
+++ b/include/ogs_raster.h
@@ -119,6 +119,8 @@
 size_t ogs_raster_tiny_max_points(void);
 int ogs_raster_forward_tiny(const OgsRasterFwdArgs* args, void* stream);
 
+size_t ogs_raster_tile_sort_capacity(int32_t level);
+
 int ogs_raster_forward_reblend(const OgsRasterFwdArgs* args, void* stream);
 
 int ogs_raster_compact_kept(int32_t W, int32_t H, int32_t C, const void* image_buffer, const void* sorted_rec,
diff --git a/opengaussian_amd/_lib.py b/opengaussian_amd/_lib.py
--- a/opengaussian_amd/_lib.py
+++ b/opengaussian_amd/_lib.py
@@ -82,6 +82,7 @@
     "ogs_raster_forward_group_stats": (C.c_int, [C.POINTER(OgsRasterFwdArgs), C.POINTER(OgsGroupStatsArgs), C.c_int64, _vp]),
     "ogs_raster_backward": (C.c_int, [C.POINTER(OgsRasterBwdArgs), _vp]),
     "ogs_raster_tiny_max_points": (C.c_size_t, []),
+    "ogs_raster_tile_sort_capacity": (C.c_size_t, [C.c_int32]),
     "ogs_raster_forward_tiny": (C.c_int, [C.POINTER(OgsRasterFwdArgs), _vp]),
     "ogs_raster_forward_reblend": (C.c_int, [C.POINTER(OgsRasterFwdArgs), _vp]),
     "ogs_raster_compact_kept": (C.c_int, [C.c_int32, C.c_int32, C.c_int32, _vp, _vp, _vp, _vp, _vp, _vp, _vp]),
diff --git a/opengaussian_amd/csrc/binning.hip b/opengaussian_amd/csrc/binning.hip
--- a/opengaussian_amd/csrc/binning.hip
+++ b/opengaussian_amd/csrc/binning.hip
@@ -455,6 +455,295 @@
     }
 }
 
+constexpr int kTileSortWaves = kBlock / kWave;
+struct TileSortLds {
+    uint32_t hist[kTileSortWaves][256];
+    uint32_t dig_start[256];
+    uint32_t base[256];
+    uint32_t scan_sums[4];
+    uint32_t red[2];
+    uint2 range[kTileSortWaves];
+    uint32_t kv[2 * kTileSortCap];
+};
+typedef __attribute__((address_space(3))) volatile uint32_t LdsWord;
+typedef __attribute__((address_space(3))) unsigned long long LdsMask;
+__device__ __forceinline__ LdsWord* lds_words(uint32_t* p) { return (LdsWord*)p; }
+__device__ __forceinline__ LdsMask* wave_masks(TileSortLds& sm, int wave) { return (LdsMask*)(sm.kv + wave * 2 * kWaveSortCap); }
+
+__device__ __forceinline__ void wave_rank_clear(LdsWord* hist, LdsMask* masks) {
+    const int lane = threadIdx.x & (kWave - 1);
+#pragma unroll
+    for (int j = 0; j < 4; ++j) {
+        hist[lane + j * kWave] = 0u;
+        __hip_atomic_store(&masks[lane + j * kWave], 0ull, __ATOMIC_SEQ_CST, __HIP_MEMORY_SCOPE_WAVEFRONT);
+    }
+    __builtin_amdgcn_wave_barrier();
+}
+
+__device__ __forceinline__ void wave_rank(LdsWord* hist, LdsMask* masks, const uint32_t (&key)[kTileSortItems],
+                                          uint32_t (&rank)[kTileSortItems], int ipl, int first, int m, int shift,
+                                          uint32_t mask) {
+    const int lane = threadIdx.x & (kWave - 1);
+    const unsigned long long me = 1ull << lane;
+#pragma unroll
+    for (int i = 0; i < kTileSortItems; ++i) {
+        if (i >= ipl) continue;
+        const bool valid = first + i * kWave + lane < m;
+        const uint32_t d = (key[i] >> shift) & mask;
+        if (valid) __hip_atomic_fetch_or(&masks[d], me, __ATOMIC_SEQ_CST, __HIP_MEMORY_SCOPE_WAVEFRONT);
+        __builtin_amdgcn_wave_barrier();
+        const unsigned long long peers =
+            valid ? __hip_atomic_load(&masks[d], __ATOMIC_SEQ_CST, __HIP_MEMORY_SCOPE_WAVEFRONT) : 0ull;
+        const uint32_t r = __builtin_amdgcn_mbcnt_hi((uint32_t)(peers >> 32), __builtin_amdgcn_mbcnt_lo((uint32_t)peers, 0u));
+        uint32_t pre = 0;
+        if (valid) pre = hist[d];
+        __builtin_amdgcn_wave_barrier();
+        if (valid && r == 0) {
+            hist[d] = pre + (uint32_t)__popcll(peers);
+            __hip_atomic_store(&masks[d], 0ull, __ATOMIC_SEQ_CST, __HIP_MEMORY_SCOPE_WAVEFRONT);
+        }
+        __builtin_amdgcn_wave_barrier();
+        rank[i] = pre + r;
+    }
+}
+
+__device__ __forceinline__ void load_items(const uint32_t* __restrict__ list, const uint32_t* __restrict__ depth_keys,
+                                           uint32_t (&key)[kTileSortItems], uint32_t (&val)[kTileSortItems], int ipl, int first,
+                                           int m) {
+#pragma unroll
+    for (int i = 0; i < kTileSortItems; ++i) {
+        if (i >= ipl) continue;
+        val[i] = list[min(first + i * kWave, m - 1)];
+    }
+#pragma unroll
+    for (int i = 0; i < kTileSortItems; ++i) {
+        if (i >= ipl) continue;
+        key[i] = depth_keys[val[i] & kGidMask];
+    }
+}
+
+__device__ __forceinline__ uint32_t tile_sort_rank(TileSortLds& sm, const uint32_t (&key)[kTileSortItems],
+                                                   uint32_t (&rank)[kTileSortItems], int ipl, int chunk, int m, int shift,
+                                                   uint32_t mask) {
+    const int tid = threadIdx.x, wave = tid >> 6;
+    LdsWord* hist = lds_words(sm.hist[wave]);
+    LdsMask* masks = wave_masks(sm, wave);
+    wave_rank_clear(hist, masks);
+    wave_rank(hist, masks, key, rank, ipl, wave * chunk, m, shift, mask);
+    __syncthreads();
+    uint32_t run_len = 0;
+#pragma unroll
+    for (int w = 0; w < kTileSortWaves; ++w) {
+        const uint32_t t = sm.hist[w][tid];
+        sm.hist[w][tid] = run_len;
+        run_len += t;
+    }
+    uint32_t total;
+    sm.dig_start[tid] = block_exclusive_scan(run_len, total, sm.scan_sums);
+    __syncthreads();
+    return run_len;
+}
+
+__device__ __forceinline__ void wave_sort_list(TileSortLds& sm, uint32_t* __restrict__ seg, int n,
+                                               const uint32_t* __restrict__ depth_keys) {
+    const int lane = threadIdx.x & (kWave - 1), wave = threadIdx.x >> 6;
+    LdsWord* wk = lds_words(sm.kv + wave * 2 * kWaveSortCap);
+    LdsWord* wv = wk + kWaveSortCap;
+    LdsWord* hist = lds_words(sm.hist[wave]);
+    LdsMask* masks = wave_masks(sm, wave);
+    uint32_t key[kTileSortItems], val[kTileSortItems], rank[kTileSortItems];
+    const int ipl = (n + kWave - 1) / kWave;
+    load_items(seg, depth_keys, key, val, ipl, lane, n);
+    uint32_t k_and = 0xFFFFFFFFu, k_or = 0u;
+#pragma unroll
+    for (int i = 0; i < kTileSortItems; ++i) {
+        if (i >= ipl) continue;
+        k_and &= key[i];
+        k_or |= key[i];
+    }
+#pragma unroll
+    for (int d = 32; d >= 1; d >>= 1) {
+        k_and &= (uint32_t)__shfl_xor((int)k_and, d, kWave);
+        k_or |= (uint32_t)__shfl_xor((int)k_or, d, kWave);
+    }
+    const uint32_t diff = (uint32_t)__builtin_amdgcn_readfirstlane((int)(k_and ^ k_or));
+    if (diff == 0u) return;
+    const int lo = __builtin_ctz(diff), hi = 31 - __builtin_clz(diff);
+    const int npass = (hi - lo + 8) / 8;
+    const int per = (hi - lo + npass) / npass;
+    for (int p = 0; p < npass; ++p) {
+        const int shift = lo + p * per, bits = min(per, hi + 1 - shift);
+        const uint32_t mask = (1u << bits) - 1u;
+        wave_rank_clear(hist, masks);
+        wave_rank(hist, masks, key, rank, ipl, 0, n, shift, mask);
+        uint32_t c[4], sum = 0;
+#pragma unroll
+        for (int j = 0; j < 4; ++j) { c[j] = hist[4 * lane + j]; sum += c[j]; }
+        uint32_t run = wave_inclusive_scan(sum) - sum;
+#pragma unroll
+        for (int j = 0; j < 4; ++j) { hist[4 * lane + j] = run; run += c[j]; }
+        __builtin_amdgcn_wave_barrier();
+#pragma unroll
+        for (int i = 0; i < kTileSortItems; ++i) {
+            if (i >= ipl) continue;
+            rank[i] += hist[(key[i] >> shift) & mask];
+        }
+#pragma unroll
+        for (int i = 0; i < kTileSortItems; ++i) {
+            if (i >= ipl) continue;
+            if (i * kWave + lane < n) {
+                wk[rank[i]] = key[i];
+                wv[rank[i]] = val[i];
+            }
+        }
+        __builtin_amdgcn_wave_barrier();
+        if (p + 1 < npass) {
+#pragma unroll
+            for (int i = 0; i < kTileSortItems; ++i) {
+                if (i >= ipl) continue;
+                const int e = min(i * kWave + lane, n - 1);
+                key[i] = wk[e];
+                val[i] = wv[e];
+            }
+            __builtin_amdgcn_wave_barrier();
+        }
+    }
+    for (int j = lane; j < n; j += kWave) seg[j] = wv[j];
+}
+
+__device__ __forceinline__ void block_sort_list(TileSortLds& sm, uint32_t* __restrict__ seg, uint32_t* __restrict__ alt, int n,
+                                                const uint32_t* __restrict__ depth_keys) {
+    const int tid = threadIdx.x, lane = tid & 63, wave = tid >> 6;
+    const bool in_lds = n <= kTileSortCap;
+    uint32_t key[kTileSortItems], val[kTileSortItems], rank[kTileSortItems];
+    __syncthreads();
+    if (tid < 2) sm.red[tid] = tid == 0 ? 0xFFFFFFFFu : 0u;
+    uint32_t k_and = 0xFFFFFFFFu, k_or = 0u;
+    const int ipl0 = (min(n, kTileSortCap) + kBlock - 1) / kBlock, chunk0 = ipl0 * kWave;
+    if (in_lds) {
+        load_items(seg, depth_keys, key, val, ipl0, wave * chunk0 + lane, n);
+#pragma unroll
+        for (int i = 0; i < kTileSortItems; ++i) {
+            if (i >= ipl0) continue;
+            k_and &= key[i];
+            k_or |= key[i];
+        }
+    } else {
+        for (int j = tid; j < n; j += kBlock) {
+            const uint32_t k = depth_keys[seg[j] & kGidMask];
+            k_and &= k;
+            k_or |= k;
+        }
+    }
+#pragma unroll
+    for (int d = 32; d >= 1; d >>= 1) {
+        k_and &= (uint32_t)__shfl_xor((int)k_and, d, kWave);
+        k_or |= (uint32_t)__shfl_xor((int)k_or, d, kWave);
+    }
+    __syncthreads();
+    if (lane == 0) { atomicAnd(&sm.red[0], k_and); atomicOr(&sm.red[1], k_or); }
+    __syncthreads();
+    const uint32_t diff = sm.red[0] ^ sm.red[1];
+    if (diff == 0u) return;
+    const int lo = __builtin_ctz(diff), hi = 31 - __builtin_clz(diff);
+    const int npass = (hi - lo + 8) / 8;
+    const int per = (hi - lo + npass) / npass;
+    uint32_t* const sk = sm.kv;
+    uint32_t* const sv = sm.kv + kTileSortCap;
+
+    if (in_lds) {
+        for (int p = 0; p < npass; ++p) {
+            const int shift = lo + p * per, bits = min(per, hi + 1 - shift);
+            const uint32_t mask = (1u << bits) - 1u;
+            tile_sort_rank(sm, key, rank, ipl0, chunk0, n, shift, mask);
+#pragma unroll
+            for (int i = 0; i < kTileSortItems; ++i) {
+                if (i >= ipl0) continue;
+                const uint32_t d = (key[i] >> shift) & mask;
+                rank[i] += sm.dig_start[d] + sm.hist[wave][d];
+            }
+#pragma unroll
+            for (int i = 0; i < kTileSortItems; ++i) {
+                if (i >= ipl0) continue;
+                if (wave * chunk0 + i * kWave + lane < n) {
+                    sk[rank[i]] = key[i];
+                    sv[rank[i]] = val[i];
+                }
+            }
+            __syncthreads();
+            if (p + 1 < npass) {
+#pragma unroll
+                for (int i = 0; i < kTileSortItems; ++i) {
+                    if (i >= ipl0) continue;
+                    const int e = min(wave * chunk0 + i * kWave + lane, n - 1);
+                    key[i] = sk[e];
+                    val[i] = sv[e];
+                }
+                __syncthreads();
+            }
+        }
+        for (int j = tid; j < n; j += kBlock) seg[j] = sv[j];
+        return;
+    }
+
+    for (int p = 0; p < npass; ++p) {
+        const int shift = lo + p * per, bits = min(per, hi + 1 - shift);
+        const uint32_t mask = (1u << bits) - 1u;
+        const uint32_t* __restrict__ src = (p & 1) ? alt : seg;
+        uint32_t* __restrict__ dst = (p & 1) ? seg : alt;
+        sm.base[tid] = 0u;
+        __syncthreads();
+        for (int j = tid; j < n; j += kBlock) atomicAdd(&sm.base[(depth_keys[src[j] & kGidMask] >> shift) & mask], 1u);
+        __syncthreads();
+        uint32_t total;
+        const uint32_t start = block_exclusive_scan(sm.base[tid], total, sm.scan_sums);
+        sm.base[tid] = start;
+        for (int c0 = 0; c0 < n; c0 += kTileSortCap) {
+            const int m = min(kTileSortCap, n - c0);
+            const int ipl = (m + kBlock - 1) / kBlock, chunk = ipl * kWave;
+            load_items(src + c0, depth_keys, key, val, ipl, wave * chunk + lane, m);
+            const uint32_t cnt = tile_sort_rank(sm, key, rank, ipl, chunk, m, shift, mask);
+#pragma unroll
+            for (int i = 0; i < kTileSortItems; ++i) {
+                if (i >= ipl) continue;
+                if (wave * chunk + i * kWave + lane < m) {
+                    const uint32_t d = (key[i] >> shift) & mask;
+                    dst[sm.base[d] + sm.hist[wave][d] + rank[i]] = val[i];
+                }
+            }
+            __syncthreads();
+            sm.base[tid] += cnt;
+        }
+        __syncthreads();
+    }
+    if (npass & 1) {
+        for (int j = tid; j < n; j += kBlock) seg[j] = alt[j];
+    }
+}
+
+__global__ __launch_bounds__(kBlock) void tile_depth_sort_kernel(const uint2* __restrict__ ranges, int tiles,
+                                                                 const uint32_t* __restrict__ tile_order,
+                                                                 uint32_t* __restrict__ point_list,
+                                                                 const uint32_t* __restrict__ depth_keys,
+                                                                 uint32_t* __restrict__ scratch) {
+    __shared__ TileSortLds sm;
+    const int wave = threadIdx.x >> 6;
+    if (threadIdx.x < kTileSortWaves) {
+        const int b = blockIdx.x * kTileSortWaves + threadIdx.x;
+        sm.range[threadIdx.x] = b < tiles ? ranges[tile_order ? tile_order[b] : (uint32_t)b] : make_uint2(0u, 0u);
+    }
+    __syncthreads();
+    const uint32_t x = (uint32_t)__builtin_amdgcn_readfirstlane((int)sm.range[wave].x);
+    const int n = __builtin_amdgcn_readfirstlane((int)(sm.range[wave].y - sm.range[wave].x));
+    if (n >= 2 && n <= kWaveSortCap) wave_sort_list(sm, point_list + x, n, depth_keys);
+#pragma unroll 1
+    for (int w = 0; w < kTileSortWaves; ++w) {
+        const uint32_t xw = (uint32_t)__builtin_amdgcn_readfirstlane((int)sm.range[w].x);
+        const int nw = __builtin_amdgcn_readfirstlane((int)(sm.range[w].y - sm.range[w].x));
+        if (nw > kWaveSortCap) block_sort_list(sm, point_list + xw, scratch + xw, nw, depth_keys);
+    }
+}
+
 __global__ __launch_bounds__(kBlock) void export_keys_kernel(const uint2* __restrict__ ranges,
                                                              const uint32_t* __restrict__ point_list,
                                                              const float4* __restrict__ rec, int recv4,
@@ -644,6 +933,17 @@
     return OGS_OK;
 }
 
+int launch_tile_depth_sort(const uint2* ranges, int64_t tiles, const uint32_t* tile_order, uint32_t* point_list,
+                           const uint32_t* depth_keys, uint32_t* scratch, hipStream_t s, int debug) {
+    if (tiles <= 0) return OGS_OK;
+    if (tiles >= (1ll << 31)) { set_error("tile_depth_sort: %lld tiles", (long long)tiles); return OGS_ERR_UNSUPPORTED; }
+    const unsigned grid = (unsigned)((tiles + kTileSortWaves - 1) / kTileSortWaves);
+    OGS_LAUNCH(tile_depth_sort_kernel, dim3(grid), dim3(kBlock), 0, s, ranges, (int)tiles, tile_order, point_list, depth_keys,
+               scratch);
+    OGS_LAUNCH_CHECK(debug, s);
+    return OGS_OK;
+}
+
 int launch_export_keys(const uint2* ranges, int tiles, const uint32_t* point_list, const float4* rec, int recv4,
                        uint64_t* keys_out, hipStream_t s) {
     OGS_LAUNCH(export_keys_kernel, dim3(tiles), dim3(kBlock), 0, s, ranges, point_list, rec, recv4, keys_out);
diff --git a/opengaussian_amd/csrc/blend_fwd.hip b/opengaussian_amd/csrc/blend_fwd.hip
--- a/opengaussian_amd/csrc/blend_fwd.hip
+++ b/opengaussian_amd/csrc/blend_fwd.hip
@@ -769,12 +769,12 @@
 }
 
 template <int C>
-int launch_c(const OgsRasterFwdArgs& a, const GeomState& gs, const ImageState& is, int64_t D, hipStream_t s) {
+int launch_c(const OgsRasterFwdArgs& a, const GeomState& gs, const ImageState& is, int64_t D, hipStream_t s, bool order_ready) {
     const int gx = (a.W + kTile - 1) / kTile, gy = (a.H + kTile - 1) / kTile;
     const int tiles = gx * gy;
     const unsigned vtiles = (unsigned)tiles * (unsigned)num_groups_of(a.num_groups);
     if (D > 0) {
-        const uint32_t* order = launch_tile_order(is, vtiles, a.P, s, a.debug);
+        const uint32_t* order = order_ready ? tile_order_of(is, vtiles, a.P) : launch_tile_order(is, vtiles, a.P, s, a.debug);
         static constexpr const char* const kChunked[4] = {"pack_blend_chunked_kernel<3>", "pack_blend_chunked_kernel<6>",
                                                           "pack_blend_chunked_kernel<9>", "pack_blend_chunked_kernel<12>"};
         OGS_LAUNCH_NAMED(chan_name<C>(kChunked), pack_blend_chunked_kernel<C>, dim3(vtiles), dim3(kBlock), 0, s,
@@ -796,7 +796,8 @@
 }
 
 template <int C>
-int stats_c(const OgsRasterFwdArgs& a, const OgsGroupStatsArgs& sa, const GeomState& gs, const ImageState& is, hipStream_t s) {
+int stats_c(const OgsRasterFwdArgs& a, const OgsGroupStatsArgs& sa, const GeomState& gs, const ImageState& is, hipStream_t s,
+            bool order_ready) {
     const int gx = (a.W + kTile - 1) / kTile, gy = (a.H + kTile - 1) / kTile;
     const int tiles = gx * gy;
     const int G = num_groups_of(a.num_groups);
@@ -806,7 +807,7 @@
     OGS_HIP_CHECK(hipMemsetAsync(sa.max_alpha, 0, (size_t)G * sizeof(float), s));
     OGS_HIP_CHECK(hipMemsetAsync(sa.count, 0, rows * sizeof(int64_t), s));
     OGS_HIP_CHECK(hipMemsetAsync(fixed, 0, rows * C * sizeof(long long), s));
-    const uint32_t* order = launch_tile_order(is, vtiles, a.P, s, a.debug);
+    const uint32_t* order = order_ready ? tile_order_of(is, vtiles, a.P) : launch_tile_order(is, vtiles, a.P, s, a.debug);
     GroupStatsOut st;
     st.labels = sa.labels;
     st.L = sa.num_labels;
@@ -924,23 +925,23 @@
 }
 
 int launch_blend_forward(const OgsRasterFwdArgs& a, const GeomState& gs, const ImageState& is, int64_t D,
-                         hipStream_t s) {
+                         hipStream_t s, bool order_ready) {
     switch (a.C) {
-        case 3: return launch_c<3>(a, gs, is, D, s);
-        case 6: return launch_c<6>(a, gs, is, D, s);
-        case 9: return launch_c<9>(a, gs, is, D, s);
-        case 12: return launch_c<12>(a, gs, is, D, s);
+        case 3: return launch_c<3>(a, gs, is, D, s, order_ready);
+        case 6: return launch_c<6>(a, gs, is, D, s, order_ready);
+        case 9: return launch_c<9>(a, gs, is, D, s, order_ready);
+        case 12: return launch_c<12>(a, gs, is, D, s, order_ready);
         default: set_error("unsupported channel count C=%d", a.C); return OGS_ERR_UNSUPPORTED;
     }
 }
 
 int launch_group_stats(const OgsRasterFwdArgs& a, const OgsGroupStatsArgs& st, const GeomState& gs, const ImageState& is,
-                       hipStream_t s) {
+                       hipStream_t s, bool order_ready) {
     switch (a.C) {
-        case 3: return stats_c<3>(a, st, gs, is, s);
-        case 6: return stats_c<6>(a, st, gs, is, s);
-        case 9: return stats_c<9>(a, st, gs, is, s);
-        case 12: return stats_c<12>(a, st, gs, is, s);
+        case 3: return stats_c<3>(a, st, gs, is, s, order_ready);
+        case 6: return stats_c<6>(a, st, gs, is, s, order_ready);
+        case 9: return stats_c<9>(a, st, gs, is, s, order_ready);
+        case 12: return stats_c<12>(a, st, gs, is, s, order_ready);
         default: set_error("unsupported channel count C=%d", a.C); return OGS_ERR_UNSUPPORTED;
     }
 }
diff --git a/opengaussian_amd/csrc/capi.hip b/opengaussian_amd/csrc/capi.hip
--- a/opengaussian_amd/csrc/capi.hip
+++ b/opengaussian_amd/csrc/capi.hip
@@ -143,7 +143,7 @@
 
 extern "C" {
 
-int ogs_version(void) { return 400; }
+int ogs_version(void) { return 401; }
 
 int ogs_check_async_status(void) { return check_async_status("ogs_check_async_status"); }
 
@@ -217,6 +217,11 @@
     if (a->P <= kSmallMaxP) {
         rc = launch_small_geometry(*a, gs, gt, s);
         if (rc != OGS_OK) return rc;
+    } else if (per_tile_depth_order(*a)) {
+        rc = launch_preprocess(*a, gs, gt, s);
+        if (rc != OGS_OK) return rc;
+        rc = exclusive_scan_u32(gt.tiles_touched, nullptr, gt.offsets, a->P, gt.num_rendered, gt.sort_tmp, s, a->debug);
+        if (rc != OGS_OK) return rc;
     } else {
         rc = launch_preprocess(*a, gs, gt, s);
         if (rc != OGS_OK) return rc;
@@ -269,6 +274,8 @@
     const int64_t tiles = (int64_t)gx * gy * G;
     if (tiles >= (1ll << 31)) { set_error("%d groups x %d tiles exceed 2^31 virtual tiles", G, gx * gy); return OGS_ERR_UNSUPPORTED; }
     const GeomState gs = GeomState::carve(a->geom_buffer, a->P > 0 ? a->P : 1, a->C);
+    const bool per_tile = per_tile_depth_order(*a);
+    bool order_ready = false;
     if (D > 0) {
         if (!a->point_list || !a->binning_tmp) { set_error("point_list / binning_tmp == NULL with num_rendered=%lld", (long long)D); return OGS_ERR_INVALID_ARG; }
         if (D >= (1ll << 31)) { set_error("num_rendered=%lld exceeds 2^31", (long long)D); return OGS_ERR_UNSUPPORTED; }
@@ -283,8 +290,8 @@
         const uint32_t* n_dev = deferred ? gt.num_rendered : nullptr;
         const bool cull = a->full_binning == 0;
         const bool zero_in_dup = tiles <= (int64_t)a->P;
-        rc = launch_duplicate(*a, gs, gt, bt.tile_keys[0], vbuf[0], (uint32_t)D, cull, s, zero_in_dup ? is.ranges : nullptr,
-                              zero_in_dup ? (int)tiles : 0);
+        rc = launch_duplicate(*a, gs, gt, bt.tile_keys[0], vbuf[0], (uint32_t)D, cull, !per_tile, s,
+                              zero_in_dup ? is.ranges : nullptr, zero_in_dup ? (int)tiles : 0);
         if (rc != OGS_OK) return rc;
         const bool sweep = radix_onesweep_enabled(D);
         int shifts[4], nbits[4];
@@ -309,12 +316,18 @@
         }
         rc = launch_tile_ranges(bt.tile_keys[passes & 1], D, is.ranges, tiles, s, a->debug, cull ? bt.kept : n_dev, zero_in_dup);
         if (rc != OGS_OK) return rc;
+        if (per_tile) {
+            const uint32_t* order = launch_tile_order(is, tiles, a->P, s, a->debug);
+            order_ready = true;
+            rc = launch_tile_depth_sort(is.ranges, tiles, order, a->point_list, gt.keys[0], bt.vals, s, a->debug);
+            if (rc != OGS_OK) return rc;
+        }
     } else {
         OGS_HIP_CHECK(hipMemsetAsync(is.ranges, 0, (size_t)tiles * sizeof(uint2), s));
     }
-    if (stats) return launch_group_stats(*a, *stats, gs, is, s);
+    if (stats) return launch_group_stats(*a, *stats, gs, is, s, order_ready);
     if (!a->sorted_rec || !a->quad_list) { set_error("sorted_rec / quad_list == NULL"); return OGS_ERR_INVALID_ARG; }
-    return launch_blend_forward(*a, gs, is, D, s);
+    return launch_blend_forward(*a, gs, is, D, s, order_ready);
 }
 
 int ogs_raster_forward_render(const OgsRasterFwdArgs* a, int64_t D, void* stream_) {
@@ -373,6 +386,10 @@
 }
 
 size_t ogs_raster_tiny_max_points(void) { return (size_t)kTinyMaxP; }
+
+size_t ogs_raster_tile_sort_capacity(int32_t level) {
+    return level == 0 ? (size_t)kWaveSortCap : level == 1 ? (size_t)kTileSortCap : 0;
+}
 
 int ogs_raster_forward_tiny(const OgsRasterFwdArgs* a, void* stream_) {
     int rc = validate_fwd(a);
diff --git a/opengaussian_amd/csrc/ogs_common.h b/opengaussian_amd/csrc/ogs_common.h
--- a/opengaussian_amd/csrc/ogs_common.h
+++ b/opengaussian_amd/csrc/ogs_common.h
@@ -257,15 +257,21 @@
 int launch_compact_kept(int W, int H, int C, const ImageState& is_old, const ImageState& is_new, const void* old_rec,
                         const void* old_quad, void* new_rec, void* new_quad, hipStream_t s);
 int launch_duplicate(const OgsRasterFwdArgs& a, const GeomState& gs, const GeomTmp& gt, uint32_t* tile_keys,
-                     uint32_t* vals, uint32_t capacity, bool drop_unreachable, hipStream_t s, uint2* zero_ranges = nullptr,
-                     int n_zero = 0);
+                     uint32_t* vals, uint32_t capacity, bool drop_unreachable, bool depth_order, hipStream_t s,
+                     uint2* zero_ranges = nullptr, int n_zero = 0);
 int launch_tile_ranges(const uint32_t* tile_keys_sorted, int64_t D, uint2* ranges, int64_t tiles, hipStream_t s,
                        int debug, const uint32_t* n_dev = nullptr, bool already_zeroed = false);
+inline bool per_tile_depth_order(const OgsRasterFwdArgs& a) { return a.num_groups <= 1 && a.P > kSmallMaxP; }
+constexpr int kTileSortItems = 16;
+constexpr int kTileSortCap = kBlock * kTileSortItems;
+constexpr int kWaveSortCap = kTileSortCap / (kBlock / kWave);
+int launch_tile_depth_sort(const uint2* ranges, int64_t tiles, const uint32_t* tile_order, uint32_t* point_list,
+                           const uint32_t* depth_keys, uint32_t* scratch, hipStream_t s, int debug);
 inline int num_groups_of(int g) { return g > 1 ? g : 1; }
 int launch_group_stats(const OgsRasterFwdArgs& a, const OgsGroupStatsArgs& st, const GeomState& gs, const ImageState& is,
-                       hipStream_t s);
+                       hipStream_t s, bool order_ready = false);
 int launch_blend_forward(const OgsRasterFwdArgs& a, const GeomState& gs, const ImageState& is, int64_t D,
-                         hipStream_t s);
+                         hipStream_t s, bool order_ready = false);
 int launch_blend_backward(const OgsRasterBwdArgs& a, const ImageState& is, void* grad_rec, hipStream_t s);
 int launch_preprocess_backward(const OgsRasterBwdArgs& a, const GeomState& gs, const void* grad_rec, hipStream_t s);
 inline bool backward_is_features_only(const OgsRasterBwdArgs& a) {
diff --git a/opengaussian_amd/csrc/preprocess_fwd.hip b/opengaussian_amd/csrc/preprocess_fwd.hip
--- a/opengaussian_amd/csrc/preprocess_fwd.hip
+++ b/opengaussian_amd/csrc/preprocess_fwd.hip
@@ -228,7 +228,7 @@
                                             means3D, colors_precomp, shs, opacities, scales, rotations, cov3D_precomp, viewmatrix,
                                             projmatrix, campos, s_rec + tid * NV, clamped_out, radii, tiles_touched, group_ids,
                                             num_groups);
-        order[idx] = (uint32_t)idx;
+        if (order) order[idx] = (uint32_t)idx;
     }
     __syncthreads();
     const size_t row0 = (size_t)blockIdx.x * kBlock;
@@ -337,14 +337,14 @@
     const int tid = threadIdx.x;
     const int r = blockIdx.x * kBlock + tid;
     if (zero_ranges != nullptr && r < n_zero) zero_ranges[r] = make_uint2(0u, 0u);
-    const int P = min(P_cap, (int)*n_visible);
+    const int P = n_visible ? min(P_cap, (int)*n_visible) : P_cap;
     if ((int)blockIdx.x * kBlock >= P) return;
     const int gx = (W + kTile - 1) / kTile, gy = (H + kTile - 1) / kTile;
     uint32_t off = 0, cnt = 0, gid = 0, rect = 1u << 24, key0 = 0;
     float4 ctr = make_float4(0.f, 0.f, 0.f, 0.f);
     float4 con = make_float4(1.f, 1.f, 0.f, 0.f);
     if (r < P) {
-        gid = order[r];
+        gid = order ? order[r] : (uint32_t)r;
         off = offsets[r];
         if (group_ids != nullptr) key0 = (uint32_t)max(group_ids[gid], 0) * (uint32_t)(gx * gy);
         const float4 a = rec[(size_t)gid * NV];
@@ -440,8 +440,8 @@
     OGS_LAUNCH_NAMED(chan_name<C>(kNames), preprocess_kernel<C>, dim3(grid), dim3(kBlock), 0, s, a.P, a.W, a.H, a.sh_degree, a.sh_coeffs,
                        a.tanfovx, a.tanfovy, focal_x, focal_y, a.scale_modifier, a.means3D, a.colors_precomp, a.shs,
                        a.opacities, a.scales, a.rotations, a.cov3D_precomp, a.viewmatrix, a.projmatrix, a.campos,
-                       gs.rec, gs.clamped, a.radii, gt.tiles_touched, gt.keys[0], gt.order[0],
-                       a.num_groups > 1 ? a.group_ids : (const int32_t*)nullptr, a.num_groups);
+                       gs.rec, gs.clamped, a.radii, gt.tiles_touched, gt.keys[0],
+                       per_tile_depth_order(a) ? (uint32_t*)nullptr : gt.order[0], a.num_groups > 1 ? a.group_ids : (const int32_t*)nullptr, a.num_groups);
     OGS_LAUNCH_CHECK(a.debug, s);
     return OGS_OK;
 }
@@ -502,7 +502,8 @@
 }
 
 int launch_duplicate(const OgsRasterFwdArgs& a, const GeomState& gs, const GeomTmp& gt, uint32_t* tile_keys,
-                     uint32_t* vals, uint32_t capacity, bool drop_unreachable, hipStream_t s, uint2* zero_ranges, int n_zero) {
+                     uint32_t* vals, uint32_t capacity, bool drop_unreachable, bool depth_order, hipStream_t s, uint2* zero_ranges,
+                     int n_zero) {
     if (n_zero > a.P) { set_error("duplicate: %d ranges to clear with %d threads", n_zero, a.P); return OGS_ERR_INVALID_ARG; }
     const int grid = (a.P + kBlock - 1) / kBlock;
     const int32_t* grp = a.num_groups > 1 ? a.group_ids : nullptr;
@@ -510,10 +511,12 @@
         set_error("image %dx%d exceeds 4095 tiles per side", a.W, a.H);
         return OGS_ERR_UNSUPPORTED;
     }
+    const uint32_t* order = depth_order ? gt.order[0] : nullptr;
+    const uint32_t* n_visible = depth_order ? gt.visible() : nullptr;
     switch (rec_vec4(a.C)) {
-        case 3: OGS_LAUNCH(duplicate_kernel<3>, dim3(grid), dim3(kBlock), 0, s, a.P, (const uint32_t*)gt.visible(), a.W, a.H, gs.rec, gt.order[0], gt.offsets, tile_keys, vals, capacity, grp, drop_unreachable, zero_ranges, n_zero); break;
-        case 4: OGS_LAUNCH(duplicate_kernel<4>, dim3(grid), dim3(kBlock), 0, s, a.P, (const uint32_t*)gt.visible(), a.W, a.H, gs.rec, gt.order[0], gt.offsets, tile_keys, vals, capacity, grp, drop_unreachable, zero_ranges, n_zero); break;
-        case 5: OGS_LAUNCH(duplicate_kernel<5>, dim3(grid), dim3(kBlock), 0, s, a.P, (const uint32_t*)gt.visible(), a.W, a.H, gs.rec, gt.order[0], gt.offsets, tile_keys, vals, capacity, grp, drop_unreachable, zero_ranges, n_zero); break;
+        case 3: OGS_LAUNCH(duplicate_kernel<3>, dim3(grid), dim3(kBlock), 0, s, a.P, n_visible, a.W, a.H, gs.rec, order, gt.offsets, tile_keys, vals, capacity, grp, drop_unreachable, zero_ranges, n_zero); break;
+        case 4: OGS_LAUNCH(duplicate_kernel<4>, dim3(grid), dim3(kBlock), 0, s, a.P, n_visible, a.W, a.H, gs.rec, order, gt.offsets, tile_keys, vals, capacity, grp, drop_unreachable, zero_ranges, n_zero); break;
+        case 5: OGS_LAUNCH(duplicate_kernel<5>, dim3(grid), dim3(kBlock), 0, s, a.P, n_visible, a.W, a.H, gs.rec, order, gt.offsets, tile_keys, vals, capacity, grp, drop_unreachable, zero_ranges, n_zero); break;
         default: set_error("unsupported record size"); return OGS_ERR_UNSUPPORTED;
     }
     OGS_LAUNCH_CHECK(a.debug, s);
```

Result: faster. 1449 Mpix/s, median of 6 (+3.9%).
